# fujii-team/deComP

Measured on AMD Instinct MI355X. Metric: nmf_mu_iterations_per_s, higher is better.
Workload: dtype f32; 1 GPU; nmf_mu l2 no-mask Y=65536x4096 k=256 fp32 (BASELINE configs[1]); rows_per_gpu=65536, parallelism=rows sharded x1, 1 all-reduce/step, loop=single-GPU dcp_nmf_mu_f32

## Files before the change

### decomp_amd/_hip.py

```python
import ctypes
import os
import threading

_HERE = os.path.dirname(os.path.abspath(__file__))
LIB_PATH = os.path.join(_HERE, 'lib', 'libdecomp_hip.so')

OK = 0
ERR_NAMES = {-1: 'DCP_ERR_INVALID', -2: 'DCP_ERR_HIP', -3: 'DCP_ERR_NOMEM',
             -4: 'DCP_ERR_INTERNAL', -5: 'DCP_ERR_UNSUPPORTED', -6: 'DCP_ERR_REF_TYPEERROR',
             -7: 'DCP_ERR_COMM'}
LIK_L2, LIK_KL, LIK_BETA = 0, 1, 2
PROF_NLABELS = 10
PROF_XUPDATE, PROF_STATS = 2, 4
LASSO_ISTA, LASSO_ACC_ISTA, LASSO_FISTA, LASSO_CD = 0, 1, 2, 3
LASSO_PARALLEL_CD, LASSO_ADMM = 4, 5
LASSO_OMP = 6
LASSO_POSITIVE = 0x100
ERR_REF_TYPEERROR = -6
ERR_COMM = -7
COMM_ID_BYTES = 128
ALLREDUCE_FN = ctypes.CFUNCTYPE(ctypes.c_int, ctypes.c_void_p, ctypes.c_int64, ctypes.c_int, ctypes.c_void_p, ctypes.c_void_p)

_c_int, _c_i64, _c_vp = ctypes.c_int, ctypes.c_int64, ctypes.c_void_p
_c_f32, _c_f64 = ctypes.c_float, ctypes.c_double
_P = ctypes.POINTER

SIGNATURES = {
    'dcp_create': (_c_int, [_P(_c_vp), _c_int]),
    'dcp_destroy': (_c_int, [_c_vp]),
    'dcp_set_stream': (_c_int, [_c_vp, _c_vp]),
    'dcp_last_error_string': (ctypes.c_char_p, [_c_vp]),
    'dcp_build_info': (ctypes.c_char_p, []),
    'dcp_comm_unique_id': (_c_int, [_c_vp, _c_i64]),
    'dcp_comm_init': (_c_int, [_c_vp, _c_vp, _c_int, _c_int]),
    'dcp_comm_destroy': (_c_int, [_c_vp]),
    'dcp_comm_set_external': (_c_int, [_c_vp, _c_vp, _c_vp, _c_int, _c_int]),
    'dcp_memcpy': (_c_int, [_c_vp, _c_vp, _c_vp, _c_i64]),
    'dcp_comm_info': (_c_int, [_c_vp, _P(_c_int), _P(_c_int)]),
    'dcp_comm_allreduce_sum_f32': (_c_int, [_c_vp, _c_vp, _c_i64]),
    'dcp_comm_allreduce_sum_f64': (_c_int, [_c_vp, _c_vp, _c_i64]),
    'dcp_nmf_mu_sharded_f32': (_c_int, [_c_vp, _c_vp, _c_vp, _c_vp, _c_vp, _c_i64, _c_i64, _c_i64,
                                        _c_int, _c_f32, _c_int, _P(_c_int), _P(_c_f32)]),
    'dcp_nmf_mu_sharded_f64': (_c_int, [_c_vp, _c_vp, _c_vp, _c_vp, _c_vp, _c_i64, _c_i64, _c_i64,
                                        _c_int, _c_f64, _c_int, _P(_c_int), _P(_c_f64)]),
    'dcp_profile_enable': (_c_int, [_c_vp, _c_int]),
    'dcp_profile_reset': (_c_int, [_c_vp]),
    'dcp_profile_select': (_c_int, [_c_vp, ctypes.c_uint]),
    'dcp_profile_read': (_c_int, [_c_vp, _c_int, _P(_c_f64), _P(_c_i64)]),
    'dcp_profile_label_name': (ctypes.c_char_p, [_c_int]),
    'dcp_l2_normalize_f32': (_c_int, [_c_vp, _c_vp, _c_i64, _c_i64, _c_int]),
    'dcp_l2_normalize_f64': (_c_int, [_c_vp, _c_vp, _c_i64, _c_i64, _c_int]),
    'dcp_l2_normalize_c64': (_c_int, [_c_vp, _c_vp, _c_i64, _c_i64, _c_int]),
    'dcp_l2_normalize_c128': (_c_int, [_c_vp, _c_vp, _c_i64, _c_i64, _c_int]),
    'dcp_count_negative_f32': (_c_int, [_c_vp, _c_vp, _c_i64, _P(_c_i64)]),
    'dcp_count_negative_f64': (_c_int, [_c_vp, _c_vp, _c_i64, _P(_c_i64)]),
    'dcp_gemm_f32': (_c_int, [_c_vp, _c_int, _c_vp, _c_vp, _c_vp, _c_i64, _c_i64, _c_i64,
                              _c_int, _c_int]),
    'dcp_gemm_f64': (_c_int, [_c_vp, _c_int, _c_vp, _c_vp, _c_vp, _c_i64, _c_i64, _c_i64,
                              _c_int, _c_int]),
    'dcp_gather_rows_bytes': (_c_int, [_c_vp, _c_vp, _c_vp, _c_i64, _c_i64, _c_vp]),
    'dcp_scatter_rows_bytes': (_c_int, [_c_vp, _c_vp, _c_vp, _c_i64, _c_i64, _c_vp]),
    'dcp_dict_prefetch_rows_bytes': (_c_int, [_c_vp, _c_vp, _c_vp, _c_i64, _c_i64, _c_vp]),
    'dcp_dict_set_pcd_order': (_c_int, [_c_vp, _c_vp, _c_i64, _c_i64]),
    'dcp_lasso_f32': (_c_int, [_c_vp, _c_vp, _c_vp, _c_int, _c_vp, _c_vp, _c_i64, _c_i64, _c_i64, _c_f64, _c_f64, _c_int, _c_int, _c_int, _P(_c_int)]),
    'dcp_lasso_f64': (_c_int, [_c_vp, _c_vp, _c_vp, _c_int, _c_vp, _c_vp, _c_i64, _c_i64, _c_i64, _c_f64, _c_f64, _c_int, _c_int, _c_int, _P(_c_int)]),
    'dcp_lasso_c64': (_c_int, [_c_vp, _c_vp, _c_vp, _c_int, _c_vp, _c_vp, _c_i64, _c_i64, _c_i64, _c_f64, _c_f64, _c_int, _c_int, _c_int, _P(_c_int)]),
    'dcp_lasso_c128': (_c_int, [_c_vp, _c_vp, _c_vp, _c_int, _c_vp, _c_vp, _c_i64, _c_i64, _c_i64, _c_f64, _c_f64, _c_int, _c_int, _c_int, _P(_c_int)]),
    'dcp_lasso_pcd_f32': (_c_int, [_c_vp, _c_vp, _c_vp, _c_int, _c_vp, _c_vp, _c_i64, _c_i64, _c_i64, _c_f64, _c_f64, _c_int, _c_int, _c_vp, _c_i64, _P(_c_int)]),
    'dcp_lasso_admm_f32': (_c_int, [_c_vp, _c_vp, _c_vp, _c_int, _c_vp, _c_vp, _c_i64, _c_i64, _c_i64, _c_f64, _c_f64, _c_int, _c_int, _c_f64, _P(_c_int)]),
    'dcp_lasso_pcd_f64': (_c_int, [_c_vp, _c_vp, _c_vp, _c_int, _c_vp, _c_vp, _c_i64, _c_i64, _c_i64, _c_f64, _c_f64, _c_int, _c_int, _c_vp, _c_i64, _P(_c_int)]),
    'dcp_lasso_admm_f64': (_c_int, [_c_vp, _c_vp, _c_vp, _c_int, _c_vp, _c_vp, _c_i64, _c_i64, _c_i64, _c_f64, _c_f64, _c_int, _c_int, _c_f64, _P(_c_int)]),
    'dcp_lasso_pcd_c64': (_c_int, [_c_vp, _c_vp, _c_vp, _c_int, _c_vp, _c_vp, _c_i64, _c_i64, _c_i64, _c_f64, _c_f64, _c_int, _c_int, _c_vp, _c_i64, _P(_c_int)]),
    'dcp_lasso_admm_c64': (_c_int, [_c_vp, _c_vp, _c_vp, _c_int, _c_vp, _c_vp, _c_i64, _c_i64, _c_i64, _c_f64, _c_f64, _c_int, _c_int, _c_f64, _P(_c_int)]),
    'dcp_lasso_pcd_c128': (_c_int, [_c_vp, _c_vp, _c_vp, _c_int, _c_vp, _c_vp, _c_i64, _c_i64, _c_i64, _c_f64, _c_f64, _c_int, _c_int, _c_vp, _c_i64, _P(_c_int)]),
    'dcp_lasso_admm_c128': (_c_int, [_c_vp, _c_vp, _c_vp, _c_int, _c_vp, _c_vp, _c_i64, _c_i64, _c_i64, _c_f64, _c_f64, _c_int, _c_int, _c_f64, _P(_c_int)]),
    'dcp_omp_f32': (_c_int, [_c_vp, _c_vp, _c_vp, _c_vp, _c_i64, _c_i64, _c_i64, _c_int, _c_f64, _P(_c_int)]),
    'dcp_omp_f64': (_c_int, [_c_vp, _c_vp, _c_vp, _c_vp, _c_i64, _c_i64, _c_i64, _c_int, _c_f64, _P(_c_int)]),
    'dcp_omp_c64': (_c_int, [_c_vp, _c_vp, _c_vp, _c_vp, _c_i64, _c_i64, _c_i64, _c_int, _c_f64, _P(_c_int)]),
    'dcp_omp_c128': (_c_int, [_c_vp, _c_vp, _c_vp, _c_vp, _c_i64, _c_i64, _c_i64, _c_int, _c_f64, _P(_c_int)]),
    'dcp_omp_gram_f32': (_c_int, [_c_vp, _c_vp, _c_vp, _c_vp, _c_vp, _c_i64, _c_i64, _c_int, _c_f64, _P(_c_int)]),
    'dcp_omp_gram_f64': (_c_int, [_c_vp, _c_vp, _c_vp, _c_vp, _c_vp, _c_i64, _c_i64, _c_int, _c_f64, _P(_c_int)]),
    'dcp_omp_gram_c64': (_c_int, [_c_vp, _c_vp, _c_vp, _c_vp, _c_vp, _c_i64, _c_i64, _c_int, _c_f64, _P(_c_int)]),
    'dcp_omp_gram_c128': (_c_int, [_c_vp, _c_vp, _c_vp, _c_vp, _c_vp, _c_i64, _c_i64, _c_int, _c_f64, _P(_c_int)]),
    'dcp_omp_mask_f32': (_c_int, [_c_vp, _c_vp, _c_vp, _c_int, _c_vp, _c_vp, _c_i64, _c_i64, _c_i64, _c_int, _c_f64, _c_int, _P(_c_int)]),
    'dcp_omp_mask_f64': (_c_int, [_c_vp, _c_vp, _c_vp, _c_int, _c_vp, _c_vp, _c_i64, _c_i64, _c_i64, _c_int, _c_f64, _c_int, _P(_c_int)]),
    'dcp_omp_mask_c64': (_c_int, [_c_vp, _c_vp, _c_vp, _c_int, _c_vp, _c_vp, _c_i64, _c_i64, _c_i64, _c_int, _c_f64, _c_int, _P(_c_int)]),
    'dcp_omp_mask_c128': (_c_int, [_c_vp, _c_vp, _c_vp, _c_int, _c_vp, _c_vp, _c_i64, _c_i64, _c_i64, _c_int, _c_f64, _c_int, _P(_c_int)]),
    'dcp_ksvd_sweep_f32': (_c_int, [_c_vp, _c_vp, _c_vp, _c_vp, _c_i64, _c_i64, _c_i64, _c_int, _P(_c_f64)]),
    'dcp_ksvd_sweep_f64': (_c_int, [_c_vp, _c_vp, _c_vp, _c_vp, _c_i64, _c_i64, _c_i64, _c_int, _P(_c_f64)]),
    'dcp_ksvd_sweep_c64': (_c_int, [_c_vp, _c_vp, _c_vp, _c_vp, _c_i64, _c_i64, _c_i64, _c_int, _P(_c_f64)]),
    'dcp_ksvd_sweep_c128': (_c_int, [_c_vp, _c_vp, _c_vp, _c_vp, _c_i64, _c_i64, _c_i64, _c_int, _P(_c_f64)]),
    'dcp_ksvd_step_f32': (_c_int, [_c_vp, _c_vp, _c_vp, _c_vp, _c_i64, _c_i64, _c_i64, _c_int, _c_f64, _P(_c_f64), _P(_c_int)]),
    'dcp_ksvd_step_f64': (_c_int, [_c_vp, _c_vp, _c_vp, _c_vp, _c_i64, _c_i64, _c_i64, _c_int, _c_f64, _P(_c_f64), _P(_c_int)]),
    'dcp_ksvd_step_c64': (_c_int, [_c_vp, _c_vp, _c_vp, _c_vp, _c_i64, _c_i64, _c_i64, _c_int, _c_f64, _P(_c_f64), _P(_c_int)]),
    'dcp_ksvd_step_c128': (_c_int, [_c_vp, _c_vp, _c_vp, _c_vp, _c_i64, _c_i64, _c_i64, _c_int, _c_f64, _P(_c_f64), _P(_c_int)]),
    'dcp_ksvd_mask_sweep_f32': (_c_int, [_c_vp, _c_vp, _c_vp, _c_int, _c_vp, _c_vp, _c_i64, _c_i64, _c_i64, _c_int, _P(_c_f64)]),
    'dcp_ksvd_mask_sweep_f64': (_c_int, [_c_vp, _c_vp, _c_vp, _c_int, _c_vp, _c_vp, _c_i64, _c_i64, _c_i64, _c_int, _P(_c_f64)]),
    'dcp_ksvd_mask_sweep_c64': (_c_int, [_c_vp, _c_vp, _c_vp, _c_int, _c_vp, _c_vp, _c_i64, _c_i64, _c_i64, _c_int, _P(_c_f64)]),
    'dcp_ksvd_mask_sweep_c128': (_c_int, [_c_vp, _c_vp, _c_vp, _c_int, _c_vp, _c_vp, _c_i64, _c_i64, _c_i64, _c_int, _P(_c_f64)]),
    'dcp_ksvd_mask_step_f32': (_c_int, [_c_vp, _c_vp, _c_vp, _c_int, _c_vp, _c_vp, _c_i64, _c_i64, _c_i64, _c_int, _c_f64, _c_int, _P(_c_f64), _P(_c_int)]),
    'dcp_ksvd_mask_step_f64': (_c_int, [_c_vp, _c_vp, _c_vp, _c_int, _c_vp, _c_vp, _c_i64, _c_i64, _c_i64, _c_int, _c_f64, _c_int, _P(_c_f64), _P(_c_int)]),
    'dcp_ksvd_mask_step_c64': (_c_int, [_c_vp, _c_vp, _c_vp, _c_int, _c_vp, _c_vp, _c_i64, _c_i64, _c_i64, _c_int, _c_f64, _c_int, _P(_c_f64), _P(_c_int)]),
    'dcp_ksvd_mask_step_c128': (_c_int, [_c_vp, _c_vp, _c_vp, _c_int, _c_vp, _c_vp, _c_i64, _c_i64, _c_i64, _c_int, _c_f64, _c_int, _P(_c_f64), _P(_c_int)]),
    'dcp_dict_stats_f32': (_c_int, [_c_vp, _c_vp, _c_vp, _c_vp, _c_i64, _c_i64, _c_i64, _c_f64, _c_int, _c_int, _c_f64, _c_vp, _P(_c_int)]),
    'dcp_dict_update_f32': (_c_int, [_c_vp, _c_vp, _c_f64, _c_vp, _c_vp, _c_vp, _c_vp, _c_i64, _c_i64, _c_vp]),
    'dcp_dict_step_f32': (_c_int, [_c_vp, _c_vp, _c_vp, _c_vp, _c_vp, _c_vp, _c_vp, _c_i64, _c_i64, _c_i64, _c_f64, _c_f64, _c_int, _c_int, _c_f64, _P(_c_f64), _P(_c_int)]),
    'dcp_dict_step_async_f32': (_c_int, [_c_vp, _c_vp, _c_vp, _c_vp, _c_vp, _c_vp, _c_vp, _c_i64, _c_i64, _c_i64, _c_f64, _c_f64, _c_int, _c_int, _c_f64, _c_vp, _P(_c_int)]),
    'dcp_gather_rows_f32': (_c_int, [_c_vp, _c_vp, _c_vp, _c_i64, _c_i64, _c_vp]),
    'dcp_dict_stats_f64': (_c_int, [_c_vp, _c_vp, _c_vp, _c_vp, _c_i64, _c_i64, _c_i64, _c_f64, _c_int, _c_int, _c_f64, _c_vp, _P(_c_int)]),
    'dcp_dict_update_f64': (_c_int, [_c_vp, _c_vp, _c_f64, _c_vp, _c_vp, _c_vp, _c_vp, _c_i64, _c_i64, _c_vp]),
    'dcp_dict_step_f64': (_c_int, [_c_vp, _c_vp, _c_vp, _c_vp, _c_vp, _c_vp, _c_vp, _c_i64, _c_i64, _c_i64, _c_f64, _c_f64, _c_int, _c_int, _c_f64, _P(_c_f64), _P(_c_int)]),
    'dcp_dict_step_async_f64': (_c_int, [_c_vp, _c_vp, _c_vp, _c_vp, _c_vp, _c_vp, _c_vp, _c_i64, _c_i64, _c_i64, _c_f64, _c_f64, _c_int, _c_int, _c_f64, _c_vp, _P(_c_int)]),
    'dcp_gather_rows_f64': (_c_int, [_c_vp, _c_vp, _c_vp, _c_i64, _c_i64, _c_vp]),
    'dcp_dict_stats_c64': (_c_int, [_c_vp, _c_vp, _c_vp, _c_vp, _c_i64, _c_i64, _c_i64, _c_f64, _c_int, _c_int, _c_f64, _c_vp, _P(_c_int)]),
    'dcp_dict_update_c64': (_c_int, [_c_vp, _c_vp, _c_f64, _c_vp, _c_vp, _c_vp, _c_vp, _c_i64, _c_i64, _c_vp]),
    'dcp_dict_step_c64': (_c_int, [_c_vp, _c_vp, _c_vp, _c_vp, _c_vp, _c_vp, _c_vp, _c_i64, _c_i64, _c_i64, _c_f64, _c_f64, _c_int, _c_int, _c_f64, _P(_c_f64), _P(_c_int)]),
    'dcp_dict_step_async_c64': (_c_int, [_c_vp, _c_vp, _c_vp, _c_vp, _c_vp, _c_vp, _c_vp, _c_i64, _c_i64, _c_i64, _c_f64, _c_f64, _c_int, _c_int, _c_f64, _c_vp, _P(_c_int)]),
    'dcp_gather_rows_c64': (_c_int, [_c_vp, _c_vp, _c_vp, _c_i64, _c_i64, _c_vp]),
    'dcp_dict_stats_c128': (_c_int, [_c_vp, _c_vp, _c_vp, _c_vp, _c_i64, _c_i64, _c_i64, _c_f64, _c_int, _c_int, _c_f64, _c_vp, _P(_c_int)]),
    'dcp_dict_update_c128': (_c_int, [_c_vp, _c_vp, _c_f64, _c_vp, _c_vp, _c_vp, _c_vp, _c_i64, _c_i64, _c_vp]),
    'dcp_dict_step_c128': (_c_int, [_c_vp, _c_vp, _c_vp, _c_vp, _c_vp, _c_vp, _c_vp, _c_i64, _c_i64, _c_i64, _c_f64, _c_f64, _c_int, _c_int, _c_f64, _P(_c_f64), _P(_c_int)]),
    'dcp_dict_step_async_c128': (_c_int, [_c_vp, _c_vp, _c_vp, _c_vp, _c_vp, _c_vp, _c_vp, _c_i64, _c_i64, _c_i64, _c_f64, _c_f64, _c_int, _c_int, _c_f64, _c_vp, _P(_c_int)]),
    'dcp_gather_rows_c128': (_c_int, [_c_vp, _c_vp, _c_vp, _c_i64, _c_i64, _c_vp]),
    'dcp_dict_mask_step_f32': (_c_int, [_c_vp, _c_vp, _c_vp, _c_vp, _c_vp, _c_vp, _c_vp, _c_vp, _c_i64, _c_i64, _c_i64, _c_f64, _c_f64, _c_int, _c_int, _c_f64, _P(_c_f64), _P(_c_int)]),
    'dcp_dict_mask_step_f64': (_c_int, [_c_vp, _c_vp, _c_vp, _c_vp, _c_vp, _c_vp, _c_vp, _c_vp, _c_i64, _c_i64, _c_i64, _c_f64, _c_f64, _c_int, _c_int, _c_f64, _P(_c_f64), _P(_c_int)]),
    'dcp_dict_mask_step_c64': (_c_int, [_c_vp, _c_vp, _c_vp, _c_vp, _c_vp, _c_vp, _c_vp, _c_vp, _c_i64, _c_i64, _c_i64, _c_f64, _c_f64, _c_int, _c_int, _c_f64, _P(_c_f64), _P(_c_int)]),
    'dcp_dict_mask_step_c128': (_c_int, [_c_vp, _c_vp, _c_vp, _c_vp, _c_vp, _c_vp, _c_vp, _c_vp, _c_i64, _c_i64, _c_i64, _c_f64, _c_f64, _c_int, _c_int, _c_f64, _P(_c_f64), _P(_c_int)]),
    'dcp_nmf_grads_f32': (_c_int, [_c_vp, _c_vp, _c_vp, _c_vp, _c_vp, _c_i64, _c_i64, _c_i64, _c_int, _c_int, _c_vp, _c_vp]),
    'dcp_nmf_grads_f64': (_c_int, [_c_vp, _c_vp, _c_vp, _c_vp, _c_vp, _c_i64, _c_i64, _c_i64, _c_int, _c_int, _c_vp, _c_vp]),
    'dcp_nmf_grad_x_f32': (_c_int, [_c_vp, _c_vp, _c_vp, _c_vp, _c_vp, _c_i64, _c_i64, _c_i64, _c_int, _c_vp, _c_vp]),
    'dcp_nmf_grad_x_f64': (_c_int, [_c_vp, _c_vp, _c_vp, _c_vp, _c_vp, _c_i64, _c_i64, _c_i64, _c_int, _c_vp, _c_vp]),
    'dcp_nmf_gauss_logp_f32': (_c_int, [_c_vp, _c_vp, _c_vp, _c_vp, _c_vp, _c_i64, _c_i64, _c_i64, _c_f64, _P(_c_f64)]),
    'dcp_nmf_gauss_logp_f64': (_c_int, [_c_vp, _c_vp, _c_vp, _c_vp, _c_vp, _c_i64, _c_i64, _c_i64, _c_f64, _P(_c_f64)]),
    'dcp_set_nmf_beta': (_c_int, [_c_vp, _c_f64]),
    'dcp_set_nmf_penalty': (_c_int, [_c_vp, _c_f64, _c_f64]),
    'dcp_nmf_beta_divergence_f32': (_c_int, [_c_vp, _c_vp, _c_vp, _c_vp, _c_vp, _c_i64, _c_i64, _c_i64, _P(_c_f64)]),
    'dcp_nmf_beta_divergence_f64': (_c_int, [_c_vp, _c_vp, _c_vp, _c_vp, _c_vp, _c_i64, _c_i64, _c_i64, _P(_c_f64)]),
    'dcp_nmf_apply_f32': (_c_int, [_c_vp, _c_vp, _c_vp, _c_vp, _c_f64, _c_vp, _c_i64, _c_i64, _P(_c_f64)]),
    'dcp_nmf_apply_f64': (_c_int, [_c_vp, _c_vp, _c_vp, _c_vp, _c_f64, _c_vp, _c_i64, _c_i64, _P(_c_f64)]),
    'dcp_axpby_f32': (_c_int, [_c_vp, _c_i64, _c_f64, _c_vp, _c_f64, _c_vp]),
    'dcp_axpby_f64': (_c_int, [_c_vp, _c_i64, _c_f64, _c_vp, _c_f64, _c_vp]),
    'dcp_mu_quotient_f32': (_c_int, [_c_vp, _c_vp, _c_vp, _c_vp, _c_i64, _c_i64, _c_vp]),
    'dcp_mu_quotient_f64': (_c_int, [_c_vp, _c_vp, _c_vp, _c_vp, _c_i64, _c_i64, _c_vp]),
    'dcp_l2_normalize_diff_f32': (_c_int, [_c_vp, _c_vp, _c_vp, _c_vp, _c_i64, _c_i64, _c_int, _P(_c_f64)]),
    'dcp_l2_normalize_diff_f64': (_c_int, [_c_vp, _c_vp, _c_vp, _c_vp, _c_i64, _c_i64, _c_int, _P(_c_f64)]),
    'dcp_gershgorin_f32': (_c_int, [_c_vp, _c_vp, _c_i64, _c_i64, _c_vp]),
    'dcp_gershgorin_f64': (_c_int, [_c_vp, _c_vp, _c_i64, _c_i64, _c_vp]),
    'dcp_gershgorin_c64': (_c_int, [_c_vp, _c_vp, _c_i64, _c_i64, _c_vp]),
    'dcp_gershgorin_c128': (_c_int, [_c_vp, _c_vp, _c_i64, _c_i64, _c_vp]),
    'dcp_inv_f32': (_c_int, [_c_vp, _c_vp, _c_i64, _c_i64, _c_vp]),
    'dcp_inv_f64': (_c_int, [_c_vp, _c_vp, _c_i64, _c_i64, _c_vp]),
    'dcp_inv_c64': (_c_int, [_c_vp, _c_vp, _c_i64, _c_i64, _c_vp]),
    'dcp_inv_c128': (_c_int, [_c_vp, _c_vp, _c_i64, _c_i64, _c_vp]),
    'dcp_debug_tn_plain': (_c_int, [_c_int]),
    'dcp_debug_gemm_route': (_c_int, [_c_int, _c_int, _c_i64, _c_i64, _c_i64, _c_i64, _c_int, _c_int, _c_int, _c_int,
                                      _c_int, _c_vp]),
    'dcp_gemm_bf16x6_f32': (_c_int, [_c_vp, _c_int, _c_vp, _c_vp, _c_vp, _c_i64, _c_i64, _c_i64, _c_int]),
    'dcp_set_f32_product_mode': (_c_int, [_c_vp, _c_int]),
    'dcp_calib_read_f32': (_c_int, [_c_vp, _c_vp, _c_i64, _c_i64, _c_int, _c_vp]),
    'dcp_gemm_c64': (_c_int, [_c_vp, _c_int, _c_vp, _c_vp, _c_vp, _c_i64, _c_i64, _c_i64,
                              _c_int, _c_int]),
    'dcp_gemm_c128': (_c_int, [_c_vp, _c_int, _c_vp, _c_vp, _c_vp, _c_i64, _c_i64, _c_i64,
                              _c_int, _c_int]),
    'dcp_nmf_mu_f32': (_c_int, [_c_vp, _c_vp, _c_vp, _c_vp, _c_vp, _c_i64, _c_i64, _c_i64,
                                _c_int, _c_f32, _c_int, _P(_c_int), _P(_c_f32), _P(_c_f32)]),
    'dcp_nmf_mu_f64': (_c_int, [_c_vp, _c_vp, _c_vp, _c_vp, _c_vp, _c_i64, _c_i64, _c_i64,
                                _c_int, _c_f64, _c_int, _P(_c_int), _P(_c_f64), _P(_c_f64)]),
    'dcp_nmf_hals_f32': (_c_int, [_c_vp, _c_vp, _c_vp, _c_vp, _c_i64, _c_i64, _c_i64, _c_f32, _c_int,
                                  _P(_c_int), _P(_c_f32), _P(_c_f32)]),
    'dcp_nmf_hals_f64': (_c_int, [_c_vp, _c_vp, _c_vp, _c_vp, _c_i64, _c_i64, _c_i64, _c_f64, _c_int,
                                  _P(_c_int), _P(_c_f64), _P(_c_f64)]),
    'dcp_nmf_hals_sharded_f32': (_c_int, [_c_vp, _c_vp, _c_vp, _c_vp, _c_i64, _c_i64, _c_i64, _c_f32, _c_int,
                                          _P(_c_int), _P(_c_f32)]),
    'dcp_nmf_hals_sharded_f64': (_c_int, [_c_vp, _c_vp, _c_vp, _c_vp, _c_i64, _c_i64, _c_i64, _c_f64, _c_int,
                                          _P(_c_int), _P(_c_f64)]),
    'dcp_nmf_impute_f32': (_c_int, [_c_vp, _c_vp, _c_vp, _c_vp, _c_vp, _c_i64, _c_i64, _c_i64, _c_vp]),
    'dcp_nmf_impute_f64': (_c_int, [_c_vp, _c_vp, _c_vp, _c_vp, _c_vp, _c_i64, _c_i64, _c_i64, _c_vp]),
    'dcp_nmf_emhals_f32': (_c_int, [_c_vp, _c_vp, _c_vp, _c_vp, _c_vp, _c_i64, _c_i64, _c_i64, _c_f32, _c_int,
                                    _P(_c_int), _P(_c_f32), _P(_c_f32)]),
    'dcp_nmf_emhals_f64': (_c_int, [_c_vp, _c_vp, _c_vp, _c_vp, _c_vp, _c_i64, _c_i64, _c_i64, _c_f64, _c_int,
                                    _P(_c_int), _P(_c_f64), _P(_c_f64)]),
    'dcp_nmf_emhals_sharded_f32': (_c_int, [_c_vp, _c_vp, _c_vp, _c_vp, _c_vp, _c_i64, _c_i64, _c_i64, _c_f32,
                                            _c_int, _P(_c_int), _P(_c_f32)]),
    'dcp_nmf_emhals_sharded_f64': (_c_int, [_c_vp, _c_vp, _c_vp, _c_vp, _c_vp, _c_i64, _c_i64, _c_i64, _c_f64,
                                            _c_int, _P(_c_int), _P(_c_f64)]),
    'dcp_nmf_hals_stats_f32': (_c_int, [_c_vp, _c_vp, _c_vp, _c_vp, _c_vp, _c_i64, _c_i64, _c_i64, _c_vp]),
    'dcp_nmf_hals_stats_f64': (_c_int, [_c_vp, _c_vp, _c_vp, _c_vp, _c_vp, _c_i64, _c_i64, _c_i64, _c_vp]),
    'dcp_nmf_hals_update_f32': (_c_int, [_c_vp, _c_vp, _c_vp, _c_vp, _c_vp, _c_i64, _c_i64, _c_i64, _c_vp, _c_vp]),
    'dcp_nmf_hals_update_f64': (_c_int, [_c_vp, _c_vp, _c_vp, _c_vp, _c_vp, _c_i64, _c_i64, _c_i64, _c_vp, _c_vp]),
    'dcp_nn_cd_sweep_f32': (_c_int, [_c_vp, _c_vp, _c_vp, _c_vp, _c_vp, _c_i64, _c_i64, _c_int]),
    'dcp_nn_cd_sweep_f64': (_c_int, [_c_vp, _c_vp, _c_vp, _c_vp, _c_vp, _c_i64, _c_i64, _c_int]),
    'dcp_nmf_mu_stats_width': (_c_i64, [_c_i64, _c_i64, _c_int, _c_int]),
    'dcp_nmf_mu_stats_f32': (_c_int, [_c_vp, _c_vp, _c_vp, _c_vp, _c_vp, _c_vp, _c_i64, _c_i64,
                                      _c_i64, _c_int, _c_vp]),
    'dcp_nmf_mu_stats_f64': (_c_int, [_c_vp, _c_vp, _c_vp, _c_vp, _c_vp, _c_vp, _c_i64, _c_i64,
                                      _c_i64, _c_int, _c_vp]),
    'dcp_nmf_mask_bits_words': (_c_i64, [_c_i64, _c_i64]),
    'dcp_nmf_mask_prepare_f32': (_c_int, [_c_vp, _c_vp, _c_vp, _c_i64, _c_i64, _c_vp, _c_vp, _P(_c_int)]),
    'dcp_nmf_mask_prepare_f64': (_c_int, [_c_vp, _c_vp, _c_vp, _c_i64, _c_i64, _c_vp, _c_vp, _P(_c_int)]),
    'dcp_nmf_mu_stats_prepared_f32': (_c_int, [_c_vp, _c_vp, _c_vp, _c_vp, _c_vp, _c_vp, _c_vp, _c_i64,
                                               _c_i64, _c_i64, _c_int, _c_vp]),
    'dcp_nmf_mu_stats_prepared_f64': (_c_int, [_c_vp, _c_vp, _c_vp, _c_vp, _c_vp, _c_vp, _c_vp, _c_i64,
                                               _c_i64, _c_i64, _c_int, _c_vp]),
    'dcp_nmf_mu_update_f32': (_c_int, [_c_vp, _c_vp, _c_vp, _c_vp, _c_i64, _c_i64, _c_int,
                                       _c_int, _c_vp, _c_vp]),
    'dcp_nmf_mu_update_f64': (_c_int, [_c_vp, _c_vp, _c_vp, _c_vp, _c_i64, _c_i64, _c_int,
                                       _c_int, _c_vp, _c_vp]),
    'dcp_nmf_residual_f32': (_c_int, [_c_vp, _c_vp, _c_vp, _c_vp, _c_vp, _c_i64, _c_i64, _c_i64,
                                      _P(_c_f64)]),
    'dcp_nmf_residual_f64': (_c_int, [_c_vp, _c_vp, _c_vp, _c_vp, _c_vp, _c_i64, _c_i64, _c_i64,
                                      _P(_c_f64)]),
    'dcp_tm_temp2mat_f32': (_c_int, [_c_vp, _c_vp, _c_i64, _c_i64, _c_i64, _c_i64, _c_int, _c_vp]),
    'dcp_tm_temp2mat_f64': (_c_int, [_c_vp, _c_vp, _c_i64, _c_i64, _c_i64, _c_i64, _c_int, _c_vp]),
    'dcp_tm_temp2mat_c64': (_c_int, [_c_vp, _c_vp, _c_i64, _c_i64, _c_i64, _c_i64, _c_int, _c_vp]),
    'dcp_tm_temp2mat_c128': (_c_int, [_c_vp, _c_vp, _c_i64, _c_i64, _c_i64, _c_i64, _c_int, _c_vp]),
    'dcp_tm_coef2mat_f32': (_c_int, [_c_vp, _c_vp, _c_i64, _c_i64, _c_i64, _c_i64, _c_i64, _c_int, _c_vp]),
    'dcp_tm_coef2mat_f64': (_c_int, [_c_vp, _c_vp, _c_i64, _c_i64, _c_i64, _c_i64, _c_i64, _c_int, _c_vp]),
    'dcp_tm_coef2mat_c64': (_c_int, [_c_vp, _c_vp, _c_i64, _c_i64, _c_i64, _c_i64, _c_i64, _c_int, _c_vp]),
    'dcp_tm_coef2mat_c128': (_c_int, [_c_vp, _c_vp, _c_i64, _c_i64, _c_i64, _c_i64, _c_i64, _c_int, _c_vp]),
    'dcp_tm_predict_f32': (_c_int, [_c_vp, _c_vp, _c_vp, _c_i64, _c_i64, _c_i64, _c_i64, _c_i64, _c_int, _c_vp]),
    'dcp_tm_predict_f64': (_c_int, [_c_vp, _c_vp, _c_vp, _c_i64, _c_i64, _c_i64, _c_i64, _c_i64, _c_int, _c_vp]),
    'dcp_tm_predict_c64': (_c_int, [_c_vp, _c_vp, _c_vp, _c_i64, _c_i64, _c_i64, _c_i64, _c_i64, _c_int, _c_vp]),
    'dcp_tm_predict_c128': (_c_int, [_c_vp, _c_vp, _c_vp, _c_i64, _c_i64, _c_i64, _c_i64, _c_i64, _c_int, _c_vp]),
    'dcp_tm_lasso_f32': (_c_int, [_c_vp, _c_vp, _c_vp, _c_vp, _c_i64, _c_i64, _c_i64, _c_i64, _c_i64, _c_int, _c_f64, _c_f64, _c_int, _c_int, _c_int, _P(_c_int)]),
    'dcp_tm_lasso_f64': (_c_int, [_c_vp, _c_vp, _c_vp, _c_vp, _c_i64, _c_i64, _c_i64, _c_i64, _c_i64, _c_int, _c_f64, _c_f64, _c_int, _c_int, _c_int, _P(_c_int)]),
    'dcp_tm_lasso_c64': (_c_int, [_c_vp, _c_vp, _c_vp, _c_vp, _c_i64, _c_i64, _c_i64, _c_i64, _c_i64, _c_int, _c_f64, _c_f64, _c_int, _c_int, _c_int, _P(_c_int)]),
    'dcp_tm_lasso_c128': (_c_int, [_c_vp, _c_vp, _c_vp, _c_vp, _c_i64, _c_i64, _c_i64, _c_i64, _c_i64, _c_int, _c_f64, _c_f64, _c_int, _c_int, _c_int, _P(_c_int)]),
    'dcp_tm_dstep_f32': (_c_int, [_c_vp, _c_vp, _c_vp, _c_vp, _c_vp, _c_vp, _c_i64, _c_i64, _c_i64, _c_i64, _c_i64, _c_int, _c_int, _P(_c_f64)]),
    'dcp_tm_dstep_f64': (_c_int, [_c_vp, _c_vp, _c_vp, _c_vp, _c_vp, _c_vp, _c_i64, _c_i64, _c_i64, _c_i64, _c_i64, _c_int, _c_int, _P(_c_f64)]),
    'dcp_tm_dstep_c64': (_c_int, [_c_vp, _c_vp, _c_vp, _c_vp, _c_vp, _c_vp, _c_i64, _c_i64, _c_i64, _c_i64, _c_i64, _c_int, _c_int, _P(_c_f64)]),
    'dcp_tm_dstep_c128': (_c_int, [_c_vp, _c_vp, _c_vp, _c_vp, _c_vp, _c_vp, _c_i64, _c_i64, _c_i64, _c_i64, _c_i64, _c_int, _c_int, _P(_c_f64)]),
    'dcp_tm_gather_windows_f32': (_c_int, [_c_vp, _c_vp, _c_vp, _c_vp, _c_vp, _c_i64, _c_i64, _c_i64, _c_i64, _c_i64, _c_i64, _c_i64, _c_int, _c_vp, _c_vp]),
    'dcp_tm_gather_windows_f64': (_c_int, [_c_vp, _c_vp, _c_vp, _c_vp, _c_vp, _c_i64, _c_i64, _c_i64, _c_i64, _c_i64, _c_i64, _c_i64, _c_int, _c_vp, _c_vp]),
    'dcp_tm_gather_windows_c64': (_c_int, [_c_vp, _c_vp, _c_vp, _c_vp, _c_vp, _c_i64, _c_i64, _c_i64, _c_i64, _c_i64, _c_i64, _c_i64, _c_int, _c_vp, _c_vp]),
    'dcp_tm_gather_windows_c128': (_c_int, [_c_vp, _c_vp, _c_vp, _c_vp, _c_vp, _c_i64, _c_i64, _c_i64, _c_i64, _c_i64, _c_i64, _c_i64, _c_int, _c_vp, _c_vp]),
    'dcp_tm_scatter_windows_f32': (_c_int, [_c_vp, _c_vp, _c_vp, _c_vp, _c_vp, _c_i64, _c_i64, _c_i64, _c_i64, _c_i64, _c_i64, _c_i64, _c_int]),
    'dcp_tm_scatter_windows_f64': (_c_int, [_c_vp, _c_vp, _c_vp, _c_vp, _c_vp, _c_i64, _c_i64, _c_i64, _c_i64, _c_i64, _c_i64, _c_i64, _c_int]),
    'dcp_tm_scatter_windows_c64': (_c_int, [_c_vp, _c_vp, _c_vp, _c_vp, _c_vp, _c_i64, _c_i64, _c_i64, _c_i64, _c_i64, _c_i64, _c_i64, _c_int]),
    'dcp_tm_scatter_windows_c128': (_c_int, [_c_vp, _c_vp, _c_vp, _c_vp, _c_vp, _c_i64, _c_i64, _c_i64, _c_i64, _c_i64, _c_i64, _c_i64, _c_int]),
}

_lib = None
_lock = threading.Lock()
_handles = {}


class HipLibraryError(RuntimeError):
    """The HIP library is missing, failed to load, or a call into it failed."""


def load():
    global _lib
    with _lock:
        if _lib is not None:
            return _lib
        if not os.path.exists(LIB_PATH):
            raise HipLibraryError(
                'libdecomp_hip.so not found at %s. Build it with `make` (or '
                '`python -c "import __graft_entry__ as g; g.build()"`). decomp_amd has no '
                'CPU fallback: the HIP library is the compute path.' % LIB_PATH)
        try:
            lib = ctypes.CDLL(LIB_PATH)
        except OSError as e:
            raise HipLibraryError('cannot load %s: %s' % (LIB_PATH, e))
        for name, (res, args) in SIGNATURES.items():
            fn = getattr(lib, name)
            fn.restype = res
            fn.argtypes = args
        _lib = lib
        return _lib


def handle(device):
    lib = load()
    with _lock:
        h = _handles.get(device)
        if h is None:
            out = _c_vp()
            rc = lib.dcp_create(ctypes.byref(out), int(device))
            if rc != OK or not out.value:
                raise HipLibraryError(
                    'dcp_create(device=%d) failed (%s): no usable HIP device. decomp_amd '
                    'computes only on the GPU.' % (device, ERR_NAMES.get(rc, rc)))
            h = out
            _handles[device] = h
        return h


def check(h, rc, what):
    if rc != OK:
        msg = load().dcp_last_error_string(h)
        raise HipLibraryError('%s failed: %s (%s)' % (
            what, ERR_NAMES.get(rc, rc), msg.decode() if msg else ''))
```

### decomp_amd/csrc/gemm_mfma_bf16x6.hpp

```cpp
#pragma once
#include "gemm_mfma_f32.hpp"
#include <type_traits>

namespace dcp {

typedef __bf16 x6_bf16x4 __attribute__((ext_vector_type(4)));
typedef __bf16 x6_bf16x8 __attribute__((ext_vector_type(8)));

template <int BM_, int BN_, int WM_, int WN_, int MINW_, int STAGES_>
struct X6Cfg {
    static constexpr int BM = BM_, BN = BN_, BK = 16, WM = WM_, WN = WN_, MINW = MINW_;
    static constexpr int NWAVES = (BM_ / WM_) * (BN_ / WN_);
    static constexpr int NTHREADS = 64 * NWAVES;
    static constexpr int STAGES = STAGES_;
};
typedef X6Cfg<256, 256, 64, 64, 1, 3> X6Huge;
typedef X6Cfg<128, 128, 64, 64, 2, 2> X6Large;

template <int ROWS>
struct X6Panel {
    static constexpr int PLANE_BYTES = ROWS * 32;
    static constexpr int BYTES = 3 * PLANE_BYTES;
};

__device__ __forceinline__ int x6_chunk(int r, int q) { return r * 32 + ((q ^ ((r >> 3) & 1)) << 4); }

__device__ __forceinline__ void x6_split(f32x4 a, x6_bf16x4& h, x6_bf16x4& m, x6_bf16x4& l) {
    h = __builtin_convertvector(a, x6_bf16x4);
    const f32x4 r1 = a - __builtin_convertvector(h, f32x4);
    m = __builtin_convertvector(r1, x6_bf16x4);
    const f32x4 r2 = r1 - __builtin_convertvector(m, f32x4);
    l = __builtin_convertvector(r2, x6_bf16x4);
}

template <int LAY, int ROWS, int NT, int G>
__device__ __forceinline__ void x6_gload(f32x4 (&r)[G], const float* __restrict__ p, long ld, int row0, int k0,
                                         int tid) {
    static_assert(G * NT * 4 == ROWS * 16, "panel must be a whole number of 4-value groups per thread");
#pragma unroll
    for (int i = 0; i < G; ++i) {
        const int idx = tid + i * NT;
        if (LAY == KMAJOR) {
            const int row = idx >> 2, kq = idx & 3;
            r[i] = *reinterpret_cast<const f32x4*>(p + (long)(row0 + row) * ld + (k0 + 4 * kq));
        } else {
            const int g = idx % (ROWS / 4), k = idx / (ROWS / 4);
            r[i] = *reinterpret_cast<const f32x4*>(p + (long)(k0 + k) * ld + (row0 + 4 * g));
        }
    }
}

template <int ROWS>
__device__ __forceinline__ int x6_granule(int k, int g) {
    static_assert(ROWS >= 128, "the XOR swizzle needs 32 granules per k row");
    return k * (ROWS * 2) + ((g ^ ((k & 3) << 3)) << 3);
}

template <int LAY, int ROWS, int NT, int G>
__device__ __forceinline__ void x6_lds_store(char* s, const f32x4 (&r)[G], int tid) {
#pragma unroll
    for (int i = 0; i < G; ++i) {
        const int idx = tid + i * NT;
        int off;
        if (LAY == KMAJOR) {
            const int row = idx >> 2, kq = idx & 3;
            off = x6_chunk(row, kq >> 1) + ((kq & 1) << 3);
        } else {
            off = x6_granule<ROWS>(idx / (ROWS / 4), idx % (ROWS / 4));
        }
        x6_bf16x4 h, m, l;
        x6_split(r[i], h, m, l);
        *reinterpret_cast<x6_bf16x4*>(s + off) = h;
        *reinterpret_cast<x6_bf16x4*>(s + X6Panel<ROWS>::PLANE_BYTES + off) = m;
        *reinterpret_cast<x6_bf16x4*>(s + 2 * X6Panel<ROWS>::PLANE_BYTES + off) = l;
    }
}

template <int LAY, int ROWS>
__device__ __forceinline__ int x6_frag_off(int r0, int lane) {
    const int l31 = lane & 31, h = lane >> 5;
    if (LAY == KMAJOR) return x6_chunk(r0 + l31, h);
    const int q = (lane >> 2) & 3, pq = lane & 3, gh = (lane >> 4) & 1;
    return x6_granule<ROWS>(8 * h + q, (r0 >> 2) + 4 * gh + pq);
}

template <int LAY, int ROWS>
__device__ __forceinline__ x6_bf16x8 x6_frag(const char* plane, int off) {
    if (LAY == KMAJOR) return *reinterpret_cast<const x6_bf16x8*>(plane + off);
    typedef short s16x4 __attribute__((ext_vector_type(4)));
    typedef __attribute__((address_space(3))) s16x4 lds_s16x4;
    const s16x4 lo = __builtin_amdgcn_ds_read_tr16_b64_v4i16((lds_s16x4*)(plane + off));
    const s16x4 hi = __builtin_amdgcn_ds_read_tr16_b64_v4i16((lds_s16x4*)(plane + off + 4 * ROWS * 2));
    return __builtin_bit_cast(x6_bf16x8, __builtin_shufflevector(lo, hi, 0, 1, 2, 3, 4, 5, 6, 7));
}

template <class E, class = void>
struct epi_den_tail { static constexpr bool value = false; };
template <class E>
struct epi_den_tail<E, decltype((void)E::kDenTail)> { static constexpr bool value = E::kDenTail; };

typedef float x6_f32x2 __attribute__((ext_vector_type(2)));

__device__ __forceinline__ int x6_den_xoff(int r, int q) { return r * 16 + ((q ^ ((r >> 2) & 3)) << 2); }

template <class Epi>
__device__ __forceinline__ void x6_den_tail(f32x16 (&num)[2][2], const Epi& epi, char* smem, int m0, int n0, int tid) {
    constexpr int XS = 128 * 16 * 4;
    constexpr int GS = 16 * 256 * 4;
    constexpr int DBUF = XS + GS;
    const int lane = tid & 63, wave = tid >> 6;
    const int wm = wave >> 2, wn = wave & 3;
    const int l31 = lane & 31, h = lane >> 5;
    const int nkd = epi.depth >> 4;

    const int pr = tid >> 3, k2 = tid & 7;
    const float* xsrc = epi.cur + (long)(m0 + (pr >> 5) * 64 + (pr & 31)) * epi.ld_cur + 2 * k2;
    const int xdst = (x6_den_xoff(pr, k2 >> 1) + 2 * (k2 & 1)) * 4;
    const int gk = tid >> 6, gc = tid & 63;
    const float* gsrc = epi.gram + (long)gk * epi.ld_gram + (n0 + 4 * gc);
    const int gdst = XS + (gk * 256 + 4 * gc) * 4;
    int lp = 0, lk = 0;
    auto gload = [&](x6_f32x2& rx, f32x4& rg) {
        rx = *reinterpret_cast<const x6_f32x2*>(xsrc + (long)(32 * lp) * epi.ld_cur + 16 * lk);
        rg = *reinterpret_cast<const f32x4*>(gsrc + (long)(16 * lk) * epi.ld_gram);
        if (lk + 1 < nkd) {
            ++lk;
        } else if (lp == 0) {
            lp = 1;
            lk = 0;
        }
    };
    auto lstore = [&](int buf, const x6_f32x2& rx, const f32x4& rg) {
        *reinterpret_cast<x6_f32x2*>(smem + buf + xdst) = rx;
        *reinterpret_cast<f32x4*>(smem + buf + gdst) = rg;
    };

    x6_f32x2 rx;
    f32x4 rg;
    int b0 = 0, b1 = DBUF, b2 = 2 * DBUF;
    {
        x6_f32x2 rx0, rx1;
        f32x4 rg0, rg1;
        gload(rx0, rg0);
        gload(rx1, rg1);
        gload(rx, rg);
        __syncthreads();
        lstore(b0, rx0, rg0);
        lstore(b1, rx1, rg1);
        __syncthreads();
    }

    const int xfrag0 = x6_den_xoff(wm * 32 + l31, h) * 4, xfrag1 = x6_den_xoff(wm * 32 + l31, 2 + h) * 4;
    const int gfrag = XS + ((4 * h) * 256 + wn * 64 + l31) * 4;
    const int tq = l31 & 3, col0 = l31 & ~3;

    auto pass = [&](auto i_tag) {
        constexpr int i = decltype(i_tag)::value;
        f32x16 den[2];
#pragma unroll
        for (int j = 0; j < 2; ++j)
#pragma unroll
            for (int r = 0; r < 16; ++r) den[j][r] = 0.0f;
        for (int kb = 0; kb < nkd; ++kb) {
            const char* s = smem + b0;
            auto frags = [&](int xoff, int c, f32x4& fa, f32x4 (&fb)[2]) {
                fa = *reinterpret_cast<const f32x4*>(s + xoff);
                const float* g = reinterpret_cast<const float*>(s + gfrag) + c * 8 * 256;
#pragma unroll
                for (int j = 0; j < 2; ++j)
#pragma unroll
                    for (int st = 0; st < 4; ++st) fb[j][st] = g[st * 256 + j * 32];
            };
            auto mfmas = [&](const f32x4& fa, const f32x4 (&fb)[2]) {
#pragma unroll
                for (int st = 0; st < 4; ++st)
#pragma unroll
                    for (int j = 0; j < 2; ++j)
                        den[j] = __builtin_amdgcn_mfma_f32_32x32x2f32(fa[st], fb[j][st], den[j], 0, 0, 0);
            };
            f32x4 fa, fb[2];
            frags(xfrag0, 0, fa, fb);
            mfmas(fa, fb);
            __builtin_amdgcn_sched_barrier(0);
            lstore(b2, rx, rg);
            f32x4 ga, gb[2];
            frags(xfrag1, 1, ga, gb);
            __builtin_amdgcn_sched_barrier(0);
            __syncthreads();
            __builtin_amdgcn_sched_barrier(0);
            gload(rx, rg);
            mfmas(ga, gb);
            __builtin_amdgcn_sched_barrier(0);
            const int t0 = b0;
            b0 = b1;
            b1 = b2;
            b2 = t0;
        }
#pragma unroll
        for (int j = 0; j < 2; ++j)
#pragma unroll
            for (int g = 0; g < 4; ++g) {
                f32x4 a, d;
#pragma unroll
                for (int e = 0; e < 4; ++e) {
                    a[e] = num[i][j][4 * g + e];
                    d[e] = den[j][4 * g + e];
                }
                epi.quot4(m0 + wm * 64 + i * 32 + 8 * g + 4 * h + tq, n0 + wn * 64 + j * 32 + col0,
                          quad_transpose(a, tq), quad_transpose(d, tq));
            }
    };
    pass(std::integral_constant<int, 0>{});
    pass(std::integral_constant<int, 1>{});
}

template <class Cfg, int ALAY, int BLAY, class Epi>
__global__ void __launch_bounds__(Cfg::NTHREADS, Cfg::MINW) gemm_bf16x6_kernel(GemmProblem p, Epi epi) {
    constexpr int BM = Cfg::BM, BN = Cfg::BN, BK = Cfg::BK, WM = Cfg::WM, WN = Cfg::WN;
    constexpr int TM = WM / 32, TN = WN / 32;
    constexpr int WAVES_N = BN / WN;
    constexpr int NT = Cfg::NTHREADS;
    constexpr int GA = BM * BK / 4 / NT, GB = BN * BK / 4 / NT;
    constexpr int PA = X6Panel<BM>::PLANE_BYTES, PB = X6Panel<BN>::PLANE_BYTES;
    constexpr int BUF = X6Panel<BM>::BYTES + X6Panel<BN>::BYTES;
    static_assert(epi_mode<Epi>::value == 0 && !epi_rowbits<Epi>::value, "bf16x6 core: plain real epilogues");

    extern __shared__ __attribute__((aligned(16))) char x6_smem[];

    const int tid = threadIdx.x;
    const int lane = tid & 63, wave = tid >> 6;
    const int wm = wave / WAVES_N, wn = wave % WAVES_N;
    const int l31 = lane & 31, h = lane >> 5;

    const int lid = xcd_remap(blockIdx.x, gridDim.x);
    const int tiles = p.tiles_m * p.tiles_n;
    const int split = lid / tiles;
    const int t = lid - split * tiles;
    int mt, nt;
    if (p.mt_fast) {
        mt = t % p.tiles_m;
        nt = t / p.tiles_m;
    } else {
        nt = t % p.tiles_n;
        mt = t / p.tiles_n;
    }
    const int m0 = mt * BM;
    const int kbeg = split * p.klen;
    const int kend = min(p.K, kbeg + p.klen);
    const float* Bp = p.B;
    long ldb = p.ldb;
    int nB0 = nt * BN;
    int n0 = nB0;
    if (nt >= p.tiles_n1) {
        Bp = p.B2;
        ldb = p.ldb2;
        nB0 = (nt - p.tiles_n1) * BN;
        n0 = p.n_b1 + nB0;
    }

    f32x16 acc[TM][TN];
#pragma unroll
    for (int i = 0; i < TM; ++i)
#pragma unroll
        for (int j = 0; j < TN; ++j)
#pragma unroll
            for (int r = 0; r < 16; ++r) acc[i][j][r] = 0.0f;

    static_assert(TM == 2, "one panel's staging per 32-row A block");
    constexpr int STAGES = Cfg::STAGES;
    static_assert(STAGES == 2 || STAGES == 3, "two buffers and a boundary barrier, or a ring of three");
    f32x4 ra[GA], rb[GB];
    const int nkb = (kend - kbeg) / BK;
    if (nkb > 0) {
        x6_gload<ALAY, BM, NT>(ra, p.A, p.lda, m0, kbeg, tid);
        x6_gload<BLAY, BN, NT>(rb, Bp, ldb, nB0, kbeg, tid);
        x6_lds_store<ALAY, BM, NT>(x6_smem, ra, tid);
        x6_lds_store<BLAY, BN, NT>(x6_smem + X6Panel<BM>::BYTES, rb, tid);
        const int k1 = kbeg + min(1, nkb - 1) * BK;
        x6_gload<ALAY, BM, NT>(ra, p.A, p.lda, m0, k1, tid);
        x6_gload<BLAY, BN, NT>(rb, Bp, ldb, nB0, k1, tid);
        if constexpr (STAGES == 3) {
            x6_lds_store<ALAY, BM, NT>(x6_smem + BUF, ra, tid);
            x6_lds_store<BLAY, BN, NT>(x6_smem + BUF + X6Panel<BM>::BYTES, rb, tid);
            const int k2 = kbeg + min(2, nkb - 1) * BK;
            x6_gload<ALAY, BM, NT>(ra, p.A, p.lda, m0, k2, tid);
            x6_gload<BLAY, BN, NT>(rb, Bp, ldb, nB0, k2, tid);
        }
    }
    __syncthreads();

    int aoff[TM], boff[TN];
#pragma unroll
    for (int i = 0; i < TM; ++i) aoff[i] = x6_frag_off<ALAY, BM>(wm * WM + i * 32, lane);
#pragma unroll
    for (int j = 0; j < TN; ++j) boff[j] = x6_frag_off<BLAY, BN>(wn * WN + j * 32, lane);

    constexpr int STAGE_AFTER = 2;
    auto kblock = [&](int cur, int nxt_off, int knext, auto stage_tag, auto bar_tag) {
        constexpr bool STAGE = decltype(stage_tag)::value;
        constexpr bool BAR = decltype(bar_tag)::value;
        const char* sA = x6_smem + cur;
        const char* sB = sA + X6Panel<BM>::BYTES;
        char* nxt = x6_smem + nxt_off;
        x6_bf16x8 fb[3][TN];
#pragma unroll
        for (int pl = 0; pl < 3; ++pl)
#pragma unroll
            for (int j = 0; j < TN; ++j) fb[pl][j] = x6_frag<BLAY, BN>(sB + pl * PB, boff[j]);
        constexpr int TA[6] = {2, 0, 1, 1, 0, 0};
        constexpr int TB[6] = {0, 2, 1, 0, 1, 0};
        auto group = [&](auto i_tag) {
            constexpr int i = decltype(i_tag)::value;
            x6_bf16x8 fa[3];
#pragma unroll
            for (int pl = 0; pl < 3; ++pl) fa[pl] = x6_frag<ALAY, BM>(sA + pl * PA, aoff[i]);
            if constexpr (BAR && i == 1) {
                __builtin_amdgcn_sched_barrier(0);
                __syncthreads();
                __builtin_amdgcn_sched_barrier(0);
            }
            auto mfmas = [&](int t0, int t1) {
#pragma unroll
                for (int tt = t0; tt < t1; ++tt)
#pragma unroll
                    for (int j = 0; j < TN; ++j)
                        acc[i][j] =
                            __builtin_amdgcn_mfma_f32_32x32x16_bf16(fa[TA[tt]], fb[TB[tt]][j], acc[i][j], 0, 0, 0);
            };
            if constexpr (STAGE) {
                mfmas(0, STAGE_AFTER);
                __builtin_amdgcn_sched_barrier(0);
                if constexpr (i == 0) {
                    x6_lds_store<ALAY, BM, NT>(nxt, ra, tid);
                    x6_gload<ALAY, BM, NT>(ra, p.A, p.lda, m0, knext, tid);
                } else {
                    x6_lds_store<BLAY, BN, NT>(nxt + X6Panel<BM>::BYTES, rb, tid);
                    x6_gload<BLAY, BN, NT>(rb, Bp, ldb, nB0, knext, tid);
                }
                __builtin_amdgcn_sched_barrier(0);
                mfmas(STAGE_AFTER, 6);
            } else {
                mfmas(0, 6);
            }
            __builtin_amdgcn_sched_barrier(0);
        };
        group(std::integral_constant<int, 0>{});
        group(std::integral_constant<int, 1>{});
    };
    if constexpr (STAGES == 2) {
        for (int kb = 0; kb + 1 < nkb; ++kb) {
            const int cur = (kb & 1) * BUF;
            kblock(cur, cur ^ BUF, kbeg + min(kb + 2, nkb - 1) * BK, std::true_type{}, std::false_type{});
            __syncthreads();
        }
        if (nkb > 0) kblock(((nkb - 1) & 1) * BUF, 0, 0, std::false_type{}, std::false_type{});
    } else {
        int b0 = 0, b1 = BUF, b2 = 2 * BUF;
        for (int kb = 0; kb + 2 < nkb; ++kb) {
            kblock(b0, b2, kbeg + min(kb + 3, nkb - 1) * BK, std::true_type{}, std::true_type{});
            const int t0 = b0;
            b0 = b1;
            b1 = b2;
            b2 = t0;
        }
        if (nkb > 1) kblock(b0, 0, 0, std::false_type{}, std::true_type{});
        if (nkb > 0) kblock(nkb > 1 ? b1 : b0, 0, 0, std::false_type{}, std::false_type{});
    }

    if constexpr (epi_den_tail<Epi>::value) {
        static_assert(BM == 256 && BN == 256 && NT == 1024 && STAGES == 3 && ALAY == KMAJOR && BLAY == KMAJOR,
                      "the denominator tail is laid out for the 256 x 256 NT tile");
        x6_den_tail(acc, epi, x6_smem, m0, n0, tid);
    } else if constexpr (epi_vec4<Epi>::value) {
        const int tq = l31 & 3, col0 = (l31 & ~3);
#pragma unroll
        for (int i = 0; i < TM; ++i)
#pragma unroll
            for (int j = 0; j < TN; ++j)
#pragma unroll
                for (int g = 0; g < 4; ++g) {
                    f32x4 x;
#pragma unroll
                    for (int e = 0; e < 4; ++e) x[e] = acc[i][j][4 * g + e];
                    const f32x4 y = quad_transpose(x, tq);
                    epi.vec4(m0 + wm * WM + i * 32 + 8 * g + 4 * h + tq, n0 + wn * WN + j * 32 + col0, y, split);
                }
    } else {
#pragma unroll
        for (int i = 0; i < TM; ++i)
#pragma unroll
            for (int j = 0; j < TN; ++j) {
                const int col = n0 + wn * WN + j * 32 + l31;
#pragma unroll
                for (int r = 0; r < 16; ++r) {
                    const int row = m0 + wm * WM + i * 32 + (r & 3) + 8 * (r >> 2) + 4 * h;
                    epi(row, col, acc[i][j][r], split);
                }
            }
    }
}

template <class Epi>
inline bool x6_epi_ok(const Epi& epi) {
    if constexpr (epi_vec4<Epi>::value) return epi.vec_ok();
    else return true;
}

template <class Cfg>
inline bool x6_eligible(const GemmProblem& p) {
    auto al16 = [](const void* q) { return (reinterpret_cast<uintptr_t>(q) & 15) == 0; };
    const int n1 = p.B2 != nullptr ? p.n_b1 : p.N;
    bool ok = p.M > 0 && p.N > 0 && p.K > 0 && (p.M % Cfg::BM) == 0 && (n1 % Cfg::BN) == 0 &&
              ((p.N - n1) % Cfg::BN) == 0 && (p.K % 16) == 0 && p.A2 == nullptr && (p.lda % 4) == 0 &&
              (p.ldb % 4) == 0 && al16(p.A) && al16(p.B);
    if (p.B2 != nullptr) ok = ok && (p.ldb2 % 4) == 0 && al16(p.B2);
    if (p.ksplits > 1) ok = ok && (p.klen % 16) == 0 && p.klen > 0;
    return ok;
}

template <class Cfg, int ALAY, int BLAY, class Epi>
inline hipError_t launch_gemm_bf16x6(hipStream_t stream, GemmProblem p, const Epi& epi) {
    if (!x6_eligible<Cfg>(p) || !x6_epi_ok(epi)) return hipErrorInvalidValue;
    if constexpr (epi_den_tail<Epi>::value) {
        if (p.ksplits > 1 || p.B2 != nullptr || epi.depth < 48 || (epi.depth % 16) != 0) return hipErrorInvalidValue;
    }
    if (p.B2 == nullptr) p.n_b1 = p.N;
    p.m_a1 = p.M;
    p.tiles_m1 = p.tiles_m = p.M / Cfg::BM;
    p.tiles_n1 = p.n_b1 / Cfg::BN;
    p.tiles_n = p.tiles_n1 + (p.N - p.n_b1) / Cfg::BN;
    if (p.ksplits < 1) p.ksplits = 1;
    if (p.ksplits == 1) p.klen = p.K;
    p.vec_epi = epi_vec4<Epi>::value ? 1 : 0;
    p.al_mask = 0;
    const int grid = p.tiles_m * p.tiles_n * p.ksplits;
    if (grid <= 0) return hipSuccess;
    constexpr int lds_bytes = Cfg::STAGES * (X6Panel<Cfg::BM>::BYTES + X6Panel<Cfg::BN>::BYTES);
    const void* fn = reinterpret_cast<const void*>(&gemm_bf16x6_kernel<Cfg, ALAY, BLAY, Epi>);
    if constexpr (lds_bytes > 65536) {
        static DynLdsRaised raised;
        std::atomic<bool>& done = raised.on_current_device();
        if (!done) {
            hipError_t e = hipFuncSetAttribute(fn, hipFuncAttributeMaxDynamicSharedMemorySize, lds_bytes);
            if (e != hipSuccess) return e;
            done = true;
        }
    }
    hipLaunchKernelGGL((gemm_bf16x6_kernel<Cfg, ALAY, BLAY, Epi>), dim3(grid), dim3(Cfg::NTHREADS), lds_bytes,
                       stream, p, epi);
    return hipGetLastError();
}

}
```

### decomp_amd/csrc/handle.hpp

```cpp
#pragma once
#include <hip/hip_runtime.h>
#include <stdint.h>
#include <stdio.h>
#include <string>
#include <vector>

#include "../../include/decomp_hip.h"
#include "scalar.hpp"

struct dcp_handle {
    int device = 0;
    hipStream_t stream = nullptr;
    hipEvent_t stream_switch = nullptr;
    hipStream_t arena_stream = nullptr;
    bool arena_stream_set = false;
    hipStream_t side = nullptr;
    hipEvent_t ev_main = nullptr, ev_side = nullptr;
    char* arena = nullptr;
    size_t arena_bytes = 0;
    size_t arena_used = 0;
    void* host_pinned = nullptr;
    size_t host_pinned_bytes = 0;
    std::string err;
    void* comm = nullptr;
    int comm_rank = 0, comm_world = 1;
    dcp_allreduce_fn comm_ext = nullptr;
    void* comm_ext_user = nullptr;
    const void* pf_in = nullptr;
    const int64_t* pf_index = nullptr;
    void* pf_out = nullptr;
    int64_t pf_rows = 0, pf_row_bytes = 0;
    bool pf_inflight = false;
    int* lasso_deferred_flag = nullptr;
    int* lasso_deferred_it = nullptr;
    int lasso_deferred_it_met = 0;
    bool lasso_deferred_copy = false;
    int lasso_it_sink = 0;
    const int* pcd_order = nullptr;
    int64_t pcd_rows = 0, pcd_K = 0;
    bool prof_on = false;
    unsigned prof_mask = 0xffffffffu;
    struct ProfRec { int label; hipEvent_t a, b; };
    std::vector<ProfRec> prof_recs;
    std::vector<hipEvent_t> prof_pool;
    double prof_ms[DCP_PROF_NLABELS] = {0};
    long long prof_cnt[DCP_PROF_NLABELS] = {0};
    int f32_product_mode = 0;
    double nmf_beta = 0.0;
    double nmf_l1 = 0.0, nmf_l2 = 0.0;
};

namespace dcp {

inline int fail(dcp_handle* h, int code, const std::string& msg) {
    if (h) h->err = msg;
    return code;
}

#define DCP_HIP_OK(h, expr)                                                                  \
    do {                                                                                     \
        hipError_t _e = (expr);                                                              \
        if (_e != hipSuccess)                                                                \
            return dcp::fail((h), DCP_ERR_HIP,                                               \
                             std::string(#expr) + ": " + hipGetErrorString(_e));             \
    } while (0)

#define DCP_LAUNCH_OK(h, what)                                                        \
    do {                                                                              \
        hipError_t _e = (what);                                                       \
        if (_e != hipSuccess)                                                         \
            return dcp::fail((h), DCP_ERR_HIP, std::string("launch failed: ") +       \
                                                   hipGetErrorString(_e));            \
    } while (0)

#define DCP_TRY(expr)                  \
    do {                               \
        int _rc = (expr);              \
        if (_rc != DCP_OK) return _rc; \
    } while (0)

struct ProfScope {
    dcp_handle* h;
    int label;
    hipEvent_t a = nullptr, b = nullptr;
    static hipEvent_t take(dcp_handle* h) {
        if (!h->prof_pool.empty()) {
            hipEvent_t e = h->prof_pool.back();
            h->prof_pool.pop_back();
            return e;
        }
        hipEvent_t e = nullptr;
        if (hipEventCreate(&e) != hipSuccess) return nullptr;
        return e;
    }
    ProfScope(dcp_handle* h_, int label_) : h(h_), label(label_) {
        if (!h->prof_on || !((h->prof_mask >> label) & 1u)) return;
        a = take(h);
        b = take(h);
        if (a) (void)hipEventRecord(a, h->stream);
    }
    ~ProfScope() {
        if (!a || !b) return;
        (void)hipEventRecord(b, h->stream);
        h->prof_recs.push_back({label, a, b});
    }
};

constexpr unsigned kOrderingEvent = hipEventDisableTiming | hipEventDisableSystemFence;

inline int side_after_main(dcp_handle* h) {
    if (h->side == nullptr) {
        if (hipStreamCreateWithFlags(&h->side, hipStreamNonBlocking) != hipSuccess ||
            hipEventCreateWithFlags(&h->ev_main, kOrderingEvent) != hipSuccess ||
            hipEventCreateWithFlags(&h->ev_side, kOrderingEvent) != hipSuccess)
            return fail(h, DCP_ERR_HIP, "side stream creation failed");
    }
    if (hipEventRecord(h->ev_main, h->stream) != hipSuccess ||
        hipStreamWaitEvent(h->side, h->ev_main, 0) != hipSuccess)
        return fail(h, DCP_ERR_HIP, "side stream fork failed");
    return DCP_OK;
}
inline int main_after_side(dcp_handle* h) {
    if (hipEventRecord(h->ev_side, h->side) != hipSuccess ||
        hipStreamWaitEvent(h->stream, h->ev_side, 0) != hipSuccess)
        return fail(h, DCP_ERR_HIP, "side stream join failed");
    return DCP_OK;
}

int move_rows_on(dcp_handle* h, hipStream_t stream, const void* in, const int64_t* in_index, void* out,
                 const int64_t* out_index, int64_t rows, int64_t row_bytes);

inline int start_registered_prefetch(dcp_handle* h) {
    if (h->pf_rows <= 0 || h->pf_row_bytes <= 0) return DCP_OK;
    DCP_TRY(side_after_main(h));
    DCP_TRY(move_rows_on(h, h->side, h->pf_in, h->pf_index, h->pf_out, nullptr, h->pf_rows, h->pf_row_bytes));
    h->pf_rows = 0;
    h->pf_inflight = true;
    return DCP_OK;
}

inline void ws_order_streams(dcp_handle* h) {
    if (h->arena_stream_set && h->arena_stream != h->stream && h->arena != nullptr) {
        bool ok = false;
        if (h->stream_switch == nullptr)
            (void)hipEventCreateWithFlags(&h->stream_switch, kOrderingEvent);
        if (h->stream_switch != nullptr && hipEventRecord(h->stream_switch, h->arena_stream) == hipSuccess &&
            hipStreamWaitEvent(h->stream, h->stream_switch, 0) == hipSuccess)
            ok = true;
        if (!ok) {
            (void)hipGetLastError();
            (void)hipDeviceSynchronize();
        }
    }
    h->arena_stream = h->stream;
    h->arena_stream_set = true;
}

inline int ws_reserve(dcp_handle* h, size_t bytes) {
    ws_order_streams(h);
    if (bytes <= h->arena_bytes) return DCP_OK;
    if (h->arena) {
        hipError_t e = hipStreamSynchronize(h->stream);
        if (e != hipSuccess) return fail(h, DCP_ERR_HIP, hipGetErrorString(e));
        (void)hipFree(h->arena);
        h->arena = nullptr;
        h->arena_bytes = 0;
    }
    size_t want = bytes + (bytes >> 3) + (1u << 20);
    void* p = nullptr;
    hipError_t e = hipMalloc(&p, want);
    if (e != hipSuccess) {
        want = bytes;
        e = hipMalloc(&p, want);
    }
    if (e != hipSuccess)
        return fail(h, DCP_ERR_NOMEM,
                    "workspace hipMalloc of " + std::to_string(bytes) + " bytes failed: " +
                        hipGetErrorString(e));
    h->arena = static_cast<char*>(p);
    h->arena_bytes = want;
    h->arena_used = 0;
    return DCP_OK;
}

inline size_t align256(size_t b) { return (b + 255) & ~size_t(255); }

struct WsLayout {
    char* base = nullptr;
    size_t used = 0;
    template <class T>
    void take(T*& p, size_t count) {
        p = base ? reinterpret_cast<T*>(base + used) : nullptr;
        used += align256(count * sizeof(T));
    }
};

template <class Items>
inline int ws_lay_out(dcp_handle* h, Items&& items) {
    WsLayout sizing;
    items(sizing);
// ... 70 lines not shown
```

### decomp_amd/csrc/kernels_small.hpp

```cpp
#pragma once
#include <hip/hip_runtime.h>
#include "reduce.hpp"
#include "scalar.hpp"

namespace dcp {

inline int grid_for(long n, int cap = 2048) {
    long g = (n + 255) / 256;
    if (g < 1) g = 1;
    if (g > cap) g = cap;
    return (int)g;
}

template <class T>
__global__ void __launch_bounds__(256) reduce_slabs_kernel(const T* __restrict__ slabs, long stride,
                                                           int S, long count, T* __restrict__ out) {
    for (long i = blockIdx.x * 256L + threadIdx.x; i < count; i += (long)gridDim.x * 256L)
        out[i] = slab_sum<16, 8>(slabs, stride, S, i);
}
template <class T>
inline void launch_reduce_slabs_scalar(hipStream_t st, const T* slabs, long stride, int S, long count, T* out,
                                       int cap = 2048) {
    hipLaunchKernelGGL((reduce_slabs_kernel<T>), dim3(grid_for(count, cap)), dim3(256), 0, st, slabs, stride, S, count,
                       out);
}

template <class T, int VEC>
__global__ void __launch_bounds__(256) reduce_slabs_vec_kernel(const T* __restrict__ slabs, long stride, int S,
                                                               long count, T* __restrict__ out) {
    typedef T vec_t __attribute__((ext_vector_type(VEC)));
    const long nvec = count / VEC, svec = stride / VEC;
    const vec_t* __restrict__ in = reinterpret_cast<const vec_t*>(slabs);
    vec_t* __restrict__ o = reinterpret_cast<vec_t*>(out);
    for (long i = blockIdx.x * 256L + threadIdx.x; i < nvec; i += (long)gridDim.x * 256L)
        o[i] = slab_sum<8, 2>(in, svec, S, i);
}

template <class T>
inline void launch_reduce_slabs(hipStream_t st, const T* slabs, long stride, int S, long count, T* out) {
    if constexpr (std::is_same<T, float>::value || std::is_same<T, double>::value) {
        constexpr int VEC = 16 / sizeof(T);
        if (count % VEC == 0 && stride % VEC == 0 && (reinterpret_cast<uintptr_t>(slabs) & 15) == 0 &&
            (reinterpret_cast<uintptr_t>(out) & 15) == 0 && count >= 64 * 1024) {
            long g = (count / VEC + 255) / 256;
            if (g > 2048) g = 2048;
            hipLaunchKernelGGL((reduce_slabs_vec_kernel<T, VEC>), dim3((unsigned)g), dim3(256), 0, st, slabs, stride, S,
                               count, out);
            return;
        }
    }
    launch_reduce_slabs_scalar<T>(st, slabs, stride, S, count, out);
}

template <class T>
__global__ void __launch_bounds__(256) reduce_slabs_affine_kernel(const T* __restrict__ slabs, long stride, int S,
                                                                  long count, T sub, long diag_n, T add_diag,
                                                                  T* __restrict__ out) {
    for (long i = blockIdx.x * 256L + threadIdx.x; i < count; i += (long)gridDim.x * 256L) {
        T acc = slab_sum(slabs, stride, S, i);
        if (diag_n > 0 && i % (diag_n + 1) == 0) acc = acc + add_diag;
        out[i] = acc - sub;
    }
}

template <class T>
inline void launch_reduce_slabs_affine(hipStream_t st, const T* slabs, long stride, int S, long count, T sub,
                                       long diag_n, T add_diag, T* out) {
    hipLaunchKernelGGL((reduce_slabs_affine_kernel<T>), dim3(grid_for(count)), dim3(256), 0, st, slabs, stride, S, count,
                       sub, diag_n, add_diag, out);
}

template <class T>
__global__ void __launch_bounds__(256) reduce_slabs_rows_kernel(const T* __restrict__ slabs,
                                                                long stride, int S, long rows,
                                                                long cols, T* __restrict__ out,
                                                                long ld_out) {
    const long count = rows * cols;
    for (long i = blockIdx.x * 256L + threadIdx.x; i < count; i += (long)gridDim.x * 256L) {
        const long r = i / cols, c = i - r * cols;
        out[r * ld_out + c] = slab_sum(slabs, stride, S, i);
    }
}

template <class T>
__global__ void __launch_bounds__(256) bcast_rows_kernel(const T* __restrict__ v, long rows,
                                                         long cols, T* __restrict__ out,
                                                         long ld_out) {
    const long count = rows * cols;
    for (long i = blockIdx.x * 256L + threadIdx.x; i < count; i += (long)gridDim.x * 256L) {
        const long r = i / cols, c = i - r * cols;
        out[r * ld_out + c] = v[r];
    }
}

template <class T>
__global__ void __launch_bounds__(256) bcast_cols_kernel(const T* __restrict__ v, long rows, long cols,
                                                         T* __restrict__ out) {
    const long count = rows * cols;
    for (long i = blockIdx.x * 256L + threadIdx.x; i < count; i += (long)gridDim.x * 256L)
        out[i] = v[i % cols];
}

template <class T>
__global__ void __launch_bounds__(256) mul_mask_kernel(const T* __restrict__ a,
                                                       const real_t<T>* __restrict__ m, long rows,
                                                       long cols, long m_row_stride,
                                                       T* __restrict__ out) {
    const long n = rows * cols;
    for (long i = blockIdx.x * 256L + threadIdx.x; i < n; i += (long)gridDim.x * 256L) {
        const long r = i / cols, c = i - r * cols;
        out[i] = scale(a[i], m[r * m_row_stride + c]);
    }
}

template <class R>
__global__ void __launch_bounds__(256) mask_rowbits_kernel(const R* __restrict__ mask, long rows, long cols,
                                                           uint32_t* __restrict__ bits,
                                                           int* __restrict__ not_binary) {
    const long groups = (rows + 31) / 32;
    const long n = groups * cols;
    bool bad = false;
    for (long i = blockIdx.x * 256L + threadIdx.x; i < n; i += (long)gridDim.x * 256L) {
        const long g = i / cols, c = i - g * cols;
        uint32_t w = 0;
        for (int b0 = 0; b0 < 32; b0 += 8) {
            R m[8];
#pragma unroll
            for (int u = 0; u < 8; ++u) {
                const long r = g * 32 + b0 + u;
                m[u] = mask[(r < rows ? r : rows - 1) * cols + c];
            }
#pragma unroll
            for (int u = 0; u < 8; ++u) {
                const bool in = (g * 32 + b0 + u) < rows;
                if (in && m[u] != R(0)) w |= (1u << (b0 + u));
                if (in && m[u] != R(0) && m[u] != R(1)) bad = true;
            }
        }
        bits[i] = w;
    }
    if (bad) atomicOr(not_binary, 1);
}

template <class T>
__global__ void __launch_bounds__(256) mu_quotient_kernel(const T* __restrict__ cur, long ld_cur,
                                                          const T* __restrict__ num, long ld_num,
                                                          const T* __restrict__ den, long ld_den,
                                                          int den_bcast, long rows, long cols,
                                                          T* __restrict__ out, long ld_out) {
    const long n = rows * cols;
    for (long i = blockIdx.x * 256L + threadIdx.x; i < n; i += (long)gridDim.x * 256L) {
        const long r = i / cols, c = i - r * cols;
        const T d = den_bcast == 0 ? den[r * ld_den + c] : (den_bcast == 1 ? den[r] : den[c]);
        const T nu = num[r * ld_num + c];
        out[r * ld_out + c] =
            cur[r * ld_cur + c] * max_np(nu, T(0)) / max_np(d, T(1.0e-15));
    }
}

template <class T, bool PEN>
__global__ void __launch_bounds__(256) mu_quotient_slabs_kernel(const T* __restrict__ cur,
                                                                const T* __restrict__ slabs,
                                                                long stride, int S,
                                                                const T* __restrict__ den, long ld_den,
                                                                long rows, long cols, T l1, T l2,
                                                                T* __restrict__ out) {
    const long n = rows * cols;
    for (long i = blockIdx.x * 256L + threadIdx.x; i < n; i += (long)gridDim.x * 256L) {
        const T nu = slab_sum(slabs, stride, S, i);
        const long r = i / cols, c = i - r * cols;
        T d = den[r * ld_den + c];
        const T x = cur[i];
        if constexpr (PEN) d = d + l1 + l2 * x;
        out[i] = x * max_np(nu, T(0)) / max_np(d, T(1.0e-15));
    }
}

template <class T, bool PEN>
__global__ void __launch_bounds__(256) mu_quotient_stacked_kernel(const T* __restrict__ cur,
                                                                  const T* __restrict__ slabs, long stride,
                                                                  int S, long count, T l1, T l2,
                                                                  T* __restrict__ out) {
    for (long i = blockIdx.x * 256L + threadIdx.x; i < count; i += (long)gridDim.x * 256L) {
        const long at[2] = {i, count + i};
        T sum[2];
        slab_sums(slabs, stride, S, at, sum);
        T de = sum[0];
        const T nu = sum[1];
        const T x = cur[i];
        if constexpr (PEN) de = de + l1 + l2 * x;
        out[i] = x * max_np(nu, T(0)) / max_np(de, T(1.0e-15));
    }
}

template <class T>
__global__ void __launch_bounds__(256) row_normalize_kernel(const T* __restrict__ U, long ld_u,
                                                            long F, int strict,
                                                            const T* __restrict__ ref, long ld_ref,
                                                            T* __restrict__ out, long ld_out,
                                                            real_t<T>* __restrict__ rowmax,
                                                            real_t<T>* __restrict__ norm_out = nullptr,
                                                            real_t<T>* __restrict__ gmax = nullptr,
                                                            real_t<T>* __restrict__ gmax_zero = nullptr,
                                                            unsigned int* __restrict__ ticket = nullptr,
                                                            real_t<T>* __restrict__ host_out = nullptr) {
    typedef real_t<T> R;
    __shared__ R sh[4];
    __shared__ R s_inv;
    const long row = blockIdx.x;
    const T* u = U + row * ld_u;
    constexpr int CACHE = 16;
    const bool cached = F <= 256L * CACHE;
    T rc[CACHE];
    R acc = 0;
    if (cached) {
#pragma unroll
        for (int q = 0; q < CACHE; ++q) {
            const long j = threadIdx.x + 256L * q;
            rc[q] = (j < F) ? u[j] : zero_of<T>();
            acc += abs2(rc[q]);
        }
    } else {
        for (long j = threadIdx.x; j < F; j += 256) acc += abs2(u[j]);
    }
    R tot = block_sum_256(acc, sh);
    if (threadIdx.x == 0) {
        if (!strict) tot = tot > R(1) ? tot : R(1);
        s_inv = sqrt(tot);
        if (norm_out != nullptr) norm_out[row] = s_inv;
    }
    __syncthreads();
    const R nrm = s_inv;
    R md = 0;
    auto emit = [&](long j, T v) {
        T o;
        if constexpr (scalar_traits<T>::is_complex) {
            o.re = v.re / nrm;
            o.im = v.im / nrm;
        } else {
            o = v / nrm;
        }
        if (ref != nullptr) {
            const R d = absval(sub(ref[row * ld_ref + j], o));
            md = max_np(d, md);
        }
        out[row * ld_out + j] = o;
    };
    if (cached) {
#pragma unroll
        for (int q = 0; q < CACHE; ++q) {
            const long j = threadIdx.x + 256L * q;
            if (j < F) emit(j, rc[q]);
        }
    } else {
        for (long j = threadIdx.x; j < F; j += 256) emit(j, u[j]);
    }
    if (rowmax != nullptr || gmax != nullptr) {
        R m = block_max_256(md, sh);
        if (threadIdx.x == 0) {
            if (rowmax != nullptr) rowmax[row] = m;
            if (gmax_zero != nullptr && row == 0) *gmax_zero = R(0);
            if (gmax != nullptr) publish_max(m, gmax, ticket, host_out, true);
        }
    }
}

template <class T>
__global__ void __launch_bounds__(256) colsum_partial_kernel(const T* __restrict__ a, long ld,
                                                             long rows, long cols, long rows_per_blk,
                                                             T* __restrict__ partial) {
    const long r0 = blockIdx.y * rows_per_blk;
    const long r1 = min(rows, r0 + rows_per_blk);
    for (long c = blockIdx.x * 256L + threadIdx.x; c < cols; c += (long)gridDim.x * 256L) {
        T a0 = zero_of<T>(), a1 = zero_of<T>(), a2 = zero_of<T>(), a3 = zero_of<T>();
        long r = r0;
        for (; r + 3 < r1; r += 4) {
            a0 = add(a0, a[r * ld + c]);
            a1 = add(a1, a[(r + 1) * ld + c]);
            a2 = add(a2, a[(r + 2) * ld + c]);
            a3 = add(a3, a[(r + 3) * ld + c]);
        }
        for (; r < r1; ++r) a0 = add(a0, a[r * ld + c]);
        partial[blockIdx.y * cols + c] = add(add(a0, a1), add(a2, a3));
    }
}

template <class T>
__global__ void __launch_bounds__(256) rowsum_kernel(const T* __restrict__ a, long ld, long cols,
                                                     T* __restrict__ out) {
    __shared__ T sh[4];
    const long row = blockIdx.x;
    T acc = 0;
    for (long j = threadIdx.x; j < cols; j += 256) acc += a[row * ld + j];
    T t = block_sum_256(acc, sh);
    if (threadIdx.x == 0) out[row] = t;
}

}
```

### decomp_amd/csrc/nmf.hip

```cpp
#include <cmath>

#include "comm.hpp"
#include "nmf_loop.hpp"

using namespace dcp;

namespace {

template <class T>
int check_nmf_args(dcp_handle* h, const T* Y, const T* X, const T* D, int64_t N, int64_t F,
                   int64_t K, int lik) {
    DCP_TRY(check_nmf_dims(h, Y, X, D, N, F, K));
    if (lik != DCP_LIK_L2 && lik != DCP_LIK_KL && lik != DCP_LIK_BETA) return fail(h, DCP_ERR_INVALID, "bad likelihood");
    return DCP_OK;
}

template <class T>
struct MuStep {
    const T* Y;
    const T* mask;
    NmfShape<T> s;
    bool sharded;
    NmfStatsWs<T> ws;
    NmfUpdateWs<T> wu;
    T* stats = nullptr;
    uint32_t* mbits = nullptr;
    int* mflag = nullptr;
    const T* Ypre = nullptr;

    int64_t W() const { return nmf_stats_width(s.F, s.K, s.lik, s.masked); }
    bool want_bits() const { return s.masked && std::is_same<T, float>::value && s.lik == DCP_LIK_L2; }
    void layout(WsLayout& a) {
        nmf_stats_layout(a, ws, s, s.masked);
        nmf_update_layout(a, wu, s.F, s.K);
        a.take(stats, (size_t)s.K * W());
        if (want_bits()) {
            a.take(mbits, mask_bits_words(s.N, s.F));
            a.take(mflag, 4);
        }
    }
    int prepare(dcp_handle* h) {
        Ypre = Y;
        if (!s.masked) return DCP_OK;
        int binary = 0;
        DCP_TRY(nmf_mask_prepare<T>(h, Y, mask, s.N, s.F, ws.Ym, mbits, mflag, &binary));
        Ypre = ws.Ym;
        if (binary) ws.mbits = mbits;
        return DCP_OK;
    }
    int iterate(dcp_handle* h, const T* Xc, T* Xn, const T* Dc, T* Dn, const NmfStopSlots<T>& slots) {
        DCP_TRY(nmf_stats<T>(h, Ypre, mask, Xc, Xn, Dc, s, stats, ws, 3, nmf_penalty(h)));
        if (sharded) {
            ProfScope ps(h, DCP_PROF_EXCHANGE);
            DCP_TRY(comm_allreduce_sum(h, stats, (size_t)s.K * W(),
                                       std::is_same<T, float>::value ? COMM_F32 : COMM_F64));
        }
        return nmf_update<T>(h, stats, Dc, Dn, s.F, s.K, s.lik, s.masked, slots.md, wu, slots.md_next, slots.ticket,
                             slots.host);
    }
};

template <class T>
int nmf_mu_solve(dcp_handle* h, const T* Y, const T* mask, T* X, T* D, int64_t N, int64_t F,
                 int64_t K, int lik, T tol, int maxiter, int* it_out, T* last_maxdiff,
                 T* resid_trace, bool sharded = false) {
    DCP_TRY(check_nmf_args(h, Y, X, D, N, F, K, lik));
    if (!it_out) return fail(h, DCP_ERR_INVALID, "it_out is null");
    if (sharded && !comm_active(h))
        return fail(h, DCP_ERR_COMM, "dcp_nmf_mu_sharded_* needs a communicator (dcp_comm_init)");
    DCP_HIP_OK(h, hipSetDevice(h->device));
    MuStep<T> step{Y, mask, NmfShape<T>{N, F, K, lik, mask != nullptr}, sharded};
    return nmf_lagged_loop<T>(h, step, Y, mask, X, D, N, F, K, tol, maxiter, it_out, last_maxdiff, resid_trace);
}

template <class T>
struct NmfScalarWs {
    static constexpr int blocks = 1024;
    T* tmp = nullptr;
    double* part = nullptr;
    double* host = nullptr;
    int reserve(dcp_handle* h, int64_t N, int64_t F) {
        DCP_TRY(ws_lay_out(h, [&](WsLayout& a) {
            a.take(tmp, (size_t)N * F);
            a.take(part, blocks);
        }));
        void* hostv = nullptr;
        DCP_TRY(host_scratch(h, sizeof(double) * blocks, &hostv));
        host = reinterpret_cast<double*>(hostv);
        return DCP_OK;
    }
    int sum(dcp_handle* h, double* out) const { return read_partial_sum(h, part, blocks, host, out); }
};

template <class T>
int nmf_mu_stats_api(dcp_handle* h, const T* Y, const T* mask, const T* X, T* X_out, const T* D,
                     int64_t N, int64_t F, int64_t K, int lik, T* stats) {
    DCP_TRY(check_nmf_args(h, Y, X, D, N, F, K, lik));
    if (!stats || !X_out) return fail(h, DCP_ERR_INVALID, "stats / X_out is null");
    DCP_HIP_OK(h, hipSetDevice(h->device));
    const bool masked = mask != nullptr;
    NmfShape<T> s{N, F, K, lik, masked};
    NmfStatsWs<T> ws;
    DCP_TRY(ws_lay_out(h, [&](WsLayout& a) { nmf_stats_layout(a, ws, s, masked); }));
    const T* Ypre = nullptr;
    DCP_TRY(nmf_premask<T>(h, Y, mask, N, F, ws.Ym, &Ypre));
    return nmf_stats<T>(h, Ypre, mask, X, X_out, D, s, stats, ws, 3, nmf_penalty(h));
}

template <class T>
int nmf_mu_stats_prepared_api(dcp_handle* h, const T* Ym, const T* mask, const uint32_t* bits, const T* X,
                              T* X_out, const T* D, int64_t N, int64_t F, int64_t K, int lik, T* stats) {
    DCP_TRY(check_nmf_args(h, Ym, X, D, N, F, K, lik));
    if (!stats || !X_out || !mask) return fail(h, DCP_ERR_INVALID, "stats / X_out / mask is null");
    DCP_HIP_OK(h, hipSetDevice(h->device));
    NmfShape<T> s{N, F, K, lik, true};
    NmfStatsWs<T> ws;
    DCP_TRY(ws_lay_out(h, [&](WsLayout& a) { nmf_stats_layout(a, ws, s, false); }));
    ws.mbits = bits;
    return nmf_stats<T>(h, Ym, mask, X, X_out, D, s, stats, ws, 3, nmf_penalty(h));
}

template <class T>
int nmf_mask_prepare_api(dcp_handle* h, const T* Y, const T* mask, int64_t N, int64_t F, T* Ym,
                         uint32_t* bits, int* binary) {
    if (!h) return DCP_ERR_INVALID;
    if (!Y || !mask || !Ym || !binary) return fail(h, DCP_ERR_INVALID, "null pointer");
    if (N <= 0 || F <= 0) return fail(h, DCP_ERR_INVALID, "sizes must be positive");
    DCP_HIP_OK(h, hipSetDevice(h->device));
    int* flag = nullptr;
    DCP_TRY(ws_lay_out(h, [&](WsLayout& a) { a.take(flag, 4); }));
    return nmf_mask_prepare<T>(h, Y, mask, N, F, Ym, bits, flag, binary);
}

template <class T>
int nmf_mu_update_api(dcp_handle* h, const T* stats, const T* D, T* D_new, int64_t F, int64_t K,
                      int lik, int masked, T* maxdiff_dev, T* maxdiff_next) {
    if (!h) return DCP_ERR_INVALID;
    if (!stats || !D || !D_new || !maxdiff_dev) return fail(h, DCP_ERR_INVALID, "null pointer");
    if (F <= 0 || K <= 0) return fail(h, DCP_ERR_INVALID, "sizes must be positive");
    DCP_HIP_OK(h, hipSetDevice(h->device));
    NmfUpdateWs<T> wu;
    DCP_TRY(ws_lay_out(h, [&](WsLayout& a) { nmf_update_layout(a, wu, F, K); }));
    return nmf_update<T>(h, stats, D, D_new, F, K, lik, masked != 0, maxdiff_dev, wu, maxdiff_next);
}

template <class T>
int nmf_residual_api(dcp_handle* h, const T* Y, const T* mask, const T* X, const T* D, int64_t N,
                     int64_t F, int64_t K, double* out) {
    DCP_TRY(check_nmf_args(h, Y, X, D, N, F, K, DCP_LIK_L2));
    if (!out) return fail(h, DCP_ERR_INVALID, "out is null");
    DCP_HIP_OK(h, hipSetDevice(h->device));
    NmfScalarWs<T> w;
    DCP_TRY(w.reserve(h, N, F));
    DCP_TRY(nmf_residual<T>(h, Y, mask, X, D, N, F, K, w.tmp, w.part, w.blocks));
    DCP_TRY(w.sum(h, out));
    *out = sqrt(*out);
    return DCP_OK;
}

template <class T>
int nmf_grads_api(dcp_handle* h, const T* Y, const T* mask, T* X, const T* D, int64_t N, int64_t F,
                  int64_t K, int lik, int n_x_updates, T* grad_pos, T* grad_neg) {
    DCP_TRY(check_nmf_args(h, Y, X, D, N, F, K, lik));
    if (!grad_pos || !grad_neg) return fail(h, DCP_ERR_INVALID, "null gradient pointer");
    if (n_x_updates < 0) return fail(h, DCP_ERR_INVALID, "negative update count");
    DCP_HIP_OK(h, hipSetDevice(h->device));
    const bool masked = mask != nullptr;
    const bool gram = (lik == DCP_LIK_L2 && !masked);
    NmfShape<T> s{N, F, K, lik, masked};
    const int64_t W = nmf_stats_width(F, K, lik, masked);
    NmfStatsWs<T> ws;
    T* stats = nullptr;
    DCP_TRY(ws_lay_out(h, [&](WsLayout& a) {
        nmf_stats_layout(a, ws, s, masked);
        a.take(stats, (size_t)K * W);
    }));
    const T* Ypre = nullptr;
    DCP_TRY(nmf_premask<T>(h, Y, mask, N, F, ws.Ym, &Ypre));
    for (int i = 0; i < n_x_updates; ++i)
        DCP_TRY(nmf_stats<T>(h, Ypre, mask, X, X, D, s, stats, ws, 1));
    DCP_TRY(nmf_stats<T>(h, Ypre, mask, X, X, D, s, stats, ws, 2));
    DCP_HIP_OK(h, hipMemcpy2DAsync(grad_pos, sizeof(T) * F, stats, sizeof(T) * W, sizeof(T) * F, K,
                                   hipMemcpyDeviceToDevice, h->stream));
    if (gram) {
        GemmArgs<T> a;
        a.A = stats + F; a.lda = W; a.B = D; a.ldb = F; a.M = (int)K; a.N = (int)F; a.K = (int)K;
        a.tile = TILE_SMALL;
        DCP_LAUNCH_OK(h, (gemm<FORM_NN>(h->stream, a, EpiStore<T>{grad_neg, (long)F})));
    } else {
        DCP_HIP_OK(h, hipMemcpy2DAsync(grad_neg, sizeof(T) * F, stats + F, sizeof(T) * W,
                                       sizeof(T) * F, K, hipMemcpyDeviceToDevice, h->stream));
    }
    return DCP_OK;
}

template <class T>
int nmf_grad_x_api(dcp_handle* h, const T* Y, const T* mask, const T* X, const T* D, int64_t N, int64_t F,
                   int64_t K, int lik, T* grad_pos, T* grad_neg) {
    DCP_TRY(check_nmf_args(h, Y, X, D, N, F, K, lik));
    if (!grad_pos || !grad_neg) return fail(h, DCP_ERR_INVALID, "null gradient pointer");
    DCP_HIP_OK(h, hipSetDevice(h->device));
    const bool masked = mask != nullptr;
    NmfShape<T> s{N, F, K, lik, masked};
    NmfStatsWs<T> ws;
    DCP_TRY(ws_lay_out(h, [&](WsLayout& a) { nmf_stats_layout(a, ws, s, masked); }));
    const T* Ypre = nullptr;
    DCP_TRY(nmf_premask<T>(h, Y, mask, N, F, ws.Ym, &Ypre));
    return nmf_grad_x<T>(h, Ypre, mask, X, D, s, grad_pos, grad_neg, ws);
}

template <class T>
int nmf_gauss_logp_api(dcp_handle* h, const T* Y, const T* mask, const T* X, const T* D, int64_t N,
                       int64_t F, int64_t K, double scale, double* out) {
    DCP_TRY(check_nmf_args(h, Y, X, D, N, F, K, DCP_LIK_L2));
    if (!out) return fail(h, DCP_ERR_INVALID, "out is null");
    DCP_HIP_OK(h, hipSetDevice(h->device));
    NmfScalarWs<T> w;
    DCP_TRY(w.reserve(h, N, F));
    GemmArgs<T> a;
    a.A = X; a.lda = K; a.B = D; a.ldb = F; a.M = (int)N; a.N = (int)F; a.K = (int)K;
    DCP_LAUNCH_OK(h, (gemm<FORM_NN>(h->stream, a, EpiResidual<T>{Y, F, nullptr, 0, w.tmp, F})));
    hipLaunchKernelGGL((reduce_partial_kernel<SumOp, MapGaussLogp<T>, double>), dim3(w.blocks), dim3(256), 0, h->stream,
                       MapGaussLogp<T>{w.tmp, mask, 1.0 / scale, log(scale) + 3.14159265358979323846 * 0.5},
                       (long)N * F, w.part);
// ... 229 lines not shown
```

### decomp_amd/csrc/nmf_hals.hip

```cpp
#include <cmath>

#include "comm.hpp"
#include "nmf_hals.hpp"
#include "nmf_loop.hpp"

using namespace dcp;

namespace {

int sweep_rc(dcp_handle* h, hipError_t e) {
    if (e != hipSuccess) return fail(h, DCP_ERR_HIP, std::string("launch failed: ") + hipGetErrorString(e));
    return DCP_OK;
}

template <class T>
int hals_x_side(dcp_handle* h, const T* Y, const T* Xc, T* Xn, const T* Dc, const NmfShape<T>& s, T* stats,
                NmfStatsWs<T>& w, NmfPenalty pen) {
    hipStream_t st = h->stream;
    const int N = (int)s.N, F = (int)s.F, K = (int)s.K;
    {
        ProfScope ps(h, DCP_PROF_GRAM);
        GemmArgs<T> g;
        g.A = Dc; g.lda = F; g.B = Dc; g.ldb = F; g.M = K; g.N = K; g.K = F;
        if (!std::is_same<T, float>::value) g.tile = TILE_SMALL_DEEP;
        plan_splits<FORM_NT>(g, 512, kMaxSplits, 16);
        DCP_LAUNCH_OK(h, (gemm<FORM_NT>(st, g, EpiSlab<T>{w.slabs, K, (long)K * K})));
        if (pen.on())
            launch_reduce_slabs_affine<T>(st, w.slabs, (long)K * K, g.ksplits, (long)K * K, T(0), (long)K, T(pen.l2),
                                          w.G);
        else
            launch_reduce_slabs_scalar<T>(st, w.slabs, (long)K * K, g.ksplits, (long)K * K, w.G);
        DCP_LAUNCH_OK(h, hipGetLastError());
    }
    {
        ProfScope ps(h, DCP_PROF_XUPDATE);
        GemmArgs<T> pg;
        pg.A = Y; pg.lda = F; pg.B = Dc; pg.ldb = F; pg.M = N; pg.N = K; pg.K = F;
        const int psplits = nmf_xupdate_splits<T>(s.N, s.F, s.K, pg);
        if (psplits <= 1) {
            pg.ksplits = 1;
            if (pen.on())
                DCP_LAUNCH_OK(h, (nmf_product<FORM_NT>(h, st, pg, EpiStoreSub<T>{w.Q, K, T(pen.l1)}, true)));
            else
                DCP_LAUNCH_OK(h, (nmf_product<FORM_NT>(h, st, pg, EpiStore<T>{w.Q, K}, true)));
        } else {
            if ((size_t)pg.ksplits * N * K > w.slab_count)
                return fail(h, DCP_ERR_INTERNAL, "hals Y.D^T slab plan mismatch");
            DCP_LAUNCH_OK(h, (nmf_product<FORM_NT>(h, st, pg, EpiSlab<T>{w.slabs, K, (long)N * K}, true)));
            if (pen.on())
                launch_reduce_slabs_affine<T>(st, w.slabs, (long)N * K, pg.ksplits, (long)N * K, T(pen.l1), 0L, T(0),
                                              w.Q);
            else
                launch_reduce_slabs<T>(st, w.slabs, (long)N * K, pg.ksplits, (long)N * K, w.Q);
            DCP_LAUNCH_OK(h, hipGetLastError());
        }
        DCP_TRY(sweep_rc(h, launch_nn_cd_sweep<T, false>(st, Xc, Xn, K, w.Q, K, w.G, K, N, K)));
    }
    return nmf_stats<T>(h, Y, nullptr, Xn, Xn, Dc, s, stats, w, 2);
}

template <class T>
int hals_impute(dcp_handle* h, const T* Y, const T* mask, const T* Xc, const T* Dc, int64_t N, int64_t F, int64_t K,
                T* Yi) {
    ProfScope ps(h, DCP_PROF_FWD);
    GemmArgs<T> a;
    a.A = Xc; a.lda = (int)K; a.B = Dc; a.ldb = (int)F; a.M = (int)N; a.N = (int)F; a.K = (int)K;
    DCP_LAUNCH_OK(h, (gemm<FORM_NN>(h->stream, a, EpiImpute<T>{Y, mask, Yi, (long)F})));
    return DCP_OK;
}

template <class T>
int hals_d_sweep(dcp_handle* h, const T* Dc, T* U, int64_t F, int64_t K, const T* stats) {
    ProfScope ps(h, DCP_PROF_DUPDATE);
    const long W = (long)(F + K);
    return sweep_rc(h, launch_nn_cd_sweep<T, true>(h->stream, Dc, U, (long)F, stats, W, stats + F, W, (int)F,
                                                   (int)K));
}

template <class T>
int hals_normalize_rescale(dcp_handle* h, const T* U, const T* Dc, T* Dn, T* X, int64_t N, int64_t F, int64_t K,
                           T* nrm, T* maxdiff_dev, T* maxdiff_next, unsigned int* ticket, T* host_out) {
    ProfScope ps(h, DCP_PROF_DNORM);
    hipLaunchKernelGGL((hals_normalize_kernel<T>), dim3((unsigned)K), dim3(256), 0, h->stream, U, (long)F, Dc, Dn,
                       nrm, maxdiff_dev, maxdiff_next, ticket, host_out);
    DCP_LAUNCH_OK(h, hipGetLastError());
    hipLaunchKernelGGL((hals_rescale_kernel<T>), dim3(grid_for((long)N * K)), dim3(256), 0, h->stream, X,
                       (long)N * K, (int)K, (const T*)nrm);
    DCP_LAUNCH_OK(h, hipGetLastError());
    return DCP_OK;
}

template <class T>
struct HalsStep {
    const T* Y;
    NmfShape<T> s;
    NmfPenalty pen;
    bool sharded;
    const T* mask = nullptr;
    T* Yi = nullptr;
    NmfStatsWs<T> ws;
    T* stats = nullptr;
    T* U = nullptr;
    T* nrm = nullptr;

    void layout(WsLayout& a) {
        nmf_stats_layout(a, ws, s, false);
        a.take(stats, (size_t)s.K * (s.F + s.K));
        a.take(U, (size_t)s.K * s.F);
        a.take(nrm, (size_t)s.K);
        if (mask) a.take(Yi, (size_t)s.N * s.F);
    }
    int prepare(dcp_handle*) { return DCP_OK; }
    int iterate(dcp_handle* h, const T* Xc, T* Xn, const T* Dc, T* Dn, const NmfStopSlots<T>& slots) {
        const T* Yd = Y;
        if (mask) {
            DCP_TRY(hals_impute<T>(h, Y, mask, Xc, Dc, s.N, s.F, s.K, Yi));
            Yd = Yi;
        }
        DCP_TRY(hals_x_side<T>(h, Yd, Xc, Xn, Dc, s, stats, ws, pen));
        if (sharded) {
            ProfScope ps(h, DCP_PROF_EXCHANGE);
            DCP_TRY(comm_allreduce_sum(h, stats, (size_t)s.K * (s.F + s.K),
                                       std::is_same<T, float>::value ? COMM_F32 : COMM_F64));
        }
        DCP_TRY(hals_d_sweep<T>(h, Dc, U, s.F, s.K, stats));
        return hals_normalize_rescale<T>(h, U, Dc, Dn, Xn, s.N, s.F, s.K, nrm, slots.md, slots.md_next, slots.ticket,
                                         slots.host);
    }
};

template <class T>
int nmf_hals_solve(dcp_handle* h, const T* Y, T* X, T* D, int64_t N, int64_t F, int64_t K, T tol, int maxiter,
                   int* it_out, T* last_maxdiff, T* resid_trace, bool sharded = false, const T* mask = nullptr) {
    DCP_TRY(check_nmf_dims(h, Y, X, D, N, F, K));
    if (!it_out) return fail(h, DCP_ERR_INVALID, "it_out is null");
    if (sharded && !comm_active(h))
        return fail(h, DCP_ERR_COMM, mask ? "dcp_nmf_emhals_sharded_* needs a communicator (dcp_comm_init)"
                                          : "dcp_nmf_hals_sharded_* needs a communicator (dcp_comm_init)");
    DCP_HIP_OK(h, hipSetDevice(h->device));
    HalsStep<T> step{Y, NmfShape<T>{N, F, K, DCP_LIK_L2, false}, nmf_penalty(h), sharded, mask};
    return nmf_lagged_loop<T>(h, step, Y, mask, X, D, N, F, K, tol, maxiter, it_out, last_maxdiff, resid_trace);
}

template <class T>
int nmf_impute_api(dcp_handle* h, const T* Y, const T* mask, const T* X, const T* D, int64_t N, int64_t F, int64_t K,
                   T* Y_out) {
    DCP_TRY(check_nmf_dims(h, Y, X, D, N, F, K));
    if (!mask || !Y_out) return fail(h, DCP_ERR_INVALID, "mask / Y_out is null");
    DCP_HIP_OK(h, hipSetDevice(h->device));
    return hals_impute<T>(h, Y, mask, X, D, N, F, K, Y_out);
}

template <class T>
int nmf_hals_stats_api(dcp_handle* h, const T* Y, const T* X, T* X_out, const T* D, int64_t N, int64_t F, int64_t K,
                       T* stats) {
    DCP_TRY(check_nmf_dims(h, Y, X, D, N, F, K));
    if (!stats || !X_out) return fail(h, DCP_ERR_INVALID, "stats / X_out is null");
    DCP_HIP_OK(h, hipSetDevice(h->device));
    NmfShape<T> s{N, F, K, DCP_LIK_L2, false};
    NmfStatsWs<T> ws;
    DCP_TRY(ws_lay_out(h, [&](WsLayout& a) { nmf_stats_layout(a, ws, s, false); }));
    return hals_x_side<T>(h, Y, X, X_out, D, s, stats, ws, nmf_penalty(h));
}

template <class T>
int nmf_hals_update_api(dcp_handle* h, const T* stats, const T* D, T* D_new, T* X, int64_t N, int64_t F,
                        int64_t K, T* maxdiff_dev, T* maxdiff_next) {
    if (h && (!D_new || !maxdiff_dev)) return fail(h, DCP_ERR_INVALID, "null pointer");
    DCP_TRY(check_nmf_dims(h, stats, D, X, N, F, K, "null pointer"));
    DCP_HIP_OK(h, hipSetDevice(h->device));
    T* U = nullptr;
    T* nrm = nullptr;
    DCP_TRY(ws_lay_out(h, [&](WsLayout& a) {
        a.take(U, (size_t)K * F);
        a.take(nrm, (size_t)K);
    }));
    DCP_TRY(hals_d_sweep<T>(h, D, U, F, K, stats));
    if (!maxdiff_next) DCP_HIP_OK(h, hipMemsetAsync(maxdiff_dev, 0, sizeof(T), h->stream));
    return hals_normalize_rescale<T>(h, U, D, D_new, X, N, F, K, nrm, maxdiff_dev, maxdiff_next, nullptr, nullptr);
}

template <class T>
int nn_cd_sweep_api(dcp_handle* h, const T* V_in, T* V_out, const T* C, const T* G, int64_t R, int64_t K,
                    int coord_major) {
    if (!h) return DCP_ERR_INVALID;
    if (!V_in || !V_out || !C || !G) return fail(h, DCP_ERR_INVALID, "null array pointer");
    if (R <= 0 || K <= 0) return fail(h, DCP_ERR_INVALID, "sizes must be positive");
    if (R > 0x7fffffffLL || K > 0x7fffffffLL) return fail(h, DCP_ERR_INVALID, "dimension exceeds 2^31-1");
    DCP_HIP_OK(h, hipSetDevice(h->device));
    if (coord_major)
        return sweep_rc(h, launch_nn_cd_sweep<T, true>(h->stream, V_in, V_out, (long)R, C, (long)R, G, (long)K,
                                                          (int)R, (int)K));
    return sweep_rc(h, launch_nn_cd_sweep<T, false>(h->stream, V_in, V_out, (long)K, C, (long)K, G, (long)K,
                                                       (int)R, (int)K));
}

}

extern "C" {

int dcp_nmf_hals_f32(dcp_handle* h, const float* Y, float* X, float* D, int64_t N, int64_t F, int64_t K, float tol,
                     int maxiter, int* it_out, float* last_maxdiff, float* resid_trace) {
    return nmf_hals_solve<float>(h, Y, X, D, N, F, K, tol, maxiter, it_out, last_maxdiff, resid_trace);
}
int dcp_nmf_hals_f64(dcp_handle* h, const double* Y, double* X, double* D, int64_t N, int64_t F, int64_t K,
                     double tol, int maxiter, int* it_out, double* last_maxdiff, double* resid_trace) {
    return nmf_hals_solve<double>(h, Y, X, D, N, F, K, tol, maxiter, it_out, last_maxdiff, resid_trace);
}
int dcp_nmf_hals_sharded_f32(dcp_handle* h, const float* Y, float* X, float* D, int64_t N, int64_t F, int64_t K,
                             float tol, int maxiter, int* it_out, float* last_maxdiff) {
    return nmf_hals_solve<float>(h, Y, X, D, N, F, K, tol, maxiter, it_out, last_maxdiff, nullptr, true);
}
int dcp_nmf_hals_sharded_f64(dcp_handle* h, const double* Y, double* X, double* D, int64_t N, int64_t F, int64_t K,
                             double tol, int maxiter, int* it_out, double* last_maxdiff) {
    return nmf_hals_solve<double>(h, Y, X, D, N, F, K, tol, maxiter, it_out, last_maxdiff, nullptr, true);
}
int dcp_nmf_impute_f32(dcp_handle* h, const float* Y, const float* mask, const float* X, const float* D, int64_t N,
                       int64_t F, int64_t K, float* Y_out) {
    return nmf_impute_api<float>(h, Y, mask, X, D, N, F, K, Y_out);
}
int dcp_nmf_impute_f64(dcp_handle* h, const double* Y, const double* mask, const double* X, const double* D,
                       int64_t N, int64_t F, int64_t K, double* Y_out) {
    return nmf_impute_api<double>(h, Y, mask, X, D, N, F, K, Y_out);
}
int dcp_nmf_emhals_f32(dcp_handle* h, const float* Y, const float* mask, float* X, float* D, int64_t N, int64_t F,
                       int64_t K, float tol, int maxiter, int* it_out, float* last_maxdiff, float* resid_trace) {
    return nmf_hals_solve<float>(h, Y, X, D, N, F, K, tol, maxiter, it_out, last_maxdiff, resid_trace, false, mask);
}
int dcp_nmf_emhals_f64(dcp_handle* h, const double* Y, const double* mask, double* X, double* D, int64_t N,
                       int64_t F, int64_t K, double tol, int maxiter, int* it_out, double* last_maxdiff,
                       double* resid_trace) {
    return nmf_hals_solve<double>(h, Y, X, D, N, F, K, tol, maxiter, it_out, last_maxdiff, resid_trace, false, mask);
}
int dcp_nmf_emhals_sharded_f32(dcp_handle* h, const float* Y, const float* mask, float* X, float* D, int64_t N,
                               int64_t F, int64_t K, float tol, int maxiter, int* it_out, float* last_maxdiff) {
    return nmf_hals_solve<float>(h, Y, X, D, N, F, K, tol, maxiter, it_out, last_maxdiff, nullptr, true, mask);
}
int dcp_nmf_emhals_sharded_f64(dcp_handle* h, const double* Y, const double* mask, double* X, double* D, int64_t N,
                               int64_t F, int64_t K, double tol, int maxiter, int* it_out, double* last_maxdiff) {
    return nmf_hals_solve<double>(h, Y, X, D, N, F, K, tol, maxiter, it_out, last_maxdiff, nullptr, true, mask);
}
int dcp_nmf_hals_stats_f32(dcp_handle* h, const float* Y, const float* X, float* X_out, const float* D, int64_t N,
                           int64_t F, int64_t K, float* stats) {
    return nmf_hals_stats_api<float>(h, Y, X, X_out, D, N, F, K, stats);
}
int dcp_nmf_hals_stats_f64(dcp_handle* h, const double* Y, const double* X, double* X_out, const double* D,
                           int64_t N, int64_t F, int64_t K, double* stats) {
    return nmf_hals_stats_api<double>(h, Y, X, X_out, D, N, F, K, stats);
}
int dcp_nmf_hals_update_f32(dcp_handle* h, const float* stats, const float* D, float* D_new, float* X, int64_t N,
                            int64_t F, int64_t K, float* maxdiff_dev, float* maxdiff_next) {
    return nmf_hals_update_api<float>(h, stats, D, D_new, X, N, F, K, maxdiff_dev, maxdiff_next);
}
int dcp_nmf_hals_update_f64(dcp_handle* h, const double* stats, const double* D, double* D_new, double* X,
                            int64_t N, int64_t F, int64_t K, double* maxdiff_dev, double* maxdiff_next) {
    return nmf_hals_update_api<double>(h, stats, D, D_new, X, N, F, K, maxdiff_dev, maxdiff_next);
}
int dcp_nn_cd_sweep_f32(dcp_handle* h, const float* V_in, float* V_out, const float* C, const float* G, int64_t R,
                        int64_t K, int coord_major) {
    return nn_cd_sweep_api<float>(h, V_in, V_out, C, G, R, K, coord_major);
}
int dcp_nn_cd_sweep_f64(dcp_handle* h, const double* V_in, double* V_out, const double* C, const double* G,
                        int64_t R, int64_t K, int coord_major) {
    return nn_cd_sweep_api<double>(h, V_in, V_out, C, G, R, K, coord_major);
// ... 4 lines not shown
```

### decomp_amd/csrc/nmf_impl.hpp

```cpp
#pragma once
#include <math.h>

#include "gemm.hpp"
#include "handle.hpp"
#include "kernels_small.hpp"

namespace dcp {

inline int64_t nmf_stats_width(int64_t F, int64_t K, int likelihood, bool masked) {
    return (likelihood == DCP_LIK_L2 && !masked) ? (F + K) : 2 * F;
}

constexpr int kSplitTarget = 1024;
constexpr int kMaxSplits = 64;

struct NmfPenalty {
    double l1 = 0.0, l2 = 0.0;
    bool on() const { return l1 != 0.0 || l2 != 0.0; }
};
inline NmfPenalty nmf_penalty(const dcp_handle* h) { return NmfPenalty{h->nmf_l1, h->nmf_l2}; }

template <class T>
struct NmfShape {
    int64_t N, F, K;
    int lik;
    bool masked;
};

inline int check_nmf_dims(dcp_handle* h, const void* a, const void* b, const void* c, int64_t N, int64_t F, int64_t K,
                          const char* null_msg = "null array pointer") {
    if (!h) return DCP_ERR_INVALID;
    if (!a || !b || !c) return fail(h, DCP_ERR_INVALID, null_msg);
    if (N <= 0 || F <= 0 || K <= 0) return fail(h, DCP_ERR_INVALID, "sizes must be positive");
    if (N > 0x7fffffffLL || F > 0x7fffffffLL || K > 0x7fffffffLL || F + K > 0x3fffffffLL)
        return fail(h, DCP_ERR_INVALID, "dimension exceeds 2^31-1");
    return DCP_OK;
}

template <class T>
struct NmfStatsWs {
    T* Q = nullptr;
    T* G = nullptr;
    T* f = nullptr;
    T* f2 = nullptr;
    T* Ym = nullptr;
    T* slabs = nullptr;
    T* vecK = nullptr;
    T* part = nullptr;
    size_t slab_count = 0;
    const uint32_t* mbits = nullptr;
};

template <class T>
inline int nmf_xupdate_splits(int64_t N, int64_t F, int64_t K, GemmArgs<T>& pg) {
    pg.M = (int)N; pg.N = (int)K; pg.K = (int)F;
    pg.tile = TILE_AUTO;
    int bm = 64, bn = 64;
    if (std::is_same<T, float>::value) {
        GemmArgs<T> planned = pg;
        planned.split_planned = true;
        const GemmRoute r = gemm_route<FORM_NT>(planned);
        bm = r.plan_bm; bn = r.plan_bn;
    }
    const long tiles = (long)ceil_div(N, bm) * ceil_div(K, bn);
    const long enough = (bm == 256) ? 192 : 512;
    if (tiles >= enough || F < 1024) {
        pg.ksplits = 1;
        return 1;
    }
    plan_splits<FORM_NT>(pg, (bm == 256) ? 256 : 1024, 8);
    return pg.ksplits;
}

template <class T>
inline size_t nmf_slab_elems(const NmfShape<T>& s) {
    const int64_t W = nmf_stats_width(s.F, s.K, s.lik, s.masked);
    GemmArgs<T> a;
    a.M = (int)s.K; a.N = (int)W; a.K = (int)s.N;
    plan_splits<FORM_TN>(a, kSplitTarget, kMaxSplits);
    size_t stats_slabs = (size_t)a.ksplits * s.K * W;
    if (s.lik == DCP_LIK_L2 && !s.masked) {
        GemmArgs<T> b;
        b.M = (int)s.K; b.N = (int)W; b.K = (int)s.N;
        if (plan_splits_x6_tn(b, (int)s.F, kMaxSplits) && (size_t)b.ksplits * s.K * W > stats_slabs)
            stats_slabs = (size_t)b.ksplits * s.K * W;
    }
    GemmArgs<T> g;
    g.M = (int)s.K; g.N = (int)s.K; g.K = (int)s.F;
    plan_splits<FORM_NT>(g, 512, kMaxSplits, 16);
    size_t g_slabs = (size_t)g.ksplits * s.K * s.K;
    GemmArgs<T> pg;
    const int ps = nmf_xupdate_splits<T>(s.N, s.F, s.K, pg);
    size_t x_slabs = ps > 1 ? (size_t)ps * s.N * s.K : 0;
    if (ps > 1 && ((s.masked && s.lik == DCP_LIK_L2) || s.lik == DCP_LIK_BETA)) {
        GemmArgs<T> sg;
        const int ss = nmf_xupdate_splits<T>(2 * s.N, s.F, s.K, sg);
        const size_t st_slabs = (size_t)(ss > 1 ? ss : 1) * 2 * s.N * s.K;
        if (st_slabs > x_slabs) x_slabs = st_slabs;
    }
    size_t m = stats_slabs > g_slabs ? stats_slabs : g_slabs;
    return m > x_slabs ? m : x_slabs;
}

template <class T>
inline void nmf_stats_layout(WsLayout& a, NmfStatsWs<T>& w, const NmfShape<T>& s, bool need_ym) {
    const bool gram = (s.lik == DCP_LIK_L2 && !s.masked);
    a.take(w.Q, (size_t)s.N * s.K);
    if (gram) a.take(w.G, (size_t)s.K * s.K);
    if (!gram) a.take(w.f, (size_t)s.N * s.F);
    if (s.lik == DCP_LIK_BETA) a.take(w.f2, (size_t)s.N * s.F);
    if (need_ym) a.take(w.Ym, (size_t)s.N * s.F);
    w.slab_count = nmf_slab_elems(s);
    a.take(w.slabs, w.slab_count);
    a.take(w.vecK, (size_t)s.K);
    a.take(w.part, (size_t)64 * (s.K > s.F ? s.K : s.F));
}

template <class T>
struct NmfUpdateWs {
    T* U = nullptr;
    T* rowmax = nullptr;
};
template <class T>
inline void nmf_update_layout(WsLayout& a, NmfUpdateWs<T>& w, int64_t F, int64_t K) {
    a.take(w.U, (size_t)K * F);
    a.take(w.rowmax, (size_t)K);
}

template <class T>
inline int column_sums(dcp_handle* h, const T* a, long ld, long rows, long cols, T* part, T* out) {
    const int stripes = rows >= 64 ? 64 : (rows > 0 ? (int)rows : 1);
    const long rows_per = (rows + stripes - 1) / stripes;
    dim3 grid(grid_for(cols, 64), stripes);
    hipLaunchKernelGGL((colsum_partial_kernel<T>), grid, dim3(256), 0, h->stream, a, ld, rows,
                       cols, rows_per, part);
    DCP_LAUNCH_OK(h, hipGetLastError());
    launch_reduce_slabs_scalar<T>(h->stream, part, cols, stripes, cols, out, 64);
    DCP_LAUNCH_OK(h, hipGetLastError());
    return DCP_OK;
}

template <int FORM, class T, class Epi>
inline hipError_t nmf_product(dcp_handle* h, hipStream_t st, const GemmArgs<T>& a, const Epi& epi, bool split_ok) {
    if constexpr (std::is_same<T, float>::value) {
        if (split_ok && h->f32_product_mode == 0 && x6_tier<FORM>(a) != X6_NONE && x6_epi_ok(epi))
            return gemm_bf16x6<FORM>(st, a, epi);
    }
    return gemm<FORM>(st, a, epi);
}

template <class T>
inline int nmf_stats(dcp_handle* h, const T* Ypre, const T* mask, const T* Xin, T* Xout, const T* D,
                     const NmfShape<T>& s, T* stats, NmfStatsWs<T>& w, int phases = 3,
                     NmfPenalty pen = NmfPenalty()) {
    hipStream_t st = h->stream;
    const int N = (int)s.N, F = (int)s.F, K = (int)s.K;
    const bool gram = (s.lik == DCP_LIK_L2 && !s.masked);
    const int W = (int)nmf_stats_width(s.F, s.K, s.lik, s.masked);
    const double beta = h->nmf_beta;
    const T l1 = T(pen.l1), l2 = T(pen.l2);

    auto forward = [&](const T* X) -> int {
        ProfScope ps(h, DCP_PROF_FWD);
        GemmArgs<T> fa;
        fa.A = X; fa.lda = K; fa.B = D; fa.ldb = F; fa.M = N; fa.N = F; fa.K = K;
        if (s.lik == DCP_LIK_BETA) {
            DCP_LAUNCH_OK(h, (gemm<FORM_NN>(st, fa, EpiBetaParts<T>{Ypre, F, mask, F, beta_mode(beta), T(beta - 2.0),
                                                                     w.f, w.f2, F})));
        } else if (s.lik == DCP_LIK_L2) {
            if constexpr (std::is_same<T, float>::value) {
                if (w.mbits != nullptr) {
                    DCP_LAUNCH_OK(h, (gemm<FORM_NN>(st, fa, EpiMulMaskBits{w.mbits, (long)F, w.f, (long)F})));
                    return DCP_OK;
                }
            }
            DCP_LAUNCH_OK(h, (gemm<FORM_NN>(st, fa, EpiMulMask<T>{mask, F, w.f, F})));
        } else
            DCP_LAUNCH_OK(h, (gemm<FORM_NN>(st, fa, EpiKlRatio<T>{Ypre, F, nullptr, 0, w.f, F})));
        return DCP_OK;
    };

    auto stacked_xupdate = [&](const T* a_neg, const T* a_pos, bool& done) -> int {
        done = false;
        if constexpr (std::is_same<T, float>::value) {
            GemmArgs<T> probe;
            const bool split_single = nmf_xupdate_splits<T>(s.N, s.F, s.K, probe) > 1;
            if (split_single && (N % 256) == 0 && (F % 16) == 0) {
                ProfScope ps(h, DCP_PROF_XUPDATE);
                GemmArgs<T> sg;
                nmf_xupdate_splits<T>(2 * s.N, s.F, s.K, sg);
                sg.A = a_neg; sg.lda = F; sg.A2 = a_pos; sg.lda2 = F; sg.m_a1 = N;
                sg.B = D; sg.ldb = F;
                if (sg.ksplits < 1) sg.ksplits = 1;
                if ((size_t)sg.ksplits * 2 * N * K > w.slab_count)
                    return fail(h, DCP_ERR_INTERNAL, "nmf stacked x-update slab plan mismatch");
                DCP_LAUNCH_OK(h, (gemm<FORM_NT>(st, sg, EpiSlab<T>{w.slabs, K, (long)2 * N * K})));
                if (pen.on())
                    hipLaunchKernelGGL((mu_quotient_stacked_kernel<T, true>), dim3(grid_for((long)N * K)), dim3(256),
                                       0, st, Xin, (const T*)w.slabs, (long)2 * N * K, sg.ksplits, (long)N * K, l1,
                                       l2, Xout);
                else
                    hipLaunchKernelGGL((mu_quotient_stacked_kernel<T, false>), dim3(grid_for((long)N * K)), dim3(256),
                                       0, st, Xin, (const T*)w.slabs, (long)2 * N * K, sg.ksplits, (long)N * K, l1,
                                       l2, Xout);
                DCP_LAUNCH_OK(h, hipGetLastError());
                done = true;
            }
        }
        return DCP_OK;
    };

    const T* X = Xin;
    bool x_done = false;
    if (phases & 1) {
    const T* xnum_A = Ypre;
    const T* xden = w.Q;
    long ld_xden = K;
    GemmArgs<T> pg_probe;
    const bool split_gram = gram && std::is_same<T, float>::value && Xout != Xin &&
                            nmf_xupdate_splits<T>(s.N, s.F, s.K, pg_probe) > 1;
    bool fused_den = false;
    if constexpr (std::is_same<T, float>::value) {
        if (gram && h->f32_product_mode == 0 && Xout != Xin) {
            GemmArgs<T> fg;
            fg.A = Ypre; fg.lda = F; fg.B = D; fg.ldb = F;
            fused_den = nmf_xupdate_splits<T>(s.N, s.F, s.K, fg) <= 1 && x6_tier<FORM_NT>(fg) == X6_HUGE &&
                        EpiMuGramDen<false>{Xin, K, w.G, K, K, Xout, K}.vec_ok();
        }
    }
    if (gram) {
        {
            ProfScope ps(h, DCP_PROF_GRAM);
            GemmArgs<T> g;
            g.A = D; g.lda = F; g.B = D; g.ldb = F; g.M = K; g.N = K; g.K = F;
            if (!std::is_same<T, float>::value) g.tile = TILE_SMALL_DEEP;
            plan_splits<FORM_NT>(g, 512, kMaxSplits, 16);
            DCP_LAUNCH_OK(h, (gemm<FORM_NT>(st, g, EpiSlab<T>{w.slabs, K, (long)K * K})));
            launch_reduce_slabs_scalar<T>(st, w.slabs, (long)K * K, g.ksplits, (long)K * K, w.G);
            DCP_LAUNCH_OK(h, hipGetLastError());
        }
        if (!split_gram && !fused_den) {
            ProfScope ps(h, DCP_PROF_XNEG);
            GemmArgs<T> q;
            q.A = Xin; q.lda = K; q.B = w.G; q.ldb = K; q.M = N; q.N = K; q.K = K;
            DCP_LAUNCH_OK(h, (gemm<FORM_NN>(st, q, EpiStore<T>{w.Q, K})));
        }
    } else if (s.lik == DCP_LIK_L2) {
        DCP_TRY(forward(Xin));
        DCP_TRY(stacked_xupdate(w.f, Ypre, x_done));
        if (!x_done) {
            ProfScope ps(h, DCP_PROF_XNEG);
            GemmArgs<T> q;
            q.A = w.f; q.lda = F; q.B = D; q.ldb = F; q.M = N; q.N = K; q.K = F;
            DCP_LAUNCH_OK(h, (gemm<FORM_NT>(st, q, EpiStore<T>{w.Q, K})));
        }
    } else if (s.lik == DCP_LIK_BETA) {
        DCP_TRY(forward(Xin));
        xnum_A = w.f;
        DCP_TRY(stacked_xupdate(w.f2, w.f, x_done));
        if (!x_done) {
            ProfScope ps(h, DCP_PROF_XNEG);
            GemmArgs<T> q;
            q.A = w.f2; q.lda = F; q.B = D; q.ldb = F; q.M = N; q.N = K; q.K = F;
            DCP_LAUNCH_OK(h, (gemm<FORM_NT>(st, q, EpiStore<T>{w.Q, K})));
        }
    } else {
        DCP_TRY(forward(Xin));
        xnum_A = w.f;
        ProfScope ps(h, DCP_PROF_XNEG);
        if (!s.masked) {
            hipLaunchKernelGGL((rowsum_kernel<T>), dim3(K), dim3(256), 0, st, D, (long)F, (long)F,
                               w.vecK);
            DCP_LAUNCH_OK(h, hipGetLastError());
            xden = w.vecK;
            ld_xden = 0;
        } else {
            GemmArgs<T> q;
            q.A = mask; q.lda = F; q.B = D; q.ldb = F; q.M = N; q.N = K; q.K = F;
            DCP_LAUNCH_OK(h, (gemm<FORM_NT>(st, q, EpiStore<T>{w.Q, K})));
        }
    }
    if (!x_done) {
        ProfScope ps(h, DCP_PROF_XUPDATE);
        GemmArgs<T> pg;
        pg.A = xnum_A; pg.lda = F; pg.B = D; pg.ldb = F; pg.M = N; pg.N = K; pg.K = F;
        const int psplits = nmf_xupdate_splits<T>(s.N, s.F, s.K, pg);
        if (fused_den) {
            if constexpr (std::is_same<T, float>::value) {
                const GemmProblem fp = fill_problem<FORM_NT>(pg);
                if (pen.on())
                    DCP_LAUNCH_OK(h, (launch_gemm_bf16x6<X6Huge, KMAJOR, KMAJOR>(
                                         st, fp, EpiMuGramDen<true>{Xin, K, w.G, K, K, Xout, K, l1, l2})));
                else
                    DCP_LAUNCH_OK(h, (launch_gemm_bf16x6<X6Huge, KMAJOR, KMAJOR>(
                                         st, fp, EpiMuGramDen<false>{Xin, K, w.G, K, K, Xout, K})));
            }
        } else if (psplits <= 1) {
            pg.ksplits = 1;
            const EpiMuNum<T> num{Xin, K, xden, ld_xden, Xout, K};
            if (pen.on())
                DCP_LAUNCH_OK(h, (nmf_product<FORM_NT>(h, st, pg, EpiMuNumPen<T>{num, l1, l2}, gram)));
            else
                DCP_LAUNCH_OK(h, (nmf_product<FORM_NT>(h, st, pg, num, gram)));
        } else {
            if ((size_t)pg.ksplits * N * K > w.slab_count)
                return fail(h, DCP_ERR_INTERNAL, "nmf x-update slab plan mismatch");
            DCP_LAUNCH_OK(h, (nmf_product<FORM_NT>(h, st, pg, EpiSlab<T>{w.slabs, K, (long)N * K}, gram)));
            if (split_gram) {
                GemmArgs<T> q;
                q.A = Xin; q.lda = K; q.B = w.G; q.ldb = K; q.M = N; q.N = K; q.K = K;
                if (pen.on())
                    DCP_LAUNCH_OK(h, (gemm<FORM_NN>(st, q, EpiMuDenSlabs<T, true>{Xin, K, w.slabs, K, (long)N * K,
                                                                                   pg.ksplits, Xout, K, l1, l2})));
                else
                    DCP_LAUNCH_OK(h, (gemm<FORM_NN>(st, q, EpiMuDenSlabs<T, false>{Xin, K, w.slabs, K, (long)N * K,
                                                                                    pg.ksplits, Xout, K})));
            } else {
                if (pen.on())
                    hipLaunchKernelGGL((mu_quotient_slabs_kernel<T, true>), dim3(grid_for((long)N * K)), dim3(256),
                                       0, st, Xin, (const T*)w.slabs, (long)N * K, pg.ksplits, xden,
                                       (long)ld_xden, (long)N, (long)K, l1, l2, Xout);
                else
                    hipLaunchKernelGGL((mu_quotient_slabs_kernel<T, false>), dim3(grid_for((long)N * K)), dim3(256),
                                       0, st, Xin, (const T*)w.slabs, (long)N * K, pg.ksplits, xden,
                                       (long)ld_xden, (long)N, (long)K, l1, l2, Xout);
                DCP_LAUNCH_OK(h, hipGetLastError());
            }
        }
    }
    X = Xout;
    }
    if (!(phases & 2)) return DCP_OK;

    GemmArgs<T> sa;
    sa.A = X; sa.lda = K; sa.M = K; sa.N = W; sa.K = N;
    if (gram) {
        sa.B = Ypre; sa.ldb = F; sa.B2 = X; sa.ldb2 = K; sa.n_b1 = F;
    } else if (s.lik == DCP_LIK_L2) {
        DCP_TRY(forward(X));
        sa.B = Ypre; sa.ldb = F; sa.B2 = w.f; sa.ldb2 = F; sa.n_b1 = F;
    } else if (s.lik == DCP_LIK_BETA) {
        DCP_TRY(forward(X));
        sa.B = w.f; sa.ldb = F; sa.B2 = w.f2; sa.ldb2 = F; sa.n_b1 = F;
    } else {
        DCP_TRY(forward(X));
        if (s.masked) {
            sa.B = w.f; sa.ldb = F; sa.B2 = mask; sa.ldb2 = F; sa.n_b1 = F;
        } else {
            sa.B = w.f; sa.ldb = F; sa.N = F;
        }
    }
    const int Wg = sa.N;
    const bool x6_allowed = std::is_same<T, float>::value && h->f32_product_mode == 0;
    if (!(gram && x6_allowed && plan_splits_x6_tn(sa, sa.n_b1, kMaxSplits)))
        plan_splits<FORM_TN>(sa, kSplitTarget, kMaxSplits);
    if ((size_t)sa.ksplits * K * Wg > w.slab_count)
        return fail(h, DCP_ERR_INTERNAL, "nmf slab plan mismatch");
    {
        ProfScope ps(h, DCP_PROF_STATS);
        DCP_LAUNCH_OK(h, (nmf_product<FORM_TN>(h, st, sa, EpiSlab<T>{w.slabs, Wg, (long)K * Wg}, gram)));
    }
    ProfScope ps(h, DCP_PROF_STATS_SUM);
    if (Wg == W) {
        launch_reduce_slabs<T>(st, w.slabs, (long)K * W, sa.ksplits, (long)K * W, stats);
        DCP_LAUNCH_OK(h, hipGetLastError());
    } else {
        hipLaunchKernelGGL((reduce_slabs_rows_kernel<T>), dim3(grid_for((long)K * F)), dim3(256), 0,
                           st, w.slabs, (long)K * F, sa.ksplits, (long)K, (long)F, stats, (long)W);
        DCP_LAUNCH_OK(h, hipGetLastError());
        DCP_TRY(column_sums<T>(h, X, K, N, K, w.part, w.vecK));
        hipLaunchKernelGGL((bcast_rows_kernel<T>), dim3(grid_for((long)K * F)), dim3(256), 0, st,
                           w.vecK, (long)K, (long)F, stats + F, (long)W);
        DCP_LAUNCH_OK(h, hipGetLastError());
    }
    return DCP_OK;
}

template <class T>
inline int nmf_grad_x(dcp_handle* h, const T* Ypre, const T* mask, const T* X, const T* D,
                      const NmfShape<T>& s, T* pos, T* neg, NmfStatsWs<T>& w) {
    hipStream_t st = h->stream;
    const int N = (int)s.N, F = (int)s.F, K = (int)s.K;
    const bool gram = (s.lik == DCP_LIK_L2 && !s.masked);
    const T* pos_A = Ypre;
    if (gram) {
        GemmArgs<T> g;
        g.A = D; g.lda = F; g.B = D; g.ldb = F; g.M = K; g.N = K; g.K = F;
        plan_splits<FORM_NT>(g, 512, kMaxSplits, 16);
        DCP_LAUNCH_OK(h, (gemm<FORM_NT>(st, g, EpiSlab<T>{w.slabs, K, (long)K * K})));
        launch_reduce_slabs_scalar<T>(st, w.slabs, (long)K * K, g.ksplits, (long)K * K, w.G);
        DCP_LAUNCH_OK(h, hipGetLastError());
        GemmArgs<T> q;
        q.A = X; q.lda = K; q.B = w.G; q.ldb = K; q.M = N; q.N = K; q.K = K;
        DCP_LAUNCH_OK(h, (gemm<FORM_NN>(st, q, EpiStore<T>{neg, K})));
    } else {
        GemmArgs<T> fa;
        fa.A = X; fa.lda = K; fa.B = D; fa.ldb = F; fa.M = N; fa.N = F; fa.K = K;
        if (s.lik == DCP_LIK_BETA) {
            const double beta = h->nmf_beta;
            DCP_LAUNCH_OK(h, (gemm<FORM_NN>(st, fa, EpiBetaParts<T>{Ypre, F, mask, F, beta_mode(beta), T(beta - 2.0),
                                                                     w.f, w.f2, F})));
            GemmArgs<T> q;
            q.A = w.f2; q.lda = F; q.B = D; q.ldb = F; q.M = N; q.N = K; q.K = F;
            DCP_LAUNCH_OK(h, (gemm<FORM_NT>(st, q, EpiStore<T>{neg, K})));
            pos_A = w.f;
        } else if (s.lik == DCP_LIK_L2) {
            DCP_LAUNCH_OK(h, (gemm<FORM_NN>(st, fa, EpiMulMask<T>{mask, F, w.f, F})));
            GemmArgs<T> q;
            q.A = w.f; q.lda = F; q.B = D; q.ldb = F; q.M = N; q.N = K; q.K = F;
            DCP_LAUNCH_OK(h, (gemm<FORM_NT>(st, q, EpiStore<T>{neg, K})));
        } else {
            DCP_LAUNCH_OK(h, (gemm<FORM_NN>(st, fa, EpiKlRatio<T>{Ypre, F, nullptr, 0, w.f, F})));
            pos_A = w.f;
            if (!s.masked) {
                hipLaunchKernelGGL((rowsum_kernel<T>), dim3(K), dim3(256), 0, st, D, (long)F, (long)F, w.vecK);
                DCP_LAUNCH_OK(h, hipGetLastError());
                hipLaunchKernelGGL((bcast_cols_kernel<T>), dim3(grid_for((long)N * K)), dim3(256), 0, st,
                                   (const T*)w.vecK, (long)N, (long)K, neg);
                DCP_LAUNCH_OK(h, hipGetLastError());
            } else {
                GemmArgs<T> q;
                q.A = mask; q.lda = F; q.B = D; q.ldb = F; q.M = N; q.N = K; q.K = F;
                DCP_LAUNCH_OK(h, (gemm<FORM_NT>(st, q, EpiStore<T>{neg, K})));
            }
        }
    }
    GemmArgs<T> pg;
    pg.A = pos_A; pg.lda = F; pg.B = D; pg.ldb = F; pg.M = N; pg.N = K; pg.K = F;
    DCP_LAUNCH_OK(h, (gemm<FORM_NT>(st, pg, EpiStore<T>{pos, K})));
    return DCP_OK;
}

template <class T>
inline int nmf_update(dcp_handle* h, const T* stats, const T* D, T* D_new, int64_t F64, int64_t K64,
                      int lik, bool masked, T* maxdiff_dev, NmfUpdateWs<T>& w,
                      T* maxdiff_next = nullptr, unsigned int* ticket = nullptr, T* host_out = nullptr) {
    hipStream_t st = h->stream;
    const int F = (int)F64, K = (int)K64;
    const bool gram = (lik == DCP_LIK_L2 && !masked);
    const int W = (int)nmf_stats_width(F64, K64, lik, masked);
    {
        ProfScope ps(h, DCP_PROF_DUPDATE);
        if (gram) {
            GemmArgs<T> a;
            a.A = stats + F; a.lda = W; a.B = D; a.ldb = F; a.M = K; a.N = F; a.K = K;
            if (std::is_same<T, float>::value) a.tile = (K % 64 == 0) ? TILE_SMALL_DEEP : TILE_SMALL;
            else a.tile = TILE_AUTO;
            DCP_LAUNCH_OK(h, (gemm<FORM_NN>(st, a, EpiMuDen<T>{D, F, stats, W, w.U, F})));
        } else {
            hipLaunchKernelGGL((mu_quotient_kernel<T>), dim3(grid_for((long)K * F)), dim3(256), 0,
                               st, D, (long)F, stats, (long)W, stats + F, (long)W, 0, (long)K,
                               (long)F, w.U, (long)F);
            DCP_LAUNCH_OK(h, hipGetLastError());
        }
    }
    ProfScope ps(h, DCP_PROF_DNORM);
    if (maxdiff_next != nullptr) {
        hipLaunchKernelGGL((row_normalize_kernel<T>), dim3(K), dim3(256), 0, st, w.U, (long)F,
                           (long)F, 1, D, (long)F, D_new, (long)F, (T*)nullptr, (T*)nullptr,
                           maxdiff_dev, maxdiff_next, ticket, host_out);
        DCP_LAUNCH_OK(h, hipGetLastError());
        return DCP_OK;
    }
    hipLaunchKernelGGL((row_normalize_kernel<T>), dim3(K), dim3(256), 0, st, w.U, (long)F, (long)F,
                       1, D, (long)F, D_new, (long)F, w.rowmax, (T*)nullptr, (T*)nullptr,
                       (T*)nullptr);
    DCP_LAUNCH_OK(h, hipGetLastError());
    launch_final_max<T>(st, w.rowmax, (long)K, maxdiff_dev);
    DCP_LAUNCH_OK(h, hipGetLastError());
    return DCP_OK;
}

template <class T>
inline int nmf_residual(dcp_handle* h, const T* Y, const T* mask, const T* X, const T* D, int64_t N,
                        int64_t F, int64_t K, T* tmpNF, double* partial_dev, int nblocks) {
    GemmArgs<T> a;
    a.A = X; a.lda = K; a.B = D; a.ldb = F; a.M = (int)N; a.N = (int)F; a.K = (int)K;
    DCP_LAUNCH_OK(h, (gemm<FORM_NN>(h->stream, a, EpiResidual<T>{Y, F, mask, F, tmpNF, F})));
    hipLaunchKernelGGL((reduce_partial_kernel<SumOp, MapAbs2<T>, double>), dim3(nblocks), dim3(256), 0, h->stream,
                       MapAbs2<T>{tmpNF}, (long)N * F, partial_dev);
    DCP_LAUNCH_OK(h, hipGetLastError());
    return DCP_OK;
}

template <class T>
inline int nmf_beta_divergence(dcp_handle* h, const T* Y, const T* mask, const T* X, const T* D, int64_t N,
                               int64_t F, int64_t K, double beta, T* tmpNF, double* partial_dev, int nblocks) {
    GemmArgs<T> a;
    a.A = X; a.lda = K; a.B = D; a.ldb = F; a.M = (int)N; a.N = (int)F; a.K = (int)K;
    DCP_LAUNCH_OK(h, (gemm<FORM_NN>(h->stream, a, EpiBetaDivergence<T>{Y, F, mask, F, beta, tmpNF, F})));
    hipLaunchKernelGGL((reduce_partial_kernel<SumOp, MapValue<T>, double>), dim3(nblocks), dim3(256), 0, h->stream,
                       MapValue<T>{tmpNF}, (long)N * F, partial_dev);
    DCP_LAUNCH_OK(h, hipGetLastError());
    return DCP_OK;
}

}

namespace dcp {

template <class T>
inline int nmf_premask(dcp_handle* h, const T* Y, const T* mask, int64_t N, int64_t F, T* Ym, const T** Ypre) {
    *Ypre = Y;
    if (mask == nullptr) return DCP_OK;
    hipLaunchKernelGGL((mul_mask_kernel<T>), dim3(grid_for(N * F)), dim3(256), 0, h->stream, Y, mask,
                       (long)N, (long)F, (long)F, Ym);
    DCP_LAUNCH_OK(h, hipGetLastError());
    *Ypre = Ym;
    return DCP_OK;
}

template <class T>
inline int nmf_mask_prepare(dcp_handle* h, const T* Y, const T* mask, int64_t N, int64_t F, T* Ym,
                            uint32_t* bits, int* flag_dev, int* binary) {
    const T* Ypre = nullptr;
    DCP_TRY(nmf_premask<T>(h, Y, mask, N, F, Ym, &Ypre));
    *binary = 0;
    if (!std::is_same<T, float>::value || bits == nullptr) return DCP_OK;
    DCP_HIP_OK(h, hipMemsetAsync(flag_dev, 0, sizeof(int), h->stream));
    hipLaunchKernelGGL((mask_rowbits_kernel<T>), dim3(grid_for(((N + 31) / 32) * F)), dim3(256), 0,
                       h->stream, mask, (long)N, (long)F, bits, flag_dev);
    DCP_LAUNCH_OK(h, hipGetLastError());
    int not_binary = 0;
    DCP_TRY(read_scalar(h, (const int*)flag_dev, &not_binary));
    *binary = (not_binary == 0) ? 1 : 0;
    return DCP_OK;
}

inline size_t mask_bits_words(int64_t N, int64_t F) { return (size_t)((N + 31) / 32) * (size_t)F; }

}
```

### decomp_amd/csrc/nmf_loop.hpp

```cpp
#pragma once
#include "nmf_impl.hpp"

namespace dcp {

template <class T>
struct NmfStopSlots {
    T* md;
    T* md_next;
    unsigned int* ticket;
    T* host;
};

template <class T, class Step>
int nmf_lagged_loop(dcp_handle* h, Step& step, const T* Y, const T* mask, T* X, T* D, int64_t N, int64_t F, int64_t K,
                    T tol, int maxiter, int* it_out, T* last_maxdiff, T* resid_trace) {
    const bool want_resid = resid_trace != nullptr;
    const int resid_blocks = 1024;
    T* D2 = nullptr;
    T* X2 = nullptr;
    T* maxdiff_dev = nullptr;
    unsigned int* ticket = nullptr;
    T* resid_tmp = nullptr;
    double* resid_part = nullptr;
    DCP_TRY(ws_lay_out(h, [&](WsLayout& a) {
        step.layout(a);
        a.take(D2, (size_t)K * F);
        a.take(X2, (size_t)N * K);
        a.take(maxdiff_dev, 2);
        a.take(ticket, 4);
        if (want_resid) {
            a.take(resid_tmp, (size_t)N * F);
            a.take(resid_part, resid_blocks);
        }
    }));
    void* hostv = nullptr;
    DCP_TRY(host_scratch(h, sizeof(double) * (resid_blocks + 4), &hostv));
    T* host_md = reinterpret_cast<T*>(hostv);
    double* host_part = reinterpret_cast<double*>(hostv) + 2;

    DCP_TRY(step.prepare(h));
    DCP_HIP_OK(h, hipMemsetAsync(maxdiff_dev, 0, 2 * sizeof(T), h->stream));
    DCP_HIP_OK(h, hipMemsetAsync(ticket, 0, 4 * sizeof(unsigned int), h->stream));

    T* Xc = X;  T* Xn = X2;
    T* Dc = D;  T* Dn = D2;
    int result_it = maxiter;
    T md_last = T(0);
    bool converged = false;
    for (int it = 1; it < maxiter; ++it) {
        const int slot = it & 1;
        *reinterpret_cast<volatile T*>(host_md + slot) = T(-1);
        DCP_TRY(step.iterate(h, Xc, Xn, Dc, Dn,
                             NmfStopSlots<T>{maxdiff_dev + slot, maxdiff_dev + (slot ^ 1), ticket, host_md + slot}));
        if (want_resid) {
            double acc = 0.0;
            DCP_TRY(nmf_residual<T>(h, Y, mask, Xn, Dn, N, F, K, resid_tmp, resid_part, resid_blocks));
            DCP_TRY(read_partial_sum(h, resid_part, resid_blocks, host_part, &acc));
            resid_trace[it - 1] = (T)sqrt(acc);
        }
        if (it > 1) {
            DCP_TRY(wait_pinned_word(h, host_md + (slot ^ 1), T(-1), &md_last));
            if (md_last < tol) {
                result_it = it - 1;
                converged = true;
                break;
            }
        }
        T* t = Xc; Xc = Xn; Xn = t;
        t = Dc; Dc = Dn; Dn = t;
    }
    if (!converged && maxiter > 1) {
        const int slot = (maxiter - 1) & 1;
        DCP_TRY(wait_pinned_word(h, host_md + slot, T(-1), &md_last));
        if (md_last < tol) result_it = maxiter - 1;
    }
    DCP_HIP_OK(h, hipStreamSynchronize(h->stream));
    if (Xc != X)
        DCP_HIP_OK(h, hipMemcpyAsync(X, Xc, sizeof(T) * (size_t)N * K, hipMemcpyDeviceToDevice, h->stream));
    if (Dc != D)
        DCP_HIP_OK(h, hipMemcpyAsync(D, Dc, sizeof(T) * (size_t)K * F, hipMemcpyDeviceToDevice, h->stream));
    DCP_HIP_OK(h, hipStreamSynchronize(h->stream));
    *it_out = result_it;
    if (last_maxdiff) *last_maxdiff = md_last;
    return DCP_OK;
}

}
```

### decomp_amd/csrc/util.hip

```cpp
#include "comm.hpp"
#include "gemm.hpp"
#include "handle.hpp"
#include "kernels_small.hpp"
#include <new>

#define DCP_STR2(x) #x
#define DCP_STR(x) DCP_STR2(x)

using namespace dcp;

namespace {

template <class T>
int l2_normalize_api(dcp_handle* h, T* U, int64_t K, int64_t F, int strict) {
    if (!h) return DCP_ERR_INVALID;
    if (!U) return fail(h, DCP_ERR_INVALID, "null array pointer");
    if (K < 0 || F < 0) return fail(h, DCP_ERR_INVALID, "negative size");
    if (K == 0 || F == 0) return DCP_OK;
    DCP_HIP_OK(h, hipSetDevice(h->device));
    hipLaunchKernelGGL((row_normalize_kernel<T>), dim3((unsigned)K), dim3(256), 0, h->stream,
                       (const T*)U, (long)F, (long)F, strict, (const T*)nullptr, 0L, U, (long)F,
                       (real_t<T>*)nullptr);
    DCP_HIP_OK(h, hipGetLastError());
    return DCP_OK;
// ... 405 lines not shown

int dcp_destroy(dcp_handle* h) {
    if (!h) return DCP_OK;
    (void)hipSetDevice(h->device);
    comm_release(h);
    if (h->arena) {
        (void)hipStreamSynchronize(h->stream);
        (void)hipFree(h->arena);
    }
    if (h->host_pinned) (void)hipHostFree(h->host_pinned);
    for (auto& r : h->prof_recs) {
        (void)hipEventDestroy(r.a);
        (void)hipEventDestroy(r.b);
    }
    for (auto e : h->prof_pool) (void)hipEventDestroy(e);
    if (h->stream_switch) (void)hipEventDestroy(h->stream_switch);
    if (h->side) {
        (void)hipStreamSynchronize(h->side);
        (void)hipStreamDestroy(h->side);
    }
    if (h->ev_main) (void)hipEventDestroy(h->ev_main);
    if (h->ev_side) (void)hipEventDestroy(h->ev_side);
    delete h;
    return DCP_OK;
}

int dcp_set_stream(dcp_handle* h, void* hip_stream) {
    if (!h) return DCP_ERR_INVALID;
    h->stream = reinterpret_cast<hipStream_t>(hip_stream);
    return DCP_OK;
}

int dcp_profile_enable(dcp_handle* h, int on) {
    if (!h) return DCP_ERR_INVALID;
    h->prof_on = on != 0;
    return DCP_OK;
}

int dcp_profile_select(dcp_handle* h, unsigned label_mask) {
    if (!h) return DCP_ERR_INVALID;
    h->prof_mask = label_mask;
    return DCP_OK;
}

static int prof_fold(dcp_handle* h) {
    if (h->prof_recs.empty()) return DCP_OK;
    DCP_HIP_OK(h, hipSetDevice(h->device));
    DCP_HIP_OK(h, hipStreamSynchronize(h->stream));
    for (auto& r : h->prof_recs) {
        float ms = 0.0f;
        if (hipEventElapsedTime(&ms, r.a, r.b) == hipSuccess && r.label >= 0 &&
            r.label < DCP_PROF_NLABELS) {
            h->prof_ms[r.label] += ms;
            h->prof_cnt[r.label] += 1;
        }
        h->prof_pool.push_back(r.a);
        h->prof_pool.push_back(r.b);
    }
    h->prof_recs.clear();
    return DCP_OK;
}

int dcp_profile_reset(dcp_handle* h) {
    if (!h) return DCP_ERR_INVALID;
    DCP_TRY(prof_fold(h));
    for (int i = 0; i < DCP_PROF_NLABELS; ++i) {
        h->prof_ms[i] = 0.0;
        h->prof_cnt[i] = 0;
    }
    return DCP_OK;
}

int dcp_profile_read(dcp_handle* h, int label, double* total_ms, int64_t* count) {
    if (!h) return DCP_ERR_INVALID;
    if (label < 0 || label >= DCP_PROF_NLABELS || !total_ms || !count)
        return fail(h, DCP_ERR_INVALID, "bad profile label or null output");
    DCP_TRY(prof_fold(h));
    *total_ms = h->prof_ms[label];
    *count = h->prof_cnt[label];
    return DCP_OK;
}

const char* dcp_profile_label_name(int label) {
    static const char* names[DCP_PROF_NLABELS] = {"gram",  "x_neg",     "x_update", "forward", "stats",
                                                  "stats_sum", "d_update", "d_norm",  "misc", "exchange"};
    return (label >= 0 && label < DCP_PROF_NLABELS) ? names[label] : "?";
}

const char* dcp_last_error_string(dcp_handle* h) { return h ? h->err.c_str() : "null handle"; }

const char* dcp_build_info(void) {
    return "libdecomp_hip: gfx950, fp32 MFMA 32x32x2 + fp64 MFMA 16x16x4 GEMM cores, HIP " DCP_STR(HIP_VERSION_MAJOR) "." DCP_STR(HIP_VERSION_MINOR);
}

int dcp_l2_normalize_f32(dcp_handle* h, float* U, int64_t K, int64_t F, int strict) {
    return l2_normalize_api<float>(h, U, K, F, strict);
}
int dcp_l2_normalize_f64(dcp_handle* h, double* U, int64_t K, int64_t F, int strict) {
    return l2_normalize_api<double>(h, U, K, F, strict);
}
int dcp_l2_normalize_c64(dcp_handle* h, void* U, int64_t K, int64_t F, int strict) {
    return l2_normalize_api<c64>(h, reinterpret_cast<c64*>(U), K, F, strict);
}
int dcp_l2_normalize_c128(dcp_handle* h, void* U, int64_t K, int64_t F, int strict) {
    return l2_normalize_api<c128>(h, reinterpret_cast<c128*>(U), K, F, strict);
}
int dcp_count_negative_f32(dcp_handle* h, const float* x, int64_t n, int64_t* count) {
    return count_negative_api<float>(h, x, n, count);
}
int dcp_count_negative_f64(dcp_handle* h, const double* x, int64_t n, int64_t* count) {
    return count_negative_api<double>(h, x, n, count);
}
int dcp_gemm_f32(dcp_handle* h, int form, const float* A, const float* B, float* C, int64_t M,
                 int64_t N, int64_t K, int ksplits, int tile) {
    return gemm_api<float>(h, form, A, B, C, M, N, K, ksplits, tile);
}
int dcp_gemm_bf16x6_f32(dcp_handle* h, int form, const float* A, const float* B, float* C, int64_t M, int64_t N,
                        int64_t K, int ksplits) {
    if (!h) return DCP_ERR_INVALID;
    if (!A || !B || !C) return fail(h, DCP_ERR_INVALID, "null array pointer");
    if (M <= 0 || N <= 0 || K <= 0 || M > INT32_MAX || N > INT32_MAX || K > INT32_MAX)
        return fail(h, DCP_ERR_INVALID, "bad sizes");
    if (form != FORM_NT && form != FORM_TN) return fail(h, DCP_ERR_INVALID, "bf16x6: form must be 0 (NT) or 2 (TN)");
    DCP_HIP_OK(h, hipSetDevice(h->device));
    GemmArgs<float> a;
    a.A = A; a.B = B; a.M = (int)M; a.N = (int)N; a.K = (int)K;
    a.lda = (form == FORM_TN) ? M : K;
    a.ldb = (form == FORM_NT) ? K : N;
    float* slabs = nullptr;
    if (ksplits > 1) {
        const long kblocks = (K + 15) / 16;
        const long s = ksplits > kblocks ? kblocks : ksplits;
        a.klen = (int)(((kblocks + s - 1) / s) * 16);
        a.ksplits = (int)((K + a.klen - 1) / a.klen);
        a.split_planned = true;
        DCP_TRY(ws_lay_out(h, [&](WsLayout& w) { w.take(slabs, (size_t)a.ksplits * M * N); }));
    }
    const bool ok = (form == FORM_NT) ? x6_tier<FORM_NT>(a) != X6_NONE : x6_tier<FORM_TN>(a) != X6_NONE;
    if (!ok) return fail(h, DCP_ERR_INVALID, "bf16x6: no split-bf16 kernel for this shape (tiles, alignment)");
    hipError_t e;
    if (slabs) {
        EpiSlab<float> epi{slabs, (long)N, (long)M * N};
        e = (form == FORM_NT) ? gemm_bf16x6<FORM_NT>(h->stream, a, epi) : gemm_bf16x6<FORM_TN>(h->stream, a, epi);
        if (e != hipSuccess) return fail(h, DCP_ERR_HIP, hipGetErrorString(e));
        launch_reduce_slabs_scalar<float>(h->stream, slabs, (long)(M * N), a.ksplits, (long)(M * N), C);
        DCP_HIP_OK(h, hipGetLastError());
    } else {
        EpiStore<float> epi{C, (long)N};
        e = (form == FORM_NT) ? gemm_bf16x6<FORM_NT>(h->stream, a, epi) : gemm_bf16x6<FORM_TN>(h->stream, a, epi);
        if (e != hipSuccess) return fail(h, DCP_ERR_HIP, hipGetErrorString(e));
    }
    return DCP_OK;
}
int dcp_set_f32_product_mode(dcp_handle* h, int mode) {
    if (!h) return DCP_ERR_INVALID;
    const int prev = h->f32_product_mode;
    if (mode > 1) return fail(h, DCP_ERR_INVALID, "f32 product mode must be 0 (bf16x6) or 1 (fp32)");
    if (mode >= 0) h->f32_product_mode = mode;
    return prev;
}
int dcp_gemm_f64(dcp_handle* h, int form, const double* A, const double* B, double* C, int64_t M,
                 int64_t N, int64_t K, int ksplits, int tile) {
    return gemm_api<double>(h, form, A, B, C, M, N, K, ksplits, tile);
}
int dcp_gemm_c64(dcp_handle* h, int form, const void* A, const void* B, void* C, int64_t M, int64_t N,
                 int64_t K, int ksplits, int tile) {
    return gemm_api<c64>(h, form, reinterpret_cast<const c64*>(A), reinterpret_cast<const c64*>(B),
                         reinterpret_cast<c64*>(C), M, N, K, ksplits, tile);
}
int dcp_gemm_c128(dcp_handle* h, int form, const void* A, const void* B, void* C, int64_t M, int64_t N,
                  int64_t K, int ksplits, int tile) {
    return gemm_api<c128>(h, form, reinterpret_cast<const c128*>(A), reinterpret_cast<const c128*>(B),
                          reinterpret_cast<c128*>(C), M, N, K, ksplits, tile);
}

int dcp_dict_prefetch_rows_bytes(dcp_handle* h, const void* in, const int64_t* index, int64_t rows,
                                 int64_t row_bytes, void* out) {
    if (!h) return DCP_ERR_INVALID;
    if (rows < 0 || row_bytes < 0) return dcp::fail(h, DCP_ERR_INVALID, "negative size");
    if (rows > 0 && row_bytes > 0 && (!in || !index || !out)) return dcp::fail(h, DCP_ERR_INVALID, "null pointer");
    h->pf_in = in;
    h->pf_index = index;
    h->pf_out = out;
    h->pf_rows = rows;
    h->pf_row_bytes = row_bytes;
    return DCP_OK;
}

int dcp_gather_rows_bytes(dcp_handle* h, const void* in, const int64_t* index, int64_t rows,
                          int64_t row_bytes, void* out) {
    if (h && !index) return dcp::fail(h, DCP_ERR_INVALID, "null index");
    return move_rows(h, in, index, out, nullptr, rows, row_bytes);
}

int dcp_scatter_rows_bytes(dcp_handle* h, const void* in, const int64_t* index, int64_t rows,
                           int64_t row_bytes, void* out) {
    if (h && !index) return dcp::fail(h, DCP_ERR_INVALID, "null index");
    return move_rows(h, in, nullptr, out, index, rows, row_bytes);
}

int dcp_dict_set_pcd_order(dcp_handle* h, const int32_t* order, int64_t rows, int64_t K) {
    if (!h) return DCP_ERR_INVALID;
    if (order != nullptr && (rows <= 0 || K <= 0)) return dcp::fail(h, DCP_ERR_INVALID, "bad table shape");
    h->pcd_order = order;
    h->pcd_rows = order ? rows : 0;
    h->pcd_K = order ? K : 0;
    return DCP_OK;
}

}
```

### include/decomp_hip.h

```cpp
#ifndef DECOMP_HIP_H
#define DECOMP_HIP_H

#include <stdint.h>

#ifdef __cplusplus
extern "C" {
#endif

typedef struct dcp_handle dcp_handle;

enum {
    DCP_OK = 0,
    DCP_ERR_INVALID = -1,
    DCP_ERR_HIP = -2,
    DCP_ERR_NOMEM = -3,
    DCP_ERR_INTERNAL = -4,
    DCP_ERR_UNSUPPORTED = -5,
    DCP_ERR_REF_TYPEERROR = -6,
    DCP_ERR_COMM = -7
};

enum { DCP_LIK_L2 = 0, DCP_LIK_KL = 1, DCP_LIK_BETA = 2 };

enum { DCP_LASSO_ISTA = 0, DCP_LASSO_ACC_ISTA = 1, DCP_LASSO_FISTA = 2, DCP_LASSO_CD = 3,
       DCP_LASSO_PARALLEL_CD = 4, DCP_LASSO_ADMM = 5 };
enum { DCP_LASSO_OMP = 6 };
enum { DCP_LASSO_POSITIVE = 0x100 };

int dcp_create(dcp_handle** out, int device);
int dcp_destroy(dcp_handle* h);
int dcp_set_stream(dcp_handle* h, void* hip_stream);
const char* dcp_last_error_string(dcp_handle* h);
const char* dcp_build_info(void);

enum { DCP_COMM_ID_BYTES = 128 };
typedef int (*dcp_allreduce_fn)(void* buf, int64_t count, int dtype, void* hip_stream, void* user);
int dcp_comm_set_external(dcp_handle* h, dcp_allreduce_fn fn, void* user, int rank, int world);
int dcp_memcpy(dcp_handle* h, void* dst, const void* src, int64_t bytes);
int dcp_comm_unique_id(void* id_out, int64_t id_bytes);
int dcp_comm_init(dcp_handle* h, const void* unique_id, int rank, int world);
int dcp_comm_destroy(dcp_handle* h);
int dcp_comm_info(dcp_handle* h, int* rank, int* world);
int dcp_comm_allreduce_sum_f32(dcp_handle* h, float* buf, int64_t count);
int dcp_comm_allreduce_sum_f64(dcp_handle* h, double* buf, int64_t count);

enum {
    DCP_PROF_GRAM = 0,
    DCP_PROF_XNEG = 1,
    DCP_PROF_XUPDATE = 2,
    DCP_PROF_FWD = 3,
    DCP_PROF_STATS = 4,
    DCP_PROF_STATS_SUM = 5,
    DCP_PROF_DUPDATE = 6,
    DCP_PROF_DNORM = 7,
    DCP_PROF_MISC = 8,
    DCP_PROF_EXCHANGE = 9,
    DCP_PROF_NLABELS = 10
};
int dcp_profile_enable(dcp_handle* h, int on);
int dcp_profile_select(dcp_handle* h, unsigned label_mask);
int dcp_profile_reset(dcp_handle* h);
int dcp_profile_read(dcp_handle* h, int label, double* total_ms, int64_t* count);
const char* dcp_profile_label_name(int label);

int dcp_l2_normalize_f32(dcp_handle* h, float* U, int64_t K, int64_t F, int strict);
int dcp_l2_normalize_f64(dcp_handle* h, double* U, int64_t K, int64_t F, int strict);
int dcp_l2_normalize_c64(dcp_handle* h, void* U, int64_t K, int64_t F, int strict);
int dcp_l2_normalize_c128(dcp_handle* h, void* U, int64_t K, int64_t F, int strict);

int dcp_count_negative_f32(dcp_handle* h, const float* x, int64_t n, int64_t* count);
int dcp_count_negative_f64(dcp_handle* h, const double* x, int64_t n, int64_t* count);

int dcp_gershgorin_f32(dcp_handle* h, const float* X, int64_t batch, int64_t n, float* out);
int dcp_gershgorin_f64(dcp_handle* h, const double* X, int64_t batch, int64_t n, double* out);
int dcp_gershgorin_c64(dcp_handle* h, const void* X, int64_t batch, int64_t n, float* out);
int dcp_gershgorin_c128(dcp_handle* h, const void* X, int64_t batch, int64_t n, double* out);

int dcp_inv_f32(dcp_handle* h, const float* X, int64_t batch, int64_t n, float* out);
int dcp_inv_f64(dcp_handle* h, const double* X, int64_t batch, int64_t n, double* out);
int dcp_inv_c64(dcp_handle* h, const void* X, int64_t batch, int64_t n, void* out);
int dcp_inv_c128(dcp_handle* h, const void* X, int64_t batch, int64_t n, void* out);

int dcp_gemm_f32(dcp_handle* h, int form, const float* A, const float* B, float* C,
                 int64_t M, int64_t N, int64_t K, int ksplits, int tile);
int dcp_gemm_f64(dcp_handle* h, int form, const double* A, const double* B, double* C,
                 int64_t M, int64_t N, int64_t K, int ksplits, int tile);
int dcp_gemm_c64(dcp_handle* h, int form, const void* A, const void* B, void* C,
                 int64_t M, int64_t N, int64_t K, int ksplits, int tile);
int dcp_gemm_c128(dcp_handle* h, int form, const void* A, const void* B, void* C,
                  int64_t M, int64_t N, int64_t K, int ksplits, int tile);

int dcp_gemm_bf16x6_f32(dcp_handle* h, int form, const float* A, const float* B, float* C,
                        int64_t M, int64_t N, int64_t K, int ksplits);

int dcp_set_f32_product_mode(dcp_handle* h, int mode);

int dcp_debug_tn_plain(int on);

int dcp_debug_gemm_route(int dtype, int form, int64_t M, int64_t N, int64_t K, int64_t n_b1, int tile, int flags,
                         int target_wgs, int max_splits, int min_blocks, int32_t* out);

int dcp_calib_read_f32(dcp_handle* h, const float* p, int64_t rows, int64_t cols, int pattern,
                       float* out);

int dcp_nmf_mu_f32(dcp_handle* h, const float* Y, const float* mask, float* X, float* D,
                   int64_t N, int64_t F, int64_t K, int likelihood, float tol, int maxiter,
                   int* it_out, float* last_maxdiff, float* resid_trace);
int dcp_nmf_mu_f64(dcp_handle* h, const double* Y, const double* mask, double* X, double* D,
                   int64_t N, int64_t F, int64_t K, int likelihood, double tol, int maxiter,
                   int* it_out, double* last_maxdiff, double* resid_trace);

int dcp_nmf_hals_f32(dcp_handle* h, const float* Y, float* X, float* D, int64_t N, int64_t F, int64_t K,
                     float tol, int maxiter, int* it_out, float* last_maxdiff, float* resid_trace);
int dcp_nmf_hals_f64(dcp_handle* h, const double* Y, double* X, double* D, int64_t N, int64_t F, int64_t K,
                     double tol, int maxiter, int* it_out, double* last_maxdiff, double* resid_trace);
int dcp_nmf_hals_sharded_f32(dcp_handle* h, const float* Y, float* X, float* D, int64_t N, int64_t F, int64_t K,
                             float tol, int maxiter, int* it_out, float* last_maxdiff);
int dcp_nmf_hals_sharded_f64(dcp_handle* h, const double* Y, double* X, double* D, int64_t N, int64_t F, int64_t K,
                             double tol, int maxiter, int* it_out, double* last_maxdiff);
int dcp_nmf_hals_stats_f32(dcp_handle* h, const float* Y, const float* X, float* X_out, const float* D, int64_t N,
                           int64_t F, int64_t K, float* stats);
int dcp_nmf_hals_stats_f64(dcp_handle* h, const double* Y, const double* X, double* X_out, const double* D,
                           int64_t N, int64_t F, int64_t K, double* stats);
int dcp_nmf_hals_update_f32(dcp_handle* h, const float* stats, const float* D, float* D_new, float* X, int64_t N,
                            int64_t F, int64_t K, float* maxdiff_dev, float* maxdiff_next);
int dcp_nmf_hals_update_f64(dcp_handle* h, const double* stats, const double* D, double* D_new, double* X,
                            int64_t N, int64_t F, int64_t K, double* maxdiff_dev, double* maxdiff_next);
int dcp_nmf_impute_f32(dcp_handle* h, const float* Y, const float* mask, const float* X, const float* D, int64_t N,
                       int64_t F, int64_t K, float* Y_out);
int dcp_nmf_impute_f64(dcp_handle* h, const double* Y, const double* mask, const double* X, const double* D,
                       int64_t N, int64_t F, int64_t K, double* Y_out);
int dcp_nmf_emhals_f32(dcp_handle* h, const float* Y, const float* mask, float* X, float* D, int64_t N, int64_t F,
                       int64_t K, float tol, int maxiter, int* it_out, float* last_maxdiff, float* resid_trace);
int dcp_nmf_emhals_f64(dcp_handle* h, const double* Y, const double* mask, double* X, double* D, int64_t N,
                       int64_t F, int64_t K, double tol, int maxiter, int* it_out, double* last_maxdiff,
                       double* resid_trace);
int dcp_nmf_emhals_sharded_f32(dcp_handle* h, const float* Y, const float* mask, float* X, float* D, int64_t N,
                               int64_t F, int64_t K, float tol, int maxiter, int* it_out, float* last_maxdiff);
int dcp_nmf_emhals_sharded_f64(dcp_handle* h, const double* Y, const double* mask, double* X, double* D, int64_t N,
                               int64_t F, int64_t K, double tol, int maxiter, int* it_out, double* last_maxdiff);
int dcp_nn_cd_sweep_f32(dcp_handle* h, const float* V_in, float* V_out, const float* C, const float* G,
                        int64_t R, int64_t K, int coord_major);
int dcp_nn_cd_sweep_f64(dcp_handle* h, const double* V_in, double* V_out, const double* C, const double* G,
                        int64_t R, int64_t K, int coord_major);

int dcp_nmf_mu_sharded_f32(dcp_handle* h, const float* Y, const float* mask, float* X, float* D,
                           int64_t N, int64_t F, int64_t K, int likelihood, float tol, int maxiter,
                           int* it_out, float* last_maxdiff);
int dcp_nmf_mu_sharded_f64(dcp_handle* h, const double* Y, const double* mask, double* X, double* D,
                           int64_t N, int64_t F, int64_t K, int likelihood, double tol, int maxiter,
                           int* it_out, double* last_maxdiff);

int64_t dcp_nmf_mu_stats_width(int64_t F, int64_t K, int likelihood, int masked);
int dcp_nmf_mu_stats_f32(dcp_handle* h, const float* Y, const float* mask, const float* X,
                         float* X_out, const float* D, int64_t N, int64_t F, int64_t K,
                         int likelihood, float* stats);
int dcp_nmf_mu_stats_f64(dcp_handle* h, const double* Y, const double* mask, const double* X,
                         double* X_out, const double* D, int64_t N, int64_t F, int64_t K,
                         int likelihood, double* stats);
int64_t dcp_nmf_mask_bits_words(int64_t N, int64_t F);
int dcp_nmf_mask_prepare_f32(dcp_handle* h, const float* Y, const float* mask, int64_t N, int64_t F,
                             float* Ym, uint32_t* bits, int* binary);
int dcp_nmf_mask_prepare_f64(dcp_handle* h, const double* Y, const double* mask, int64_t N, int64_t F,
                             double* Ym, uint32_t* bits, int* binary);
int dcp_nmf_mu_stats_prepared_f32(dcp_handle* h, const float* Ym, const float* mask, const uint32_t* bits,
                                  const float* X, float* X_out, const float* D, int64_t N, int64_t F,
                                  int64_t K, int likelihood, float* stats);
int dcp_nmf_mu_stats_prepared_f64(dcp_handle* h, const double* Ym, const double* mask, const uint32_t* bits,
                                  const double* X, double* X_out, const double* D, int64_t N, int64_t F,
                                  int64_t K, int likelihood, double* stats);
int dcp_nmf_mu_update_f32(dcp_handle* h, const float* stats, const float* D, float* D_new,
                          int64_t F, int64_t K, int likelihood, int masked,
                          float* maxdiff_dev, float* maxdiff_next);
int dcp_nmf_mu_update_f64(dcp_handle* h, const double* stats, const double* D, double* D_new,
                          int64_t F, int64_t K, int likelihood, int masked,
                          double* maxdiff_dev, double* maxdiff_next);

int dcp_nmf_grads_f32(dcp_handle* h, const float* Y, const float* mask, float* X, const float* D,
                      int64_t N, int64_t F, int64_t K, int likelihood, int n_x_updates,
                      float* grad_pos, float* grad_neg);
int dcp_nmf_grads_f64(dcp_handle* h, const double* Y, const double* mask, double* X, const double* D,
                      int64_t N, int64_t F, int64_t K, int likelihood, int n_x_updates,
                      double* grad_pos, double* grad_neg);
int dcp_nmf_grad_x_f32(dcp_handle* h, const float* Y, const float* mask, const float* X, const float* D,
                       int64_t N, int64_t F, int64_t K, int likelihood, float* grad_pos, float* grad_neg);
int dcp_nmf_grad_x_f64(dcp_handle* h, const double* Y, const double* mask, const double* X, const double* D,
                       int64_t N, int64_t F, int64_t K, int likelihood, double* grad_pos, double* grad_neg);
int dcp_nmf_gauss_logp_f32(dcp_handle* h, const float* Y, const float* mask, const float* X, const float* D,
                           int64_t N, int64_t F, int64_t K, double scale, double* out);
int dcp_nmf_gauss_logp_f64(dcp_handle* h, const double* Y, const double* mask, const double* X, const double* D,
                           int64_t N, int64_t F, int64_t K, double scale, double* out);
int dcp_set_nmf_beta(dcp_handle* h, double beta);
int dcp_set_nmf_penalty(dcp_handle* h, double l1, double l2);
int dcp_nmf_beta_divergence_f32(dcp_handle* h, const float* Y, const float* mask, const float* X, const float* D,
                                int64_t N, int64_t F, int64_t K, double* out);
int dcp_nmf_beta_divergence_f64(dcp_handle* h, const double* Y, const double* mask, const double* X,
                                const double* D, int64_t N, int64_t F, int64_t K, double* out);
int dcp_nmf_apply_f32(dcp_handle* h, const float* D, const float* P, const float* Q, double alpha,
                      float* D_new, int64_t K, int64_t F, double* maxdiff);
int dcp_nmf_apply_f64(dcp_handle* h, const double* D, const double* P, const double* Q, double alpha,
                      double* D_new, int64_t K, int64_t F, double* maxdiff);
int dcp_axpby_f32(dcp_handle* h, int64_t n, double a, const float* x, double b, float* y);
int dcp_axpby_f64(dcp_handle* h, int64_t n, double a, const double* x, double b, double* y);

int dcp_mu_quotient_f32(dcp_handle* h, const float* cur, const float* pos, const float* neg,
                        int64_t rows, int64_t cols, float* out);
int dcp_mu_quotient_f64(dcp_handle* h, const double* cur, const double* pos, const double* neg,
                        int64_t rows, int64_t cols, double* out);
int dcp_l2_normalize_diff_f32(dcp_handle* h, const float* U, const float* ref, float* out, int64_t K,
                              int64_t F, int strict, double* maxdiff);
int dcp_l2_normalize_diff_f64(dcp_handle* h, const double* U, const double* ref, double* out, int64_t K,
                              int64_t F, int strict, double* maxdiff);

int dcp_nmf_residual_f32(dcp_handle* h, const float* Y, const float* mask, const float* X,
                         const float* D, int64_t N, int64_t F, int64_t K, double* out);
int dcp_nmf_residual_f64(dcp_handle* h, const double* Y, const double* mask, const double* X,
                         const double* D, int64_t N, int64_t F, int64_t K, double* out);

int dcp_lasso_f32(dcp_handle* h, const float* Y, const float* mask, int mask_ndim, const float* A,
                  float* X, int64_t N, int64_t F, int64_t K, double alpha, double tol, int maxiter,
                  int method, int positive, int* it_out);
int dcp_lasso_f64(dcp_handle* h, const double* Y, const double* mask, int mask_ndim, const double* A,
                  double* X, int64_t N, int64_t F, int64_t K, double alpha, double tol, int maxiter,
                  int method, int positive, int* it_out);
int dcp_lasso_c64(dcp_handle* h, const void* Y, const float* mask, int mask_ndim, const void* A,
                  void* X, int64_t N, int64_t F, int64_t K, double alpha, double tol, int maxiter,
                  int method, int positive, int* it_out);
int dcp_lasso_c128(dcp_handle* h, const void* Y, const double* mask, int mask_ndim, const void* A,
                   void* X, int64_t N, int64_t F, int64_t K, double alpha, double tol, int maxiter,
                   int method, int positive, int* it_out);

int dcp_lasso_pcd_f32(dcp_handle* h, const float* Y, const float* mask, int mask_ndim, const float* A,
                      float* X, int64_t N, int64_t F, int64_t K, double alpha, double tol, int maxiter,
                      int positive, const int32_t* order, int64_t order_rows, int* it_out);
int dcp_lasso_pcd_f64(dcp_handle* h, const double* Y, const double* mask, int mask_ndim, const double* A,
                      double* X, int64_t N, int64_t F, int64_t K, double alpha, double tol, int maxiter,
                      int positive, const int32_t* order, int64_t order_rows, int* it_out);
int dcp_lasso_pcd_c64(dcp_handle* h, const void* Y, const float* mask, int mask_ndim, const void* A,
                      void* X, int64_t N, int64_t F, int64_t K, double alpha, double tol, int maxiter,
                      int positive, const int32_t* order, int64_t order_rows, int* it_out);
int dcp_lasso_pcd_c128(dcp_handle* h, const void* Y, const double* mask, int mask_ndim, const void* A,
                       void* X, int64_t N, int64_t F, int64_t K, double alpha, double tol, int maxiter,
                       int positive, const int32_t* order, int64_t order_rows, int* it_out);

int dcp_lasso_admm_f32(dcp_handle* h, const float* Y, const float* mask, int mask_ndim, const float* A,
                       float* X, int64_t N, int64_t F, int64_t K, double alpha, double tol, int maxiter,
                       int positive, double rho, int* it_out);
int dcp_lasso_admm_f64(dcp_handle* h, const double* Y, const double* mask, int mask_ndim, const double* A,
// ... 186 lines not shown
```

Before: 713.3 iterations/s.

## Feed bf16x6 GEMM from pre-split bf16 plane images of D in NMF MU

Adds a pre-split image format that stores the hi/mid/lo bf16 planes of an f32 operand in 16x16 blocks. The fused-denominator X-update GEMM in NMF MU can then load D (and optionally Y, in mode 2) as ready-made planes instead of splitting f32 values in every tile. The row-normalize kernel writes the D image directly when it emits D, so the split is done once per D update rather than per GEMM tile. This removes redundant split arithmetic in the GEMM main loop. In exchange it costs extra workspace, an image-building pass during prepare, and extra stores in the normalize kernel.

```diff
diff --git a/decomp_amd/_hip.py b/decomp_amd/_hip.py
--- a/decomp_amd/_hip.py
+++ b/decomp_amd/_hip.py
@@ -157,6 +157,9 @@
                                       _c_int, _c_vp]),
     'dcp_gemm_bf16x6_f32': (_c_int, [_c_vp, _c_int, _c_vp, _c_vp, _c_vp, _c_i64, _c_i64, _c_i64, _c_int]),
     'dcp_set_f32_product_mode': (_c_int, [_c_vp, _c_int]),
+    'dcp_set_x6_presplit': (_c_int, [_c_vp, _c_int]),
+    'dcp_x6_image_f32': (_c_int, [_c_vp, _c_vp, _c_i64, _c_i64, _c_vp]),
+    'dcp_gemm_bf16x6_img_f32': (_c_int, [_c_vp, _c_int, _c_vp, _c_vp, _c_vp, _c_i64, _c_i64, _c_i64, _c_int, _c_int]),
     'dcp_calib_read_f32': (_c_int, [_c_vp, _c_vp, _c_i64, _c_i64, _c_int, _c_vp]),
     'dcp_gemm_c64': (_c_int, [_c_vp, _c_int, _c_vp, _c_vp, _c_vp, _c_i64, _c_i64, _c_i64,
                               _c_int, _c_int]),
diff --git a/decomp_amd/csrc/gemm_mfma_bf16x6.hpp b/decomp_amd/csrc/gemm_mfma_bf16x6.hpp
--- a/decomp_amd/csrc/gemm_mfma_bf16x6.hpp
+++ b/decomp_amd/csrc/gemm_mfma_bf16x6.hpp
@@ -1,10 +1,10 @@
 #pragma once
 #include "gemm_mfma_f32.hpp"
+#include "x6_planes.hpp"
 #include <type_traits>
 
 namespace dcp {
 
-typedef __bf16 x6_bf16x4 __attribute__((ext_vector_type(4)));
 typedef __bf16 x6_bf16x8 __attribute__((ext_vector_type(8)));
 
 template <int BM_, int BN_, int WM_, int WN_, int MINW_, int STAGES_>
@@ -25,14 +25,6 @@
 
 __device__ __forceinline__ int x6_chunk(int r, int q) { return r * 32 + ((q ^ ((r >> 3) & 1)) << 4); }
 
-__device__ __forceinline__ void x6_split(f32x4 a, x6_bf16x4& h, x6_bf16x4& m, x6_bf16x4& l) {
-    h = __builtin_convertvector(a, x6_bf16x4);
-    const f32x4 r1 = a - __builtin_convertvector(h, f32x4);
-    m = __builtin_convertvector(r1, x6_bf16x4);
-    const f32x4 r2 = r1 - __builtin_convertvector(m, f32x4);
-    l = __builtin_convertvector(r2, x6_bf16x4);
-}
-
 template <int LAY, int ROWS, int NT, int G>
 __device__ __forceinline__ void x6_gload(f32x4 (&r)[G], const float* __restrict__ p, long ld, int row0, int k0,
                                          int tid) {
@@ -56,23 +48,65 @@
     return k * (ROWS * 2) + ((g ^ ((k & 3) << 3)) << 3);
 }
 
+template <int LAY, int ROWS>
+__device__ __forceinline__ int x6_stage_off(int idx) {
+    if (LAY == KMAJOR) {
+        const int row = idx >> 2, kq = idx & 3;
+        return x6_chunk(row, kq >> 1) + ((kq & 1) << 3);
+    }
+    return x6_granule<ROWS>(idx / (ROWS / 4), idx % (ROWS / 4));
+}
+
 template <int LAY, int ROWS, int NT, int G>
 __device__ __forceinline__ void x6_lds_store(char* s, const f32x4 (&r)[G], int tid) {
 #pragma unroll
     for (int i = 0; i < G; ++i) {
-        const int idx = tid + i * NT;
-        int off;
-        if (LAY == KMAJOR) {
-            const int row = idx >> 2, kq = idx & 3;
-            off = x6_chunk(row, kq >> 1) + ((kq & 1) << 3);
-        } else {
-            off = x6_granule<ROWS>(idx / (ROWS / 4), idx % (ROWS / 4));
-        }
+        const int off = x6_stage_off<LAY, ROWS>(tid + i * NT);
         x6_bf16x4 h, m, l;
         x6_split(r[i], h, m, l);
         *reinterpret_cast<x6_bf16x4*>(s + off) = h;
         *reinterpret_cast<x6_bf16x4*>(s + X6Panel<ROWS>::PLANE_BYTES + off) = m;
         *reinterpret_cast<x6_bf16x4*>(s + 2 * X6Panel<ROWS>::PLANE_BYTES + off) = l;
+    }
+}
+
+struct X6Planes {
+    x6_bf16x4 h, m, l;
+};
+struct X6Images {
+    const char* a = nullptr;
+    const char* b = nullptr;
+    long cb = 0;
+};
+
+template <int NT, int G>
+__device__ __forceinline__ void x6_image_voff(unsigned (&v)[G], long cb, int tid) {
+#pragma unroll
+    for (int i = 0; i < G; ++i) {
+        const int idx = tid + i * NT;
+        v[i] = (unsigned)(idx >> 6) * ((unsigned)cb * kX6ImgBlock) + ((idx & 63) << 3);
+    }
+}
+
+template <int G>
+__device__ __forceinline__ void x6_gload(X6Planes (&r)[G], const char* __restrict__ blk, const unsigned (&voff)[G]) {
+#pragma unroll
+    for (int i = 0; i < G; ++i) {
+        const char* src = blk + voff[i];
+        r[i].h = *reinterpret_cast<const x6_bf16x4*>(src);
+        r[i].m = *reinterpret_cast<const x6_bf16x4*>(src + kX6ImgPlane);
+        r[i].l = *reinterpret_cast<const x6_bf16x4*>(src + 2 * kX6ImgPlane);
+    }
+}
+
+template <int LAY, int ROWS, int NT, int G>
+__device__ __forceinline__ void x6_lds_store(char* s, const X6Planes (&r)[G], int tid) {
+#pragma unroll
+    for (int i = 0; i < G; ++i) {
+        const int off = x6_stage_off<LAY, ROWS>(tid + i * NT);
+        *reinterpret_cast<x6_bf16x4*>(s + off) = r[i].h;
+        *reinterpret_cast<x6_bf16x4*>(s + X6Panel<ROWS>::PLANE_BYTES + off) = r[i].m;
+        *reinterpret_cast<x6_bf16x4*>(s + 2 * X6Panel<ROWS>::PLANE_BYTES + off) = r[i].l;
     }
 }
 
@@ -214,8 +248,8 @@
     pass(std::integral_constant<int, 1>{});
 }
 
-template <class Cfg, int ALAY, int BLAY, class Epi>
-__global__ void __launch_bounds__(Cfg::NTHREADS, Cfg::MINW) gemm_bf16x6_kernel(GemmProblem p, Epi epi) {
+template <class Cfg, int ALAY, int BLAY, class Epi, int IMG = 0>
+__global__ void __launch_bounds__(Cfg::NTHREADS, Cfg::MINW) gemm_bf16x6_kernel(GemmProblem p, Epi epi, X6Images im) {
     constexpr int BM = Cfg::BM, BN = Cfg::BN, BK = Cfg::BK, WM = Cfg::WM, WN = Cfg::WN;
     constexpr int TM = WM / 32, TN = WN / 32;
     constexpr int WAVES_N = BN / WN;
@@ -269,22 +303,36 @@
     static_assert(TM == 2, "one panel's staging per 32-row A block");
     constexpr int STAGES = Cfg::STAGES;
     static_assert(STAGES == 2 || STAGES == 3, "two buffers and a boundary barrier, or a ring of three");
-    f32x4 ra[GA], rb[GB];
+    constexpr bool IMG_A = (IMG & 1) != 0, IMG_B = (IMG & 2) != 0;
+    static_assert(IMG == 0 || (ALAY == KMAJOR && BLAY == KMAJOR && STAGES == 3), "images feed the 256 x 256 NT tile");
+    std::conditional_t<IMG_A, X6Planes, f32x4> ra[GA];
+    std::conditional_t<IMG_B, X6Planes, f32x4> rb[GB];
+    unsigned voa[IMG_A ? GA : 1], vob[IMG_B ? GB : 1];
+    if constexpr (IMG_A) x6_image_voff<NT>(voa, im.cb, tid);
+    if constexpr (IMG_B) x6_image_voff<NT>(vob, im.cb, tid);
+    auto gload_a = [&](int k0) {
+        if constexpr (IMG_A) x6_gload(ra, im.a + ((long)(m0 >> 4) * im.cb + (k0 >> 4)) * kX6ImgBlock, voa);
+        else x6_gload<ALAY, BM, NT>(ra, p.A, p.lda, m0, k0, tid);
+    };
+    auto gload_b = [&](int k0) {
+        if constexpr (IMG_B) x6_gload(rb, im.b + ((long)(nB0 >> 4) * im.cb + (k0 >> 4)) * kX6ImgBlock, vob);
+        else x6_gload<BLAY, BN, NT>(rb, Bp, ldb, nB0, k0, tid);
+    };
     const int nkb = (kend - kbeg) / BK;
     if (nkb > 0) {
-        x6_gload<ALAY, BM, NT>(ra, p.A, p.lda, m0, kbeg, tid);
-        x6_gload<BLAY, BN, NT>(rb, Bp, ldb, nB0, kbeg, tid);
+        gload_a(kbeg);
+        gload_b(kbeg);
         x6_lds_store<ALAY, BM, NT>(x6_smem, ra, tid);
         x6_lds_store<BLAY, BN, NT>(x6_smem + X6Panel<BM>::BYTES, rb, tid);
         const int k1 = kbeg + min(1, nkb - 1) * BK;
-        x6_gload<ALAY, BM, NT>(ra, p.A, p.lda, m0, k1, tid);
-        x6_gload<BLAY, BN, NT>(rb, Bp, ldb, nB0, k1, tid);
+        gload_a(k1);
+        gload_b(k1);
         if constexpr (STAGES == 3) {
             x6_lds_store<ALAY, BM, NT>(x6_smem + BUF, ra, tid);
             x6_lds_store<BLAY, BN, NT>(x6_smem + BUF + X6Panel<BM>::BYTES, rb, tid);
             const int k2 = kbeg + min(2, nkb - 1) * BK;
-            x6_gload<ALAY, BM, NT>(ra, p.A, p.lda, m0, k2, tid);
-            x6_gload<BLAY, BN, NT>(rb, Bp, ldb, nB0, k2, tid);
+            gload_a(k2);
+            gload_b(k2);
         }
     }
     __syncthreads();
@@ -332,10 +380,10 @@
                 __builtin_amdgcn_sched_barrier(0);
                 if constexpr (i == 0) {
                     x6_lds_store<ALAY, BM, NT>(nxt, ra, tid);
-                    x6_gload<ALAY, BM, NT>(ra, p.A, p.lda, m0, knext, tid);
+                    gload_a(knext);
                 } else {
                     x6_lds_store<BLAY, BN, NT>(nxt + X6Panel<BM>::BYTES, rb, tid);
-                    x6_gload<BLAY, BN, NT>(rb, Bp, ldb, nB0, knext, tid);
+                    gload_b(knext);
                 }
                 __builtin_amdgcn_sched_barrier(0);
                 mfmas(STAGE_AFTER, 6);
@@ -418,9 +466,13 @@
     return ok;
 }
 
-template <class Cfg, int ALAY, int BLAY, class Epi>
-inline hipError_t launch_gemm_bf16x6(hipStream_t stream, GemmProblem p, const Epi& epi) {
+template <class Cfg, int ALAY, int BLAY, class Epi, int IMG = 0>
+inline hipError_t launch_gemm_bf16x6(hipStream_t stream, GemmProblem p, const Epi& epi, X6Images im = X6Images()) {
     if (!x6_eligible<Cfg>(p) || !x6_epi_ok(epi)) return hipErrorInvalidValue;
+    if constexpr (IMG != 0) {
+        if (p.B2 != nullptr || im.cb * 16 != p.K || p.K > (1 << 20) || ((IMG & 1) && im.a == nullptr) || ((IMG & 2) && im.b == nullptr))
+            return hipErrorInvalidValue;
+    }
     if constexpr (epi_den_tail<Epi>::value) {
         if (p.ksplits > 1 || p.B2 != nullptr || epi.depth < 48 || (epi.depth % 16) != 0) return hipErrorInvalidValue;
     }
@@ -436,7 +488,7 @@
     const int grid = p.tiles_m * p.tiles_n * p.ksplits;
     if (grid <= 0) return hipSuccess;
     constexpr int lds_bytes = Cfg::STAGES * (X6Panel<Cfg::BM>::BYTES + X6Panel<Cfg::BN>::BYTES);
-    const void* fn = reinterpret_cast<const void*>(&gemm_bf16x6_kernel<Cfg, ALAY, BLAY, Epi>);
+    const void* fn = reinterpret_cast<const void*>(&gemm_bf16x6_kernel<Cfg, ALAY, BLAY, Epi, IMG>);
     if constexpr (lds_bytes > 65536) {
         static DynLdsRaised raised;
         std::atomic<bool>& done = raised.on_current_device();
@@ -446,8 +498,8 @@
             done = true;
         }
     }
-    hipLaunchKernelGGL((gemm_bf16x6_kernel<Cfg, ALAY, BLAY, Epi>), dim3(grid), dim3(Cfg::NTHREADS), lds_bytes,
-                       stream, p, epi);
+    hipLaunchKernelGGL((gemm_bf16x6_kernel<Cfg, ALAY, BLAY, Epi, IMG>), dim3(grid), dim3(Cfg::NTHREADS), lds_bytes,
+                       stream, p, epi, im);
     return hipGetLastError();
 }
 
diff --git a/decomp_amd/csrc/handle.hpp b/decomp_amd/csrc/handle.hpp
--- a/decomp_amd/csrc/handle.hpp
+++ b/decomp_amd/csrc/handle.hpp
@@ -46,6 +46,7 @@
     double prof_ms[DCP_PROF_NLABELS] = {0};
     long long prof_cnt[DCP_PROF_NLABELS] = {0};
     int f32_product_mode = 0;
+    int x6_presplit = 1;
     double nmf_beta = 0.0;
     double nmf_l1 = 0.0, nmf_l2 = 0.0;
 };
diff --git a/decomp_amd/csrc/kernels_small.hpp b/decomp_amd/csrc/kernels_small.hpp
--- a/decomp_amd/csrc/kernels_small.hpp
+++ b/decomp_amd/csrc/kernels_small.hpp
@@ -1,7 +1,9 @@
 #pragma once
 #include <hip/hip_runtime.h>
+#include <type_traits>
 #include "reduce.hpp"
 #include "scalar.hpp"
+#include "x6_planes.hpp"
 
 namespace dcp {
 
@@ -203,7 +205,8 @@
                                                             real_t<T>* __restrict__ gmax = nullptr,
                                                             real_t<T>* __restrict__ gmax_zero = nullptr,
                                                             unsigned int* __restrict__ ticket = nullptr,
-                                                            real_t<T>* __restrict__ host_out = nullptr) {
+                                                            real_t<T>* __restrict__ host_out = nullptr,
+                                                            char* __restrict__ img_out = nullptr) {
     typedef real_t<T> R;
     __shared__ R sh[4];
     __shared__ R s_inv;
@@ -255,6 +258,14 @@
     } else {
         for (long j = threadIdx.x; j < F; j += 256) emit(j, u[j]);
     }
+    if constexpr (std::is_same<T, float>::value) {
+        if (img_out != nullptr) {
+            __syncthreads();
+            const float* o = out + row * ld_out;
+            for (long g = threadIdx.x; g < (F >> 2); g += 256)
+                x6_image_put(img_out, x6_image_off(row, F >> 4, g), *reinterpret_cast<const f32x4*>(o + 4 * g));
+        }
+    }
     if (rowmax != nullptr || gmax != nullptr) {
         R m = block_max_256(md, sh);
         if (threadIdx.x == 0) {
diff --git a/decomp_amd/csrc/nmf.hip b/decomp_amd/csrc/nmf.hip
--- a/decomp_amd/csrc/nmf.hip
+++ b/decomp_amd/csrc/nmf.hip
@@ -27,6 +27,10 @@
     uint32_t* mbits = nullptr;
     int* mflag = nullptr;
     const T* Ypre = nullptr;
+    bool presplit = false, presplit_y = false;
+    const T* D0 = nullptr;
+    char* y_img = nullptr;
+    char* d_img = nullptr;
 
     int64_t W() const { return nmf_stats_width(s.F, s.K, s.lik, s.masked); }
     bool want_bits() const { return s.masked && std::is_same<T, float>::value && s.lik == DCP_LIK_L2; }
@@ -38,9 +42,28 @@
             a.take(mbits, mask_bits_words(s.N, s.F));
             a.take(mflag, 4);
         }
+        if (presplit) a.take(d_img, x6_image_bytes(s.K, s.F));
+        if (presplit_y) a.take(y_img, x6_image_bytes(s.N, s.F));
+    }
+    bool shrink() {
+        const bool had = presplit_y;
+        presplit_y = false;
+        return had;
     }
     int prepare(dcp_handle* h) {
         Ypre = Y;
+        if constexpr (std::is_same<T, float>::value) {
+            if (presplit) {
+                ProfScope ps(h, DCP_PROF_MISC);
+                DCP_LAUNCH_OK(h, launch_x6_image(h->stream, D0, (long)s.F, (long)s.K, (long)s.F, d_img));
+                ws.d_img = d_img;
+                if (presplit_y) {
+                    DCP_LAUNCH_OK(h, launch_x6_image(h->stream, Y, (long)s.F, (long)s.N, (long)s.F, y_img));
+                    ws.y_img = y_img;
+                }
+                wu.d_img = d_img;
+            }
+        }
         if (!s.masked) return DCP_OK;
         int binary = 0;
         DCP_TRY(nmf_mask_prepare<T>(h, Y, mask, s.N, s.F, ws.Ym, mbits, mflag, &binary));
@@ -70,6 +93,10 @@
         return fail(h, DCP_ERR_COMM, "dcp_nmf_mu_sharded_* needs a communicator (dcp_comm_init)");
     DCP_HIP_OK(h, hipSetDevice(h->device));
     MuStep<T> step{Y, mask, NmfShape<T>{N, F, K, lik, mask != nullptr}, sharded};
+    step.D0 = D;
+    step.presplit = !sharded && h->x6_presplit != 0 && maxiter > 1 &&
+                    nmf_fused_den_ok<T>(h, step.s, Y, D, X, static_cast<const T*>(nullptr), static_cast<const T*>(nullptr));
+    step.presplit_y = step.presplit && h->x6_presplit == 2;
     return nmf_lagged_loop<T>(h, step, Y, mask, X, D, N, F, K, tol, maxiter, it_out, last_maxdiff, resid_trace);
 }
 
diff --git a/decomp_amd/csrc/nmf_hals.hip b/decomp_amd/csrc/nmf_hals.hip
--- a/decomp_amd/csrc/nmf_hals.hip
+++ b/decomp_amd/csrc/nmf_hals.hip
@@ -110,6 +110,7 @@
         a.take(nrm, (size_t)s.K);
         if (mask) a.take(Yi, (size_t)s.N * s.F);
     }
+    bool shrink() { return false; }
     int prepare(dcp_handle*) { return DCP_OK; }
     int iterate(dcp_handle* h, const T* Xc, T* Xn, const T* Dc, T* Dn, const NmfStopSlots<T>& slots) {
         const T* Yd = Y;
diff --git a/decomp_amd/csrc/nmf_impl.hpp b/decomp_amd/csrc/nmf_impl.hpp
--- a/decomp_amd/csrc/nmf_impl.hpp
+++ b/decomp_amd/csrc/nmf_impl.hpp
@@ -49,6 +49,8 @@
     T* part = nullptr;
     size_t slab_count = 0;
     const uint32_t* mbits = nullptr;
+    const char* y_img = nullptr;
+    const char* d_img = nullptr;
 };
 
 template <class T>
@@ -120,6 +122,7 @@
 struct NmfUpdateWs {
     T* U = nullptr;
     T* rowmax = nullptr;
+    char* d_img = nullptr;
 };
 template <class T>
 inline void nmf_update_layout(WsLayout& a, NmfUpdateWs<T>& w, int64_t F, int64_t K) {
@@ -147,6 +150,20 @@
             return gemm_bf16x6<FORM>(st, a, epi);
     }
     return gemm<FORM>(st, a, epi);
+}
+
+template <class T>
+inline bool nmf_fused_den_ok(const dcp_handle* h, const NmfShape<T>& s, const T* Ypre, const T* D, const T* Xin,
+                             const T* Xout, const T* G) {
+    if constexpr (std::is_same<T, float>::value) {
+        if (s.lik != DCP_LIK_L2 || s.masked || h->f32_product_mode != 0 || Xout == Xin) return false;
+        const int K = (int)s.K;
+        GemmArgs<T> fg;
+        fg.A = Ypre; fg.lda = s.F; fg.B = D; fg.ldb = s.F;
+        return nmf_xupdate_splits<T>(s.N, s.F, s.K, fg) <= 1 && x6_tier<FORM_NT>(fg) == X6_HUGE &&
+               EpiMuGramDen<false>{Xin, K, G, K, K, const_cast<float*>(Xout), K}.vec_ok();
+    }
+    return false;
 }
 
 template <class T>
@@ -219,15 +236,7 @@
     GemmArgs<T> pg_probe;
     const bool split_gram = gram && std::is_same<T, float>::value && Xout != Xin &&
                             nmf_xupdate_splits<T>(s.N, s.F, s.K, pg_probe) > 1;
-    bool fused_den = false;
-    if constexpr (std::is_same<T, float>::value) {
-        if (gram && h->f32_product_mode == 0 && Xout != Xin) {
-            GemmArgs<T> fg;
-            fg.A = Ypre; fg.lda = F; fg.B = D; fg.ldb = F;
-            fused_den = nmf_xupdate_splits<T>(s.N, s.F, s.K, fg) <= 1 && x6_tier<FORM_NT>(fg) == X6_HUGE &&
-                        EpiMuGramDen<false>{Xin, K, w.G, K, K, Xout, K}.vec_ok();
-        }
-    }
+    const bool fused_den = nmf_fused_den_ok<T>(h, s, Ypre, D, Xin, Xout, w.G);
     if (gram) {
         {
             ProfScope ps(h, DCP_PROF_GRAM);
@@ -288,12 +297,16 @@
         if (fused_den) {
             if constexpr (std::is_same<T, float>::value) {
                 const GemmProblem fp = fill_problem<FORM_NT>(pg);
-                if (pen.on())
-                    DCP_LAUNCH_OK(h, (launch_gemm_bf16x6<X6Huge, KMAJOR, KMAJOR>(
-                                         st, fp, EpiMuGramDen<true>{Xin, K, w.G, K, K, Xout, K, l1, l2})));
-                else
-                    DCP_LAUNCH_OK(h, (launch_gemm_bf16x6<X6Huge, KMAJOR, KMAJOR>(
-                                         st, fp, EpiMuGramDen<false>{Xin, K, w.G, K, K, Xout, K})));
+                const bool img_d = w.d_img != nullptr, img_y = img_d && w.y_img != nullptr;
+                const X6Images im{img_y ? w.y_img : nullptr, w.d_img, (long)(F / 16)};
+                auto fused = [&](const auto& epi) {
+                    typedef std::decay_t<decltype(epi)> E;
+                    if (img_y) return launch_gemm_bf16x6<X6Huge, KMAJOR, KMAJOR, E, 3>(st, fp, epi, im);
+                    if (img_d) return launch_gemm_bf16x6<X6Huge, KMAJOR, KMAJOR, E, 2>(st, fp, epi, im);
+                    return launch_gemm_bf16x6<X6Huge, KMAJOR, KMAJOR, E>(st, fp, epi);
+                };
+                if (pen.on()) DCP_LAUNCH_OK(h, fused(EpiMuGramDen<true>{Xin, K, w.G, K, K, Xout, K, l1, l2}));
+                else DCP_LAUNCH_OK(h, fused(EpiMuGramDen<false>{Xin, K, w.G, K, K, Xout, K}));
             }
         } else if (psplits <= 1) {
             pg.ksplits = 1;
@@ -458,7 +471,7 @@
     if (maxdiff_next != nullptr) {
         hipLaunchKernelGGL((row_normalize_kernel<T>), dim3(K), dim3(256), 0, st, w.U, (long)F,
                            (long)F, 1, D, (long)F, D_new, (long)F, (T*)nullptr, (T*)nullptr,
-                           maxdiff_dev, maxdiff_next, ticket, host_out);
+                           maxdiff_dev, maxdiff_next, ticket, host_out, w.d_img);
         DCP_LAUNCH_OK(h, hipGetLastError());
         return DCP_OK;
     }
diff --git a/decomp_amd/csrc/nmf_loop.hpp b/decomp_amd/csrc/nmf_loop.hpp
--- a/decomp_amd/csrc/nmf_loop.hpp
+++ b/decomp_amd/csrc/nmf_loop.hpp
@@ -22,7 +22,7 @@
     unsigned int* ticket = nullptr;
     T* resid_tmp = nullptr;
     double* resid_part = nullptr;
-    DCP_TRY(ws_lay_out(h, [&](WsLayout& a) {
+    auto items = [&](WsLayout& a) {
         step.layout(a);
         a.take(D2, (size_t)K * F);
         a.take(X2, (size_t)N * K);
@@ -32,7 +32,10 @@
             a.take(resid_tmp, (size_t)N * F);
             a.take(resid_part, resid_blocks);
         }
-    }));
+    };
+    int reserved = ws_lay_out(h, items);
+    if (reserved == DCP_ERR_NOMEM && step.shrink()) reserved = ws_lay_out(h, items);
+    DCP_TRY(reserved);
     void* hostv = nullptr;
     DCP_TRY(host_scratch(h, sizeof(double) * (resid_blocks + 4), &hostv));
     T* host_md = reinterpret_cast<T*>(hostv);
diff --git a/decomp_amd/csrc/util.hip b/decomp_amd/csrc/util.hip
--- a/decomp_amd/csrc/util.hip
+++ b/decomp_amd/csrc/util.hip
@@ -581,6 +581,57 @@
     }
     return DCP_OK;
 }
+int dcp_x6_image_f32(dcp_handle* h, const float* A, int64_t R, int64_t C, void* image) {
+    if (!h) return DCP_ERR_INVALID;
+    if (!A || !image) return fail(h, DCP_ERR_INVALID, "null array pointer");
+    if (R <= 0 || C <= 0 || R > INT32_MAX || C > INT32_MAX || (R % 16) != 0 || (C % 16) != 0)
+        return fail(h, DCP_ERR_INVALID, "plane image: sizes must be positive multiples of 16");
+    DCP_HIP_OK(h, hipSetDevice(h->device));
+    hipError_t e = launch_x6_image(h->stream, A, (long)C, (long)R, (long)C, static_cast<char*>(image));
+    if (e != hipSuccess) return fail(h, DCP_ERR_INVALID, "plane image: arrays must be 16-byte aligned");
+    return DCP_OK;
+}
+int dcp_gemm_bf16x6_img_f32(dcp_handle* h, int form, const float* A, const float* B, float* C, int64_t M, int64_t N,
+                            int64_t K, int ksplits, int operands) {
+    if (!h) return DCP_ERR_INVALID;
+    if (!A || !B || !C) return fail(h, DCP_ERR_INVALID, "null array pointer");
+    if (M <= 0 || N <= 0 || K <= 0 || M > INT32_MAX || N > INT32_MAX || K > INT32_MAX)
+        return fail(h, DCP_ERR_INVALID, "bad sizes");
+    if (operands < 1 || operands > 3) return fail(h, DCP_ERR_INVALID, "bf16x6 images: operands must be 1 (A), 2 (B) or 3");
+    if (form != FORM_NT || ksplits > 1)
+        return fail(h, DCP_ERR_INVALID, "bf16x6 images: no image-fed kernel for this form / split");
+    DCP_HIP_OK(h, hipSetDevice(h->device));
+    GemmArgs<float> a;
+    a.A = A; a.B = B; a.M = (int)M; a.N = (int)N; a.K = (int)K;
+    a.lda = K;
+    a.ldb = K;
+    if (x6_tier<FORM_NT>(a) != X6_HUGE)
+        return fail(h, DCP_ERR_INVALID, "bf16x6 images: no image-fed kernel for this shape (256 x 256 NT tiles only)");
+    char* ia = nullptr;
+    char* ib = nullptr;
+    DCP_TRY(ws_lay_out(h, [&](WsLayout& w) {
+        w.take(ia, x6_image_bytes(M, K));
+        w.take(ib, x6_image_bytes(N, K));
+    }));
+    if (operands & 1) DCP_LAUNCH_OK(h, launch_x6_image(h->stream, A, (long)K, (long)M, (long)K, ia));
+    if (operands & 2) DCP_LAUNCH_OK(h, launch_x6_image(h->stream, B, (long)K, (long)N, (long)K, ib));
+    const X6Images im{(operands & 1) ? ia : nullptr, (operands & 2) ? ib : nullptr, (long)(K / 16)};
+    const GemmProblem p = fill_problem<FORM_NT>(a);
+    const EpiStore<float> epi{C, (long)N};
+    hipError_t e;
+    if (operands == 1) e = launch_gemm_bf16x6<X6Huge, KMAJOR, KMAJOR, EpiStore<float>, 1>(h->stream, p, epi, im);
+    else if (operands == 2) e = launch_gemm_bf16x6<X6Huge, KMAJOR, KMAJOR, EpiStore<float>, 2>(h->stream, p, epi, im);
+    else e = launch_gemm_bf16x6<X6Huge, KMAJOR, KMAJOR, EpiStore<float>, 3>(h->stream, p, epi, im);
+    if (e != hipSuccess) return fail(h, DCP_ERR_HIP, hipGetErrorString(e));
+    return DCP_OK;
+}
+int dcp_set_x6_presplit(dcp_handle* h, int mode) {
+    if (!h) return DCP_ERR_INVALID;
+    const int prev = h->x6_presplit;
+    if (mode < -1 || mode > 2) return fail(h, DCP_ERR_INVALID, "x6 presplit mode must be 0 (never), 1 (automatic) or 2 (always)");
+    if (mode >= 0) h->x6_presplit = mode;
+    return prev;
+}
 int dcp_set_f32_product_mode(dcp_handle* h, int mode) {
     if (!h) return DCP_ERR_INVALID;
     const int prev = h->f32_product_mode;
diff --git a/decomp_amd/csrc/x6_planes.hpp b/decomp_amd/csrc/x6_planes.hpp
--- /dev/null
+++ b/decomp_amd/csrc/x6_planes.hpp
@@ -0,0 +1,61 @@
+#pragma once
+#include <hip/hip_runtime.h>
+#include <stddef.h>
+#include <stdint.h>
+
+namespace dcp {
+
+typedef float f32x4 __attribute__((ext_vector_type(4)));
+typedef __bf16 x6_bf16x4 __attribute__((ext_vector_type(4)));
+
+__device__ __forceinline__ void x6_split(f32x4 a, x6_bf16x4& h, x6_bf16x4& m, x6_bf16x4& l) {
+    h = __builtin_convertvector(a, x6_bf16x4);
+    const f32x4 r1 = a - __builtin_convertvector(h, f32x4);
+    m = __builtin_convertvector(r1, x6_bf16x4);
+    const f32x4 r2 = r1 - __builtin_convertvector(m, f32x4);
+    l = __builtin_convertvector(r2, x6_bf16x4);
+}
+
+constexpr int kX6ImgPlane = 512;
+constexpr int kX6ImgBlock = 3 * kX6ImgPlane;
+
+inline size_t x6_image_bytes(long rows, long cols) { return (size_t)(rows / 16) * (size_t)(cols / 16) * kX6ImgBlock; }
+
+__device__ __forceinline__ long x6_image_off(long row, long cb, long g) {
+    return ((row >> 4) * cb + (g >> 2)) * kX6ImgBlock + ((row & 15) << 5) + ((g & 3) << 3);
+}
+
+__device__ __forceinline__ void x6_image_put(char* img, long off, f32x4 v) {
+    x6_bf16x4 h, m, l;
+    x6_split(v, h, m, l);
+    *reinterpret_cast<x6_bf16x4*>(img + off) = h;
+    *reinterpret_cast<x6_bf16x4*>(img + off + kX6ImgPlane) = m;
+    *reinterpret_cast<x6_bf16x4*>(img + off + 2 * kX6ImgPlane) = l;
+}
+
+template <int NT>
+__global__ void __launch_bounds__(NT) x6_image_kernel(const float* __restrict__ a, long ld, long rb, long cb,
+                                                      char* __restrict__ img) {
+    const int lane = threadIdx.x & 63;
+    const long blocks = rb * cb;
+    const long wave = blockIdx.x * (long)(NT / 64) + (threadIdx.x >> 6), nwaves = (long)gridDim.x * (NT / 64);
+    for (long b = wave; b < blocks; b += nwaves) {
+        const long br = b / cb, bc = b - br * cb;
+        const long row = br * 16 + (lane >> 2), g = bc * 4 + (lane & 3);
+        x6_image_put(img, x6_image_off(row, cb, g), *reinterpret_cast<const f32x4*>(a + row * ld + 4 * g));
+    }
+}
+
+inline hipError_t launch_x6_image(hipStream_t stream, const float* a, long ld, long rows, long cols, char* img) {
+    if (rows <= 0 || cols <= 0 || (rows % 16) != 0 || (cols % 16) != 0 || (ld % 4) != 0 || a == nullptr ||
+        img == nullptr || (reinterpret_cast<uintptr_t>(a) & 15) != 0 || (reinterpret_cast<uintptr_t>(img) & 15) != 0)
+        return hipErrorInvalidValue;
+    const long blocks = (rows / 16) * (cols / 16);
+    long wgs = (blocks + 3) / 4;
+    if (wgs > 16384) wgs = 16384;
+    hipLaunchKernelGGL((x6_image_kernel<256>), dim3((unsigned)wgs), dim3(256), 0, stream, a, ld, rows / 16, cols / 16,
+                       img);
+    return hipGetLastError();
+}
+
+}
diff --git a/include/decomp_hip.h b/include/decomp_hip.h
--- a/include/decomp_hip.h
+++ b/include/decomp_hip.h
@@ -94,6 +94,13 @@
                         int64_t M, int64_t N, int64_t K, int ksplits);
 
 int dcp_set_f32_product_mode(dcp_handle* h, int mode);
+
+int dcp_set_x6_presplit(dcp_handle* h, int mode);
+
+int dcp_x6_image_f32(dcp_handle* h, const float* A, int64_t R, int64_t C, void* image);
+
+int dcp_gemm_bf16x6_img_f32(dcp_handle* h, int form, const float* A, const float* B, float* C,
+                            int64_t M, int64_t N, int64_t K, int ksplits, int operands);
 
 int dcp_debug_tn_plain(int on);
 
```

After: 718.6 iterations/s, median of 6. Within noise of the previous version (+0.7%).
